# soedinglab/PEnG-motif

Measured on AMD Instinct MI355X. Metric: 4^W pattern z-scores/s + EM PWM-kmer evals/s at W=10; Gbp/s k-mer count, higher is better.
Workload: dtype u32 counts / f32 scores / f32 serial EM sums (f64 tree sums in the throughput EM mode)

## Files before the change

### include/pengk.h

```cpp
#ifndef PENGK_H_
#define PENGK_H_

#include <stddef.h>
#include <stdint.h>

#ifdef __cplusplus
extern "C" {
#endif
#if defined(__GNUC__)
#pragma GCC visibility push(default)
#endif

#define PENGK_VERSION 100

#define PENGK_OK 0
#define PENGK_ERR_ARG 1
#define PENGK_ERR_DEVICE 2
#define PENGK_ERR_RANGE 3
#define PENGK_ERR_UNSUPPORTED 4
#define PENGK_ERR_NOMEM 5

#define PENGK_MIN_W 2
#define PENGK_MAX_W 14
#define PENGK_FRONT_PAD_BASES 64
#define PENGK_DEFAULT_ITEM_WINDOWS 256
#define PENGK_MIN_ITEM_WINDOWS 64

typedef struct pengk_ctx pengk_ctx;

int pengk_version(void);
const char* pengk_last_error(void);
const char* pengk_error_name(int code);

int pengk_create(int device, pengk_ctx** out);
int pengk_destroy(pengk_ctx* ctx);
int pengk_synchronize(pengk_ctx* ctx);
void* pengk_stream(pengk_ctx* ctx);
int pengk_set_stream(pengk_ctx* ctx, void* hip_stream);

int pengk_set_option(pengk_ctx* ctx, const char* name, int64_t value);
int pengk_get_info(pengk_ctx* ctx, const char* name, int64_t* value_out);

int pengk_malloc(pengk_ctx* ctx, size_t bytes, void** d_out);
int pengk_free(pengk_ctx* ctx, void* d_ptr);
int pengk_memcpy_h2d(pengk_ctx* ctx, void* d_dst, const void* h_src, size_t bytes);
int pengk_memcpy_d2h(pengk_ctx* ctx, void* h_dst, const void* d_src, size_t bytes);
int pengk_warmup(pengk_ctx* ctx);
int pengk_memset(pengk_ctx* ctx, void* d_dst, int byte, size_t bytes);
int pengk_host_alloc(pengk_ctx* ctx, size_t bytes, void** h_out);
int pengk_host_free(pengk_ctx* ctx, void* h_ptr);

int pengk_timer_create(pengk_ctx* ctx, void** timer_out);
int pengk_timer_record(pengk_ctx* ctx, void* timer);
int pengk_timer_elapsed_ms(pengk_ctx* ctx, void* start, void* stop, float* ms_out);
int pengk_timer_destroy(pengk_ctx* ctx, void* timer);

typedef struct pengk_packed {
  uint64_t* words;
  uint64_t n_words;
  uint64_t* items;
  uint64_t n_items;
  uint64_t n_bases;
  uint64_t n_windows;
  uint64_t max_bin_bound;
  int64_t bg_counts[84];
  uint64_t n_sequences;
  uint64_t max_len;
  int W;
  int item_windows;
  int all_whole;
} pengk_packed;

int pengk_pack(const uint8_t* h_codes, const int64_t* h_offs, int64_t n_seq, int W, int item_windows,
               pengk_packed* out);
int pengk_pack_threads(const uint8_t* h_codes, const int64_t* h_offs, int64_t n_seq, int W, int item_windows, int threads,
                       pengk_packed* out);
void pengk_packed_free(pengk_packed* p);

typedef struct pengk_pack_target {
  uint64_t* words;
  uint64_t words_cap;
  uint64_t* items;
  uint64_t items_cap;
  uint64_t word_cursor;
  uint64_t item_cursor;
} pengk_pack_target;
int pengk_pack_append(const uint8_t* h_codes, const int64_t* h_offs, int64_t n_seq, int W, int item_windows,
                      pengk_pack_target* target, pengk_packed* out);

int pengk_set_sequences(pengk_ctx* ctx, const uint64_t* d_words, uint64_t n_words, const uint64_t* d_items,
                        uint64_t n_items, int W, int item_windows, uint64_t max_bin_bound, int all_whole);

int pengk_synth_sizes(uint64_t n_seq, uint32_t L, int W, int item_windows, uint64_t* n_words, uint64_t* n_items);
int pengk_synth_sequences(pengk_ctx* ctx, uint64_t seed, uint64_t seq0, uint64_t n_seq, uint32_t L, int W,
                          int item_windows, uint64_t* d_words, uint64_t* d_items);

int pengk_count(pengk_ctx* ctx, int both_strands, uint32_t* d_counts, uint64_t* d_ltot);
int pengk_mirror_counts(pengk_ctx* ctx, int W, uint32_t* d_counts);
int pengk_count_bg(pengk_ctx* ctx, int both_strands, uint32_t* d_counts, uint64_t* d_ltot, uint64_t* d_bg_counts);

int pengk_bg_count(pengk_ctx* ctx, uint64_t* d_bg_counts);

int pengk_bg_model(pengk_ctx* ctx, const uint64_t* d_bg_counts, int K, const float* h_alpha, float* d_V);

int pengk_pattern_stats(pengk_ctx* ctx, int W, int both_strands, int k, int max_k, const float* d_V,
                        const uint64_t* d_ltot, const uint32_t* d_counts, float* d_bgprob, float* d_expected,
                        float* d_logp, float* d_z);

int pengk_seed_candidates(pengk_ctx* ctx, int W, const float* d_z, const uint32_t* d_counts, float z_threshold,
                          uint64_t count_threshold, uint32_t* h_ids, float* h_z, int64_t capacity, int64_t* n_out);

typedef struct pengk_iupac_stats {
  uint64_t sites;
  float bg_p;
  float expected;
  float zscore;
  float log_pvalue;
} pengk_iupac_stats;

int pengk_iupac_aggregate(pengk_ctx* ctx, int W, int both_strands, const uint64_t* h_iupac_ids, int64_t n,
                          const uint32_t* d_counts, const float* d_bgp, const float* d_expected,
                          pengk_iupac_stats* h_out);

int pengk_em(pengk_ctx* ctx, int W, int64_t n_pwm, float* h_pwms, float saturation, float threshold,
             int max_iterations, const uint32_t* d_counts, const float* d_bg, int* h_iters, float* h_change);

int pengk_test_em_generation(pengk_ctx* ctx, int generation);

int pengk_em_device(pengk_ctx* ctx, int W, int64_t n_pwm, float* d_pwms, float saturation, float threshold,
                    int max_iterations, const uint32_t* d_counts, const float* d_bg, int32_t* d_state,
                    float* d_change);

int pengk_sequential_sum_f32(pengk_ctx* ctx, const float* d_terms, uint64_t n_chains, uint64_t chain_len, float* d_out);

#define PENGK_MAX_MOTIF_LEN 64
int pengk_motif_similarity(pengk_ctx* ctx, int n, const float* h_pwm, const float* h_comp, const int32_t* h_len,
                           const uint64_t* h_sites, int both_strands, const float* h_bg, int first_new, float* h_out);

#define PENGK_SCORE_SENTINEL (-2147483647 - 1)

int pengk_scan_layout_words(const int64_t* h_code_offs, int64_t n_seq, uint64_t* n_words);
int pengk_scan_layout_build(const uint8_t* h_codes, const int64_t* h_code_offs, int64_t n_seq, uint64_t word0,
                            uint64_t* h_words, uint32_t* h_valid, int64_t* h_offs, uint32_t* h_lens);
int pengk_synth_scan_sequences(pengk_ctx* ctx, uint64_t seed, uint64_t seq0, uint64_t n_seq, uint32_t L, uint64_t* d_words,
                               uint32_t* d_valid, int64_t* d_offs, uint32_t* d_lens);
int pengk_sample_background(pengk_ctx* ctx, uint64_t seed, uint64_t seq0, uint64_t n_seq, const int64_t* d_offs,
                            const uint32_t* d_lens, int K, const uint32_t* h_thresholds, uint64_t* d_words);
int pengk_shuffle_sequences(pengk_ctx* ctx, uint64_t seed, uint64_t seq0, uint64_t n_seq, const uint64_t* d_words,
                            const uint32_t* d_valid, const int64_t* d_offs, const uint32_t* d_lens, uint64_t* d_out_words,
                            uint32_t* d_out_valid);
int pengk_motif_scan(pengk_ctx* ctx, const uint64_t* d_words, const uint32_t* d_valid, const int64_t* d_offs,
                     const uint32_t* d_lens, uint64_t n_seq, int n_motifs, const int32_t* h_S, const int32_t* h_len,
                     int both_strands, int32_t* d_best);
int pengk_score_histograms(pengk_ctx* ctx, int n_motifs, const int32_t* d_best, uint64_t n_seq, const int32_t* h_lo,
                           const int32_t* h_hi, const uint64_t* h_hist_offs, uint64_t* d_hist);
int pengk_score_summary(const uint64_t* h_pos, const uint64_t* h_neg, uint64_t nbins, double* zoops_out, double* occur_out);

#define PENGK_SITES_BLOCK 4096
typedef struct {
  uint32_t seq;
  uint32_t pos;
  int32_t score;
  uint32_t motif_strand;
} pengk_site;

int pengk_score_tail_pvalues(const int32_t* h_S, int w, const float* h_bg, int32_t* lo_out, int32_t* hi_out, double* h_tail);
int pengk_score_threshold(const double* h_tail, int32_t lo, int32_t hi, double p, int32_t* t_out);
int pengk_sites_count(pengk_ctx* ctx, const uint64_t* d_words, const uint32_t* d_valid, const int64_t* d_offs,
                      const uint32_t* d_lens, uint64_t n_seq, int n_motifs, const int32_t* h_S, const int32_t* h_len,
                      int both_strands, const int32_t* h_thr, uint64_t* d_counts);
int pengk_sites_histograms(pengk_ctx* ctx, const uint64_t* d_words, const uint32_t* d_valid, const int64_t* d_offs,
                           const uint32_t* d_lens, uint64_t n_seq, int n_motifs, const int32_t* h_S, const int32_t* h_len,
                           int both_strands, const int32_t* h_thr, const int32_t* h_hi, const uint64_t* h_hist_offs,
                           uint64_t* d_hist, uint64_t* d_tests, uint64_t* d_counts);
int pengk_sites_qvalues(const uint64_t* h_hist, uint64_t nbins, uint64_t n_tests, const double* h_tail_from_thr, double* h_q);
int pengk_qvalue_threshold(const double* h_q, uint64_t nbins, int32_t t, double q_max, int32_t* t_out);
int pengk_sites_slices(pengk_ctx* ctx, const uint64_t* d_counts, uint64_t n_seq, int n_motifs, uint64_t* h_motif_totals,
                       uint64_t max_slices, uint64_t* h_bounds, uint64_t* h_records, uint64_t* n_slices);
int pengk_sites_emit(pengk_ctx* ctx, const uint64_t* d_words, const uint32_t* d_valid, const int64_t* d_offs,
                     const uint32_t* d_lens, uint64_t n_seq, int n_motifs, const int32_t* h_S, const int32_t* h_len,
                     int both_strands, const int32_t* h_thr, const uint64_t* d_counts, uint64_t i0, uint64_t i1,
                     pengk_site* d_sites, uint64_t cap);

#define PENGK_CENTRALITY_MAX_LEN 65536
int pengk_motif_best_sites(pengk_ctx* ctx, const uint64_t* d_words, const uint32_t* d_valid, const int64_t* d_offs,
                           const uint32_t* d_lens, uint64_t n_seq, uint64_t seq0, int n_motifs, const int32_t* h_S,
                           const int32_t* h_len, int both_strands, int32_t* d_best, uint64_t* d_site);
int pengk_centrality_histograms(pengk_ctx* ctx, int n_motifs, const int32_t* d_best, const uint64_t* d_site,
                                const uint32_t* d_lens, uint64_t n_seq, const int32_t* h_len, const int32_t* h_thr,
                                uint32_t max_len, uint64_t* d_hist_offsets, uint64_t* d_hist_lengths);
typedef struct {
  uint64_t sites;
  uint32_t max_offset;
  uint32_t window;
  uint64_t in_window;
  double expected;
  double log10_pvalue;
  double log10_evalue;
} pengk_centrality;
int pengk_centrality_summary(const uint64_t* h_hist_offsets, const uint64_t* h_hist_lengths, uint32_t max_len, int w,
                             int n_motifs, pengk_centrality* out);
int pengk_binomial_log10_sf(uint64_t n, uint64_t k, double p, double* out);

int pengk_site_profiles(pengk_ctx* ctx, const uint64_t* d_words, const uint32_t* d_valid, const int64_t* d_offs,
                        const uint32_t* d_lens, uint64_t n_seq, int n_motifs, const int32_t* d_best, const uint64_t* d_site,
                        const int32_t* h_len, const int32_t* h_thr, int flank, uint64_t* d_counts);
int pengk_profile_refine(const uint64_t* h_counts, int w, int flank, const float* h_bg, double min_ic, double* h_q,
                         double* h_ic, float* h_pwm, int32_t* first_out, int32_t* last_out, uint64_t* sites_out);

int pengk_site_pair_profiles(pengk_ctx* ctx, const uint64_t* d_words, const uint32_t* d_valid, const int64_t* d_offs,
                             const uint32_t* d_lens, uint64_t n_seq, int n_motifs, const int32_t* d_best, const uint64_t* d_site,
                             const int32_t* h_len, const int32_t* h_thr, int flank, uint64_t* d_counts);
int pengk_dinuc_model(const uint64_t* h_counts1, const uint64_t* h_counts2, int w, int flank, const float* h_bg0,
                      const float* h_bg1, double alpha, double* h_q0, double* h_q1, double* h_mi, int32_t* h_S0, int32_t* h_D1,
                      int32_t* h_D0, uint64_t* sites_out);
int pengk_motif_scan_dinuc(pengk_ctx* ctx, const uint64_t* d_words, const uint32_t* d_valid, const int64_t* d_offs,
                           const uint32_t* d_lens, uint64_t n_seq, int n_motifs, const int32_t* h_S0, const int32_t* h_D,
                           const int32_t* h_len, int both_strands, int32_t* d_best);

#define PENGK_SPACING_MAX_MOTIFS 64
#define PENGK_SPACING_MAX_GAP 1024
int pengk_spacing_histograms(pengk_ctx* ctx, int n_motifs, const int32_t* d_best, const uint64_t* d_site,
                             const uint32_t* d_lens, uint64_t n_seq, const int32_t* h_len, const int32_t* h_thr,
                             uint32_t max_gap, uint32_t min_len, uint32_t max_len,
                             uint64_t* d_hist_gaps,
                             uint64_t* d_hist_lengths,
                             uint64_t* d_hist_motifs);
typedef struct {
  uint64_t both;
  uint64_t overlapping;
  uint64_t apart;
  uint64_t far;
  double expected_both;
  double log10_pvalue_both;
  uint32_t orientation;
  uint32_t gap;
  uint64_t count;
  double expected;
  double log10_pvalue;
  double log10_evalue;
  uint32_t tested_gaps;
} pengk_spacing;
int pengk_spacing_summary(const uint64_t* h_gaps , const uint64_t* h_lengths ,
                          uint32_t max_gap, uint32_t max_len, int w_a, int w_b, int n_classes ,
                          uint64_t n, uint64_t n_a, uint64_t n_b, int n_pairs, pengk_spacing* out);

int pengk_selftest_division(pengk_ctx* ctx, uint64_t seed, uint32_t pairs_per_thread, uint64_t* h_out );

int pengk_comm_host_init_env(void);
int pengk_comm_host_info(int* rank_out, int* world_out);
int pengk_comm_host_allgather(const void* h_send, void* h_recv, size_t bytes_per_rank);
int pengk_comm_host_allreduce_u64(uint64_t* h_buf, size_t n);
int pengk_comm_host_shutdown(void);

#define PENGK_COMM_ID_BYTES 128
int pengk_comm_unique_id(void* id_out );
int pengk_comm_init(pengk_ctx* ctx, const void* id, int rank, int world);
int pengk_comm_init_env(pengk_ctx* ctx);
int pengk_comm_info(pengk_ctx* ctx, int* rank_out, int* world_out);
int pengk_comm_init_abandoned(void);
int pengk_comm_rccl_version(void);
int pengk_comm_destroy(pengk_ctx* ctx);
int pengk_allreduce_tables(pengk_ctx* ctx, int W, uint32_t* d_counts, uint64_t* d_ltot, uint64_t* d_bg_counts);
int pengk_comm_check_bin_bound(pengk_ctx* ctx);
int pengk_allgather(pengk_ctx* ctx, const void* d_send, void* d_recv, size_t bytes_per_rank);

#if defined(__GNUC__)
#pragma GCC visibility pop
#endif
#ifdef __cplusplus
}
#endif
#endif
```

### peng-motif_amd/__init__.py

```python
import ctypes as C
import os

import numpy as np

_HERE = os.path.dirname(os.path.abspath(__file__))
LIB_PATH = os.environ.get("PENGK_LIB") or os.path.join(_HERE, "libpengk.so")
_lib = None

PENGK_OK = 0
ERR_ARG, ERR_DEVICE, ERR_RANGE, ERR_UNSUPPORTED, ERR_NOMEM = 1, 2, 3, 4, 5
FRONT_PAD_BASES = 64

EXPORTS = [
    "pengk_version", "pengk_last_error", "pengk_error_name", "pengk_create", "pengk_destroy", "pengk_synchronize",
    "pengk_stream", "pengk_set_stream", "pengk_set_option", "pengk_get_info", "pengk_malloc", "pengk_free", "pengk_memcpy_h2d", "pengk_memcpy_d2h",
    "pengk_memset", "pengk_warmup", "pengk_host_alloc", "pengk_host_free", "pengk_timer_create", "pengk_timer_record", "pengk_timer_elapsed_ms", "pengk_timer_destroy",
    "pengk_pack", "pengk_pack_threads", "pengk_pack_append", "pengk_packed_free", "pengk_set_sequences", "pengk_synth_sizes", "pengk_synth_sequences",
    "pengk_count", "pengk_count_bg", "pengk_mirror_counts", "pengk_bg_count", "pengk_bg_model", "pengk_pattern_stats",
    "pengk_seed_candidates", "pengk_iupac_aggregate", "pengk_em", "pengk_em_device", "pengk_test_em_generation", "pengk_sequential_sum_f32", "pengk_motif_similarity", "pengk_selftest_division",
    "pengk_comm_unique_id", "pengk_comm_init", "pengk_comm_init_env", "pengk_comm_info", "pengk_comm_init_abandoned", "pengk_comm_rccl_version", "pengk_comm_destroy",
    "pengk_allreduce_tables", "pengk_comm_check_bin_bound", "pengk_allgather",
    "pengk_comm_host_init_env", "pengk_comm_host_info", "pengk_comm_host_allgather", "pengk_comm_host_allreduce_u64",
    "pengk_comm_host_shutdown",
    "pengk_scan_layout_words", "pengk_scan_layout_build", "pengk_synth_scan_sequences", "pengk_sample_background",
    "pengk_shuffle_sequences",
    "pengk_motif_scan", "pengk_score_histograms", "pengk_score_summary",
    "pengk_score_tail_pvalues", "pengk_score_threshold", "pengk_sites_count", "pengk_sites_slices", "pengk_sites_emit",
    "pengk_sites_histograms", "pengk_sites_qvalues", "pengk_qvalue_threshold",
    "pengk_motif_best_sites", "pengk_centrality_histograms", "pengk_centrality_summary", "pengk_binomial_log10_sf",
    "pengk_site_profiles", "pengk_profile_refine",
    "pengk_site_pair_profiles", "pengk_dinuc_model", "pengk_motif_scan_dinuc",
    "pengk_spacing_histograms", "pengk_spacing_summary",
]
MAX_MOTIF_LEN = 64
SCORE_SENTINEL = -2 ** 31
SITES_BLOCK = 4096
SITE = np.dtype([("seq", np.uint32), ("pos", np.uint32), ("score", np.int32), ("motif_strand", np.uint32)])
CENTRALITY_MAX_LEN = 65536
SPACING_MAX_MOTIFS = 64
SPACING_MAX_GAP = 1024
SPACING_CLASSES = ("same_downstream", "same_upstream", "opposite_downstream", "opposite_upstream")


class CentralityStruct(C.Structure):
    _fields_ = [("sites", C.c_uint64), ("max_offset", C.c_uint32), ("window", C.c_uint32), ("in_window", C.c_uint64),
                ("expected", C.c_double), ("log10_pvalue", C.c_double), ("log10_evalue", C.c_double)]


class SpacingStruct(C.Structure):
    _fields_ = [("both", C.c_uint64), ("overlapping", C.c_uint64), ("apart", C.c_uint64), ("far", C.c_uint64),
                ("expected_both", C.c_double), ("log10_pvalue_both", C.c_double), ("orientation", C.c_uint32),
                ("gap", C.c_uint32), ("count", C.c_uint64), ("expected", C.c_double), ("log10_pvalue", C.c_double),
                ("log10_evalue", C.c_double), ("tested_gaps", C.c_uint32)]


class PengkError(RuntimeError):
    def __init__(self, code, msg):
        super().__init__("%s: %s" % (lib().pengk_error_name(code).decode(), msg))
        self.code = code


class PackedStruct(C.Structure):
    _fields_ = [("words", C.POINTER(C.c_uint64)), ("n_words", C.c_uint64), ("items", C.POINTER(C.c_uint64)),
                ("n_items", C.c_uint64), ("n_bases", C.c_uint64), ("n_windows", C.c_uint64), ("max_bin_bound", C.c_uint64),
                ("bg_counts", C.c_int64 * 84), ("n_sequences", C.c_uint64), ("max_len", C.c_uint64), ("W", C.c_int),
                ("item_windows", C.c_int), ("all_whole", C.c_int)]


IUPAC_STATS = np.dtype([("sites", np.uint64), ("bg_p", np.float32), ("expected", np.float32), ("zscore", np.float32),
                        ("log_pvalue", np.float32)], align=True)


def lib():
    global _lib
    if _lib is None:
        if not os.path.exists(LIB_PATH):
            raise ImportError("libpengk.so is not built: run `python peng-motif_amd/build.py` (needs hipcc)")
        L = C.CDLL(LIB_PATH)
        vp, u64, i64, f32 = C.c_void_p, C.c_uint64, C.c_int64, C.c_float
        L.pengk_version.restype = C.c_int
        L.pengk_last_error.restype = C.c_char_p
        L.pengk_error_name.restype = C.c_char_p
        L.pengk_error_name.argtypes = [C.c_int]
        L.pengk_create.argtypes = [C.c_int, C.POINTER(vp)]
        L.pengk_destroy.argtypes = [vp]
        L.pengk_synchronize.argtypes = [vp]
        L.pengk_stream.restype = vp
        L.pengk_stream.argtypes = [vp]
        L.pengk_set_stream.argtypes = [vp, vp]
        L.pengk_set_option.argtypes = [vp, C.c_char_p, i64]
        L.pengk_get_info.argtypes = [vp, C.c_char_p, C.POINTER(i64)]
        L.pengk_malloc.argtypes = [vp, C.c_size_t, C.POINTER(vp)]
        L.pengk_free.argtypes = [vp, vp]
        L.pengk_memcpy_h2d.argtypes = [vp, vp, vp, C.c_size_t]
        L.pengk_memcpy_d2h.argtypes = [vp, vp, vp, C.c_size_t]
        L.pengk_memset.argtypes = [vp, vp, C.c_int, C.c_size_t]
        L.pengk_warmup.argtypes = [vp]
        L.pengk_host_alloc.argtypes = [vp, C.c_size_t, C.POINTER(vp)]
        L.pengk_host_free.argtypes = [vp, vp]
        L.pengk_timer_create.argtypes = [vp, C.POINTER(vp)]
        L.pengk_timer_record.argtypes = [vp, vp]
        L.pengk_timer_elapsed_ms.argtypes = [vp, vp, vp, C.POINTER(f32)]
        L.pengk_timer_destroy.argtypes = [vp, vp]
        L.pengk_pack.argtypes = [vp, vp, i64, C.c_int, C.c_int, C.POINTER(PackedStruct)]
        L.pengk_pack_threads.argtypes = [vp, vp, i64, C.c_int, C.c_int, C.c_int, C.POINTER(PackedStruct)]
        L.pengk_pack_append.argtypes = [vp, vp, i64, C.c_int, C.c_int, vp, C.POINTER(PackedStruct)]
        L.pengk_packed_free.restype = None
        L.pengk_packed_free.argtypes = [C.POINTER(PackedStruct)]
        L.pengk_set_sequences.argtypes = [vp, vp, u64, vp, u64, C.c_int, C.c_int, u64, C.c_int]
        L.pengk_synth_sizes.argtypes = [u64, C.c_uint32, C.c_int, C.c_int, C.POINTER(u64), C.POINTER(u64)]
        L.pengk_synth_sequences.argtypes = [vp, u64, u64, u64, C.c_uint32, C.c_int, C.c_int, vp, vp]
        L.pengk_count.argtypes = [vp, C.c_int, vp, vp]
        L.pengk_count_bg.argtypes = [vp, C.c_int, vp, vp, vp]
        L.pengk_mirror_counts.argtypes = [vp, C.c_int, vp]
        L.pengk_bg_count.argtypes = [vp, vp]
        L.pengk_bg_model.argtypes = [vp, vp, C.c_int, vp, vp]
        L.pengk_pattern_stats.argtypes = [vp, C.c_int, C.c_int, C.c_int, C.c_int, vp, vp, vp, vp, vp, vp, vp]
        L.pengk_seed_candidates.argtypes = [vp, C.c_int, vp, vp, f32, u64, vp, vp, i64, C.POINTER(i64)]
        L.pengk_iupac_aggregate.argtypes = [vp, C.c_int, C.c_int, vp, i64, vp, vp, vp, vp]
        L.pengk_em.argtypes = [vp, C.c_int, i64, vp, f32, f32, C.c_int, vp, vp, vp, vp]
        L.pengk_em_device.argtypes = [vp, C.c_int, i64, vp, f32, f32, C.c_int, vp, vp, vp, vp]
        L.pengk_test_em_generation.argtypes = [vp, C.c_int]
        L.pengk_sequential_sum_f32.argtypes = [vp, vp, u64, u64, vp]
        L.pengk_selftest_division.argtypes = [vp, u64, C.c_uint32, vp]
        L.pengk_motif_similarity.argtypes = [vp, C.c_int, vp, vp, vp, vp, C.c_int, vp, C.c_int, vp]
        L.pengk_comm_unique_id.argtypes = [vp]
        L.pengk_comm_init.argtypes = [vp, vp, C.c_int, C.c_int]
        L.pengk_comm_init_env.argtypes = [vp]
        L.pengk_comm_info.argtypes = [vp, C.POINTER(C.c_int), C.POINTER(C.c_int)]
        L.pengk_comm_destroy.argtypes = [vp]
        L.pengk_allreduce_tables.argtypes = [vp, C.c_int, vp, vp, vp]
        L.pengk_comm_check_bin_bound.argtypes = [vp]
        L.pengk_allgather.argtypes = [vp, vp, vp, C.c_size_t]
        L.pengk_comm_host_init_env.argtypes = []
        L.pengk_comm_host_info.argtypes = [C.POINTER(C.c_int), C.POINTER(C.c_int)]
        L.pengk_comm_host_allgather.argtypes = [vp, vp, C.c_size_t]
        L.pengk_comm_host_allreduce_u64.argtypes = [vp, C.c_size_t]
        L.pengk_comm_host_shutdown.argtypes = []
        L.pengk_scan_layout_words.argtypes = [vp, i64, C.POINTER(u64)]
        L.pengk_scan_layout_build.argtypes = [vp, vp, i64, u64, vp, vp, vp, vp]
        L.pengk_synth_scan_sequences.argtypes = [vp, u64, u64, u64, C.c_uint32, vp, vp, vp, vp]
        L.pengk_sample_background.argtypes = [vp, u64, u64, u64, vp, vp, C.c_int, vp, vp]
        L.pengk_shuffle_sequences.argtypes = [vp, u64, u64, u64, vp, vp, vp, vp, vp, vp]
        L.pengk_motif_scan.argtypes = [vp, vp, vp, vp, vp, u64, C.c_int, vp, vp, C.c_int, vp]
        L.pengk_score_histograms.argtypes = [vp, C.c_int, vp, u64, vp, vp, vp, vp]
        L.pengk_score_summary.argtypes = [vp, vp, u64, C.POINTER(C.c_double), C.POINTER(C.c_double)]
        L.pengk_score_tail_pvalues.argtypes = [vp, C.c_int, vp, C.POINTER(C.c_int32), C.POINTER(C.c_int32), vp]
        L.pengk_score_threshold.argtypes = [vp, C.c_int32, C.c_int32, C.c_double, C.POINTER(C.c_int32)]
        L.pengk_sites_count.argtypes = [vp, vp, vp, vp, vp, u64, C.c_int, vp, vp, C.c_int, vp, vp]
        L.pengk_sites_histograms.argtypes = [vp, vp, vp, vp, vp, u64, C.c_int, vp, vp, C.c_int, vp, vp, vp, vp, vp, vp]
        L.pengk_sites_qvalues.argtypes = [vp, u64, u64, vp, vp]
        L.pengk_qvalue_threshold.argtypes = [vp, u64, C.c_int32, C.c_double, C.POINTER(C.c_int32)]
        L.pengk_sites_slices.argtypes = [vp, vp, u64, C.c_int, vp, u64, vp, vp, C.POINTER(u64)]
        L.pengk_sites_emit.argtypes = [vp, vp, vp, vp, vp, u64, C.c_int, vp, vp, C.c_int, vp, vp, u64, u64, vp, u64]
        L.pengk_motif_best_sites.argtypes = [vp, vp, vp, vp, vp, u64, u64, C.c_int, vp, vp, C.c_int, vp, vp]
        L.pengk_centrality_histograms.argtypes = [vp, C.c_int, vp, vp, vp, u64, vp, vp, C.c_uint32, vp, vp]
        L.pengk_centrality_summary.argtypes = [vp, vp, C.c_uint32, C.c_int, C.c_int, C.POINTER(CentralityStruct)]
        L.pengk_binomial_log10_sf.argtypes = [u64, u64, C.c_double, C.POINTER(C.c_double)]
        L.pengk_site_profiles.argtypes = [vp, vp, vp, vp, vp, u64, C.c_int, vp, vp, vp, vp, C.c_int, vp]
        L.pengk_profile_refine.argtypes = [vp, C.c_int, C.c_int, vp, C.c_double, vp, vp, vp, C.POINTER(C.c_int32),
                                           C.POINTER(C.c_int32), C.POINTER(u64)]
        L.pengk_site_pair_profiles.argtypes = [vp, vp, vp, vp, vp, u64, C.c_int, vp, vp, vp, vp, C.c_int, vp]
        L.pengk_dinuc_model.argtypes = [vp, vp, C.c_int, C.c_int, vp, vp, C.c_double, vp, vp, vp, vp, vp, vp, C.POINTER(u64)]
        L.pengk_motif_scan_dinuc.argtypes = [vp, vp, vp, vp, vp, u64, C.c_int, vp, vp, vp, C.c_int, vp]
        L.pengk_spacing_histograms.argtypes = [vp, C.c_int, vp, vp, vp, u64, vp, vp, C.c_uint32, C.c_uint32, C.c_uint32, vp, vp, vp]
        L.pengk_spacing_summary.argtypes = [vp, vp, C.c_uint32, C.c_uint32, C.c_int, C.c_int, C.c_int, u64, u64, u64, C.c_int,
                                            C.POINTER(SpacingStruct)]
        _lib = L
    return _lib


def _check(rc):
    if rc != PENGK_OK:
        raise PengkError(rc, lib().pengk_last_error().decode())


class Packed:

    def __init__(self, codes, offs, W, item_windows=0):
        codes = np.ascontiguousarray(codes, np.uint8)
        offs = np.ascontiguousarray(offs, np.int64)
        st = PackedStruct()
        _check(lib().pengk_pack(codes.ctypes.data, offs.ctypes.data, len(offs) - 1, W, item_windows, C.byref(st)))
        try:
            self.words = np.ctypeslib.as_array(st.words, shape=(st.n_words,)).copy()
            self.items = np.ctypeslib.as_array(st.items, shape=(max(st.n_items, 1),)).copy()[:st.n_items]
            self.n_bases = int(st.n_bases)
            self.n_windows = int(st.n_windows)
            self.max_bin_bound = int(st.max_bin_bound)
            self.bg_counts = np.array(list(st.bg_counts), np.int64)
            self.n_sequences = int(st.n_sequences)
            self.max_len = int(st.max_len)
            self.W = int(st.W)
            self.item_windows = int(st.item_windows)
            self.all_whole = int(st.all_whole)
        finally:
            lib().pengk_packed_free(C.byref(st))


class ScanLayout:

    def __init__(self, codes, offs):
        codes = np.ascontiguousarray(codes, np.uint8)
        offs = np.ascontiguousarray(offs, np.int64)
        n = len(offs) - 1
        nw = C.c_uint64()
        _check(lib().pengk_scan_layout_words(offs.ctypes.data, n, C.byref(nw)))
        self.n_seq = n
        self.words = np.zeros(max(nw.value, 1), np.uint64)
        self.valid = np.zeros(max(nw.value, 1), np.uint32)
        self.offs = np.zeros(max(n, 1), np.int64)
        self.lens = np.zeros(max(n, 1), np.uint32)
        _check(lib().pengk_scan_layout_build(codes.ctypes.data, offs.ctypes.data, n, 0, self.words.ctypes.data,
                                             self.valid.ctypes.data, self.offs.ctypes.data, self.lens.ctypes.data))


def score_summary(pos_hist, neg_hist):
    p = np.ascontiguousarray(pos_hist, np.uint64)
    n = np.ascontiguousarray(neg_hist, np.uint64)
    assert p.shape == n.shape
    z, o = C.c_double(), C.c_double()
    _check(lib().pengk_score_summary(p.ctypes.data, n.ctypes.data, len(p), C.byref(z), C.byref(o)))
    return z.value, o.value


def score_tail_pvalues(S, bg):
    S = np.ascontiguousarray(S, np.int32)
    bg = np.ascontiguousarray(bg, np.float32)
    lo, hi = C.c_int32(), C.c_int32()
    _check(lib().pengk_score_tail_pvalues(S.ctypes.data, S.shape[0], bg.ctypes.data, C.byref(lo), C.byref(hi), None))
    tail = np.zeros(hi.value - lo.value + 1, np.float64)
    _check(lib().pengk_score_tail_pvalues(S.ctypes.data, S.shape[0], bg.ctypes.data, C.byref(lo), C.byref(hi), tail.ctypes.data))
    return lo.value, tail


def score_threshold(tail, lo, p):
    tail = np.ascontiguousarray(tail, np.float64)
    t = C.c_int32()
    _check(lib().pengk_score_threshold(tail.ctypes.data, lo, lo + len(tail) - 1, p, C.byref(t)))
    return t.value


def sites_qvalues(hist, n_tests, tail_from_thr):
    h = np.ascontiguousarray(hist, np.uint64)
    tail = np.ascontiguousarray(tail_from_thr, np.float64)
    assert len(tail) >= len(h)
    q = np.zeros(len(h), np.float64)
    _check(lib().pengk_sites_qvalues(h.ctypes.data, len(h), int(n_tests), tail.ctypes.data, q.ctypes.data))
    return q


def qvalue_threshold(q, t, q_max):
    q = np.ascontiguousarray(q, np.float64)
    out = C.c_int32()
    _check(lib().pengk_qvalue_threshold(q.ctypes.data, len(q), t, q_max, C.byref(out)))
    return out.value


def centrality_summary(hist_offsets, hist_lengths, max_len, w, n_motifs):
    hd = np.ascontiguousarray(hist_offsets, np.uint64)
    hl = np.ascontiguousarray(hist_lengths, np.uint64)
    assert len(hd) == 2 * max_len + 1 and len(hl) == max_len + 1
    out = CentralityStruct()
    _check(lib().pengk_centrality_summary(hd.ctypes.data, hl.ctypes.data, max_len, w, n_motifs, C.byref(out)))
    return {k: getattr(out, k) for k, _ in CentralityStruct._fields_}


def binomial_log10_sf(n, k, p):
    out = C.c_double()
    _check(lib().pengk_binomial_log10_sf(int(n), int(k), float(p), C.byref(out)))
    return out.value


def spacing_summary(hist_gaps, hist_lengths, max_gap, max_len, w_a, w_b, n_classes, n, n_a, n_b, n_pairs):
    hg = np.ascontiguousarray(hist_gaps, np.uint64)
    hl = np.ascontiguousarray(hist_lengths, np.uint64)
    assert len(hg) == 4 * (max_gap + 1) + 2 and len(hl) == max_len + 1
    out = SpacingStruct()
    _check(lib().pengk_spacing_summary(hg.ctypes.data, hl.ctypes.data, max_gap, max_len, w_a, w_b, n_classes, int(n), int(n_a),
                                       int(n_b), n_pairs, C.byref(out)))
    return {k: getattr(out, k) for k, _ in SpacingStruct._fields_}


def clamp_flank(w, flank):
    return min(int(flank), (MAX_MOTIF_LEN - int(w)) // 2)


def profile_refine(counts, w, flank, bg, min_ic):
    F = clamp_flank(w, flank)
    n = w + 2 * F
    k = np.ascontiguousarray(np.asarray(counts, np.uint64).reshape(-1, 5)[:n])
    assert len(k) == n
    b = np.ascontiguousarray(bg, np.float32)
    q, ic = np.zeros((n, 4), np.float64), np.zeros(n, np.float64)
    pwm = np.zeros((MAX_MOTIF_LEN, 4), np.float32)
    first, last, sites = C.c_int32(), C.c_int32(), C.c_uint64()
    _check(lib().pengk_profile_refine(k.ctypes.data, w, int(flank), b.ctypes.data, float(min_ic), q.ctypes.data, ic.ctypes.data,
                                      pwm.ctypes.data, C.byref(first), C.byref(last), C.byref(sites)))
    return {"q": q, "ic": ic, "first": first.value, "last": last.value, "pwm": pwm[:last.value - first.value].copy(),
            "sites": sites.value}


def dinuc_model(counts1, counts2, w, flank, bg0, bg1, alpha):
    F = clamp_flank(w, flank)
    n = w + 2 * F
    k1 = np.ascontiguousarray(np.asarray(counts1, np.uint64).reshape(-1, 5)[:n])
    k2 = np.ascontiguousarray(np.asarray(counts2, np.uint64).reshape(-1, 17)[:n])
    assert len(k1) == n and len(k2) == n
    g0 = np.ascontiguousarray(bg0, np.float32)
    g1 = np.ascontiguousarray(bg1, np.float32).reshape(-1)
    assert len(g0) == 4 and len(g1) == 16
    q0, q1, mi = np.zeros((n, 4), np.float64), np.zeros((n, 16), np.float64), np.zeros(n, np.float64)
    S0, D1, D0 = np.zeros(4, np.int32), np.zeros((n, 16), np.int32), np.zeros((n, 16), np.int32)
    sites = C.c_uint64()
    _check(lib().pengk_dinuc_model(k1.ctypes.data, k2.ctypes.data, w, int(flank), g0.ctypes.data, g1.ctypes.data, float(alpha),
                                   q0.ctypes.data, q1.ctypes.data, mi.ctypes.data, S0.ctypes.data, D1.ctypes.data,
                                   D0.ctypes.data, C.byref(sites)))
    return {"q0": q0, "q1": q1, "mi": mi, "S0": S0, "D1": D1, "D0": D0, "sites": sites.value, "flank": F}


def _pad_motifs(S, lens):
    n = len(lens)
    Sp = np.zeros((max(n, 1), MAX_MOTIF_LEN, 4), np.int32)
    for m in range(n):
        Sp[m, :lens[m]] = np.asarray(S[m], np.int32)[:lens[m]]
    return Sp, np.ascontiguousarray(lens, np.int32)


class DeviceArray:

    def __init__(self, ctx, shape, dtype):
        self.ctx = ctx
        self.shape = tuple(np.atleast_1d(shape).tolist())
        self.dtype = np.dtype(dtype)
        self.nbytes = int(np.prod(self.shape)) * self.dtype.itemsize
        p = C.c_void_p()
        _check(lib().pengk_malloc(ctx.h, self.nbytes, C.byref(p)))
        self.ptr = p.value

    @classmethod
    def from_host(cls, ctx, a):
        a = np.ascontiguousarray(a)
        d = cls(ctx, a.shape, a.dtype)
        if d.nbytes:
            _check(lib().pengk_memcpy_h2d(ctx.h, d.ptr, a.ctypes.data, d.nbytes))
        return d

    def to_host(self):
        out = np.empty(self.shape, self.dtype)
        if self.nbytes:
            _check(lib().pengk_memcpy_d2h(self.ctx.h, out.ctypes.data, self.ptr, self.nbytes))
        return out

    def free(self):
        if self.ptr and self.ctx.h:
            lib().pengk_free(self.ctx.h, self.ptr)
        self.ptr = None

    def __del__(self):
        try:
            self.free()
        except Exception:
            pass


def _ptr(x):
    if isinstance(x, DeviceArray):
        return x.ptr
    if hasattr(x, "data_ptr"):
        return x.data_ptr()
    return int(x)


class Context:
    def __init__(self, device=0):
        h = C.c_void_p()
        self.h = None
        _check(lib().pengk_create(device, C.byref(h)))
        self.h = h.value
        self._keep = []
        self.W = None

    def close(self):
        if self.h:
            for k in self._keep:
                if isinstance(k, DeviceArray):
                    k.free()
            self._keep = []
            lib().pengk_destroy(self.h)
            self.h = None

    def __del__(self):
        try:
            self.close()
        except Exception:
            pass

    def synchronize(self):
        _check(lib().pengk_synchronize(self.h))

    def set_option(self, name, value):
        _check(lib().pengk_set_option(self.h, name.encode(), int(value)))

    def test_em_generation(self, generation):
        _check(lib().pengk_test_em_generation(self.h, int(generation)))

    def info(self, name):
        v = C.c_int64()
        _check(lib().pengk_get_info(self.h, name.encode(), C.byref(v)))
        return int(v.value)

    def empty(self, shape, dtype):
        return DeviceArray(self, shape, dtype)

    def to_device(self, a):
        return DeviceArray.from_host(self, a)

    def timer(self):
        t = C.c_void_p()
        _check(lib().pengk_timer_create(self.h, C.byref(t)))
        return t.value

    def record(self, t):
        _check(lib().pengk_timer_record(self.h, t))

    def elapsed_ms(self, a, b):
        ms = C.c_float()
        _check(lib().pengk_timer_elapsed_ms(self.h, a, b, C.byref(ms)))
        return float(ms.value)

    def set_sequences(self, words, items, n_words, n_items, W, item_windows, max_bin_bound, all_whole):
        _check(lib().pengk_set_sequences(self.h, _ptr(words), n_words, _ptr(items), n_items, W, item_windows,
                                         max_bin_bound, all_whole))
        self._keep = [words, items]
        self.W = W

    def upload(self, packed):
        words = self.to_device(packed.words)
        items = self.to_device(packed.items if len(packed.items) else np.zeros(1, np.uint64))
        self.set_sequences(words, items, len(packed.words), len(packed.items), packed.W, packed.item_windows,
                           packed.max_bin_bound, packed.all_whole)
        self.set_option("n_windows_hint", packed.n_windows)
        return words, items

    def synth(self, seed, seq0, n_seq, L, W, item_windows=0, words=None, items=None):
        nw, ni = C.c_uint64(), C.c_uint64()
        _check(lib().pengk_synth_sizes(n_seq, L, W, item_windows, C.byref(nw), C.byref(ni)))
        if words is None:
            words = self.empty(nw.value, np.uint64)
        if items is None:
            items = self.empty(max(ni.value, 1), np.uint64)
        _check(lib().pengk_synth_sequences(self.h, seed, seq0, n_seq, L, W, item_windows, _ptr(words), _ptr(items)))
        self._keep = [words, items]
        self.W = W
        return words, items, int(nw.value), int(ni.value)

    def count(self, both, counts=None, ltot=None):
        if counts is None:
            counts = self.empty(4 ** self.W, np.uint32)
        if ltot is None:
            ltot = self.empty(1, np.uint64)
        _check(lib().pengk_count(self.h, int(both), _ptr(counts), _ptr(ltot)))
        return counts, ltot

    def count_bg(self, both, counts=None, ltot=None, bg=None):
        counts = counts if counts is not None else self.empty(4 ** self.W, np.uint32)
        ltot = ltot if ltot is not None else self.empty(1, np.uint64)
        bg = bg if bg is not None else self.empty(84, np.uint64)
        _check(lib().pengk_count_bg(self.h, int(both), _ptr(counts), _ptr(ltot), _ptr(bg)))
        return counts, ltot, bg

    def mirror(self, W, counts):
        _check(lib().pengk_mirror_counts(self.h, W, _ptr(counts)))

    def bg_count(self, out=None):
        if out is None:
            out = self.empty(84, np.uint64)
        _check(lib().pengk_bg_count(self.h, _ptr(out)))
        return out

    def bg_model(self, bg_counts, K=2, alpha=(1.0, 1.0, 1.0), out=None):
        if out is None:
            out = self.empty(84, np.float32)
        a = np.asarray(alpha, np.float32)
        _check(lib().pengk_bg_model(self.h, _ptr(bg_counts), K, a.ctypes.data, _ptr(out)))
        return out

    def pattern_stats(self, W, both, k, max_k, V, ltot, counts, bgprob=None, expected=None, logp=None, z=None):
        n = 4 ** W
        bgprob = bgprob if bgprob is not None else self.empty((max_k + 1, n), np.float32)
        expected = expected if expected is not None else self.empty(n, np.float32)
        logp = logp if logp is not None else self.empty(n, np.float32)
        z = z if z is not None else self.empty(n, np.float32)
        _check(lib().pengk_pattern_stats(self.h, W, int(both), k, max_k, _ptr(V), _ptr(ltot), _ptr(counts), _ptr(bgprob),
                                         _ptr(expected), _ptr(logp), _ptr(z)))
        return bgprob, expected, logp, z

    def iupac_aggregate(self, W, both, ids, counts, bgp, expected):
        ids = np.ascontiguousarray(ids, np.uint64)
        out = np.zeros(len(ids), IUPAC_STATS)
        assert IUPAC_STATS.itemsize == 24
        _check(lib().pengk_iupac_aggregate(self.h, W, int(both), ids.ctypes.data, len(ids), _ptr(counts), _ptr(bgp),
                                           _ptr(expected), out.ctypes.data))
        return out

    def em(self, W, pwms, counts, bg, saturation=1e4, threshold=0.08, max_iterations=10):
        p = np.ascontiguousarray(pwms, np.float32).copy().reshape(-1, W, 4)
        n = p.shape[0]
        iters = np.zeros(n, np.int32)
        change = np.zeros(n, np.float32)
        _check(lib().pengk_em(self.h, W, n, p.ctypes.data, saturation, threshold, max_iterations, _ptr(counts), _ptr(bg),
                              iters.ctypes.data, change.ctypes.data))
        return p, iters, change

    def sequential_sum(self, terms):
        t = np.ascontiguousarray(terms, np.float32)
        t = t.reshape(1, -1) if t.ndim == 1 else t
        d_t = DeviceArray.from_host(self, t.reshape(-1)) if t.size else None
        d_o = DeviceArray.from_host(self, np.zeros(max(t.shape[0], 1), np.float32))
        _check(lib().pengk_sequential_sum_f32(self.h, _ptr(d_t) if d_t is not None else None, t.shape[0], t.shape[1], _ptr(d_o)))
        return d_o.to_host()[:t.shape[0]]

    def upload_scan(self, layout):
        return (self.to_device(layout.words), self.to_device(layout.valid), self.to_device(layout.offs),
                self.to_device(layout.lens), layout.n_seq)

    def synth_scan(self, seed, seq0, n_seq, L):
        nw = n_seq * ((L + 31) // 32)
        words, valid = self.empty(max(nw, 1), np.uint64), self.empty(max(nw, 1), np.uint32)
        offs, lens = self.empty(max(n_seq, 1), np.int64), self.empty(max(n_seq, 1), np.uint32)
        _check(lib().pengk_synth_scan_sequences(self.h, seed, seq0, n_seq, L, _ptr(words), _ptr(valid), _ptr(offs), _ptr(lens)))
        return words, valid, offs, lens, n_seq

    def sample_background(self, scan, seed, seq0, K, thresholds, words=None):
        th = np.ascontiguousarray(thresholds, np.uint32).reshape(-1)
        assert len(th) == 3 * (1, 5, 21)[K]
        if words is None:
            words = self.empty(scan[0].shape, np.uint64)
        _check(lib().pengk_sample_background(self.h, seed, seq0, scan[4], _ptr(scan[2]), _ptr(scan[3]), K, th.ctypes.data,
                                             _ptr(words)))
        return words

    def shuffle_sequences(self, scan, seed, seq0, all_valid=False, words=None, valid=None):
        if words is None:
            words = self.empty(scan[0].shape, np.uint64)
        if valid is None and not all_valid:
            valid = self.empty(scan[1].shape, np.uint32)
        _check(lib().pengk_shuffle_sequences(self.h, seed, seq0, scan[4], _ptr(scan[0]), None if all_valid else _ptr(scan[1]),
                                             _ptr(scan[2]), _ptr(scan[3]), _ptr(words), None if valid is None else _ptr(valid)))
        return words, valid

    def motif_scan(self, scan, S, lens, both, words=None, all_valid=False, best=None):
        n = len(lens)
        Sp = np.zeros((max(n, 1), MAX_MOTIF_LEN, 4), np.int32)
        for m in range(n):
            Sp[m, :lens[m]] = np.asarray(S[m], np.int32)[:lens[m]]
        ln = np.ascontiguousarray(lens, np.int32)
        if best is None:
            best = self.empty((max(n, 1), max(scan[4], 1)), np.int32)
# ... 176 lines not shown
```

### peng-motif_amd/csrc/api.hip

```cpp
#include <stdarg.h>
#include <stdio.h>
#include <string.h>
#include <stdlib.h>
#include <time.h>

#include <new>

#include "pengk_internal.h"

namespace pengk {

static thread_local char g_err[512] = "";

int fail(int code, const char* fmt, ...) {
  va_list ap;
  va_start(ap, fmt);
  vsnprintf(g_err, sizeof g_err, fmt, ap);
  va_end(ap);
  return code;
}

int hip_fail(hipError_t e, const char* what) {
  return fail(PENGK_ERR_DEVICE, "%s: %s", what, hipGetErrorString(e));
}

int ensure_scratch(pengk_ctx* ctx, void** slot, size_t* have, size_t need) {
  if (*have >= need) return PENGK_OK;
  if (*slot) PENGK_HIP(hipFree(*slot));
  *slot = nullptr;
  *have = 0;
  PENGK_HIP(hipMalloc(slot, need));
  *have = need;
  return PENGK_OK;
}

int enter(pengk_ctx* ctx) {
  PENGK_HIP(hipSetDevice(ctx->device));
  return PENGK_OK;
}

static int warm_code_objects() {
  int rc = warm_stats();
  if (!rc) rc = warm_iupac();
  if (!rc) rc = warm_em();
  if (!rc) rc = warm_similarity();
  return rc;
}

}

using namespace pengk;

#define PENGK_ENTER(ctx)               \
  do {                                 \
    int rc_enter_ = ::pengk::enter(ctx); \
    if (rc_enter_) return rc_enter_;   \
  } while (0)

extern "C" {

int pengk_version(void) { return PENGK_VERSION; }
const char* pengk_last_error(void) { return g_err; }

const char* pengk_error_name(int code) {
  switch (code) {
    case PENGK_OK: return "PENGK_OK";
    case PENGK_ERR_ARG: return "PENGK_ERR_ARG";
    case PENGK_ERR_DEVICE: return "PENGK_ERR_DEVICE";
    case PENGK_ERR_RANGE: return "PENGK_ERR_RANGE";
    case PENGK_ERR_UNSUPPORTED: return "PENGK_ERR_UNSUPPORTED";
    case PENGK_ERR_NOMEM: return "PENGK_ERR_NOMEM";
    default: return "PENGK_ERR_?";
  }
}

int pengk_create(int device, pengk_ctx** out) {
  if (!out) return fail(PENGK_ERR_ARG, "pengk_create: out is NULL");
  *out = nullptr;
  const bool timing = getenv("PENGK_TIMING_CREATE") != nullptr;
  timespec t_prev;
  clock_gettime(CLOCK_MONOTONIC, &t_prev);
  auto lap = [&](const char* what) {
    if (!timing) return;
    timespec t;
    clock_gettime(CLOCK_MONOTONIC, &t);
    fprintf(stderr, "[pengk_create] %s: %.1f ms\n", what, (t.tv_sec - t_prev.tv_sec) * 1e3 + (t.tv_nsec - t_prev.tv_nsec) * 1e-6);
    t_prev = t;
  };
  int n = 0;
  hipError_t e = hipGetDeviceCount(&n);
  lap("hipGetDeviceCount (runtime start)");
  if (e != hipSuccess || n <= 0)
    return fail(PENGK_ERR_DEVICE, "pengk_create: no HIP device (%s); this library has no CPU fallback",
                e == hipSuccess ? "device count 0" : hipGetErrorString(e));
  if (device < 0 || device >= n) return fail(PENGK_ERR_ARG, "pengk_create: device %d out of range [0,%d)", device, n);
  PENGK_HIP(hipSetDevice(device));
  hipDeviceProp_t prop;
  PENGK_HIP(hipGetDeviceProperties(&prop, device));
  lap("hipSetDevice + properties");
  if (strncmp(prop.gcnArchName, "gfx950", 6) != 0)
    return fail(PENGK_ERR_DEVICE, "pengk_create: device %d is %s; this build targets gfx950 only", device, prop.gcnArchName);
  pengk_ctx* c = new (std::nothrow) pengk_ctx();
  if (!c) return fail(PENGK_ERR_NOMEM, "pengk_create: out of host memory");
  c->device = device;
  c->num_cu = prop.multiProcessorCount;
  e = hipStreamCreateWithFlags(&c->stream, hipStreamNonBlocking);
  if (e != hipSuccess) {
    delete c;
    return hip_fail(e, "hipStreamCreate");
  }
  c->own_stream = true;
  lap("stream");
  int rc = count_init_device();
  lap("kernel attributes (code object load)");
  if (rc) {
    (void)hipStreamDestroy(c->stream);
    delete c;
    return rc;
  }
  *out = c;
  return PENGK_OK;
}

int pengk_destroy(pengk_ctx* ctx) {
  if (!ctx) return PENGK_OK;
  (void)hipSetDevice(ctx->device);
  (void)hipStreamSynchronize(ctx->stream);
  comm_release(ctx);
  if (ctx->d_defer) (void)hipFree(ctx->d_defer);
  if (ctx->d_em_partials) (void)hipFree(ctx->d_em_partials);
  if (ctx->d_em_tables) (void)hipFree(ctx->d_em_tables);
  if (ctx->d_em_blocks) (void)hipFree(ctx->d_em_blocks);
  if (ctx->d_em_counters) (void)hipFree(ctx->d_em_counters);
  if (ctx->d_em_look) (void)hipFree(ctx->d_em_look);
  if (ctx->d_pair_mids) (void)hipFree(ctx->d_pair_mids);
  for (int l = 0; l < 3; ++l) {
    if (ctx->em_streams[l]) (void)hipStreamDestroy(ctx->em_streams[l]);
    if (ctx->em_join[l]) (void)hipEventDestroy(ctx->em_join[l]);
  }
  if (ctx->em_fork) (void)hipEventDestroy(ctx->em_fork);
  if (ctx->d_misc) (void)hipFree(ctx->d_misc);
  if (ctx->d_keys) (void)hipFree(ctx->d_keys);
  if (ctx->d_iupac_big) (void)hipFree(ctx->d_iupac_big);
  if (ctx->d_bg_partials) (void)hipFree(ctx->d_bg_partials);
  if (ctx->d_count_aux) (void)hipFree(ctx->d_count_aux);
  if (ctx->d_sim) (void)hipFree(ctx->d_sim);
  if (ctx->d_score) (void)hipFree(ctx->d_score);
  if (ctx->d_sites) (void)hipFree(ctx->d_sites);
  if (ctx->own_stream && ctx->stream) (void)hipStreamDestroy(ctx->stream);
  delete ctx;
  return PENGK_OK;
}

int pengk_synchronize(pengk_ctx* ctx) {
  if (!ctx) return fail(PENGK_ERR_ARG, "ctx is NULL");
  PENGK_ENTER(ctx);
  PENGK_HIP(hipStreamSynchronize(ctx->stream));
  return PENGK_OK;
}

int pengk_set_option(pengk_ctx* ctx, const char* name, int64_t value) {
  if (!ctx || !name) return fail(PENGK_ERR_ARG, "pengk_set_option: NULL argument");
  if (strcmp(name, "count_impl") == 0) {
    if (value < 0 || value > 2) return fail(PENGK_ERR_ARG, "count_impl must be 0 (auto), 1 (direct) or 2 (partition)");
    ctx->count_impl = (int)value;
    return PENGK_OK;
  }
  if (strcmp(name, "count_group") == 0) {
    if (value != 0 && value != 64 && value != 128) return fail(PENGK_ERR_ARG, "count_group must be 0 (auto), 64 or 128 keys per group");
    ctx->count_group = (int)value;
    return PENGK_OK;
  }
  if (strcmp(name, "count_probe_slice") == 0) {
    if (value < 0) return fail(PENGK_ERR_ARG, "count_probe_slice must be >= 0 (wave * buckets + bucket)");
    ctx->count_probe_slice = (uint64_t)value;
    return PENGK_OK;
  }
  if (strcmp(name, "key_cap_override") == 0) {
    ctx->key_cap_override = (uint64_t)value;
    return PENGK_OK;
  }
  if (strcmp(name, "em_fast") == 0) {
    if (value < 0 || value > 2) return fail(PENGK_ERR_ARG, "em_fast must be 0 (reference terms), 1 (fast) or 2 (serial, bit-exact)");
    ctx->em_fast = (int)value;
    return PENGK_OK;
  }
  if (strcmp(name, "em_serial_scan") == 0) {
    if (value < 2 || value > 3)
      return fail(PENGK_ERR_ARG, "em_serial_scan must be 2 (blocks evaluated ahead of their chain, three launches per iteration) or 3 (two: weights and block evaluation as one kernel); earlier generations: pengk_test_em_generation");
    ctx->em_serial_scan = (int)value;
    return PENGK_OK;
  }
  if (strcmp(name, "em_test_lookback") == 0) {
    if (value < 0 || value > 1000000) return fail(PENGK_ERR_ARG, "em_test_lookback must be 0 (off) or the n of 'every n-th workgroup'");
    ctx->em_test_lookback = (int)value;
    return PENGK_OK;
  }
  if (strcmp(name, "em_test_skew") == 0) {
    if (value < 0 || value > 1000000) return fail(PENGK_ERR_ARG, "em_test_skew must be 0 (off) or the n of 'every n-th block'");
    ctx->em_test_skew = (int)value;
    return PENGK_OK;
  }
  if (strcmp(name, "em_head_blocks") == 0) {
    if (value < 1 || value > 64) return PENGK_ERR_ARG;
    ctx->em_head_blocks = (int)value;
    return PENGK_OK;
  }
  if (strcmp(name, "sweep_pairs") == 0) {
    ctx->sweep_pairs = value != 0;
    return PENGK_OK;
  }
  if (strcmp(name, "em_lean_div") == 0) {
    ctx->em_lean_div = value != 0;
    return PENGK_OK;
  }
  if (strcmp(name, "em_overlap") == 0) {
    if (value < 1 || value > MAX_EM_LANES) return fail(PENGK_ERR_ARG, "em_overlap must be 1 .. %d streams", MAX_EM_LANES);
    ctx->em_overlap = (int)value;
    return PENGK_OK;
  }
  if (strcmp(name, "em_table_budget_mb") == 0) {
    if (value < 0) return fail(PENGK_ERR_ARG, "em_table_budget_mb must be >= 0 (0 = automatic)");
    ctx->em_table_budget_mb = (uint64_t)value;
    return PENGK_OK;
  }
  if (strcmp(name, "iupac_group_bytes") == 0) {
    ctx->iupac_group_bytes = (uint64_t)value;
    return PENGK_OK;
  }
  if (strcmp(name, "sites_record_budget") == 0) {
    if (value < 1) return fail(PENGK_ERR_ARG, "sites_record_budget must be >= 1 record");
    ctx->sites_record_budget = (uint64_t)value;
    return PENGK_OK;
  }
  if (strcmp(name, "scatter_blocks_per_cu") == 0) {
    if (value < 0 || value > 8) return fail(PENGK_ERR_ARG, "scatter_blocks_per_cu must be 0 (default) .. 8");
    ctx->scatter_blocks_per_cu = (int)value;
    return PENGK_OK;
  }
  if (strcmp(name, "n_windows_hint") == 0) {
    ctx->n_windows_hint = (uint64_t)value;
    return PENGK_OK;
  }
  return fail(PENGK_ERR_ARG, "unknown option '%s'", name);
}

int pengk_get_info(pengk_ctx* ctx, const char* name, int64_t* value) {
  if (!ctx || !name || !value) return fail(PENGK_ERR_ARG, "pengk_get_info: NULL argument");
  PENGK_ENTER(ctx);
  if (strcmp(name, "deferred_items") == 0) {
    uint32_t n = 0;
    if (ctx->d_defer_count) {
      PENGK_HIP(hipMemcpyAsync(&n, ctx->d_defer_count, sizeof n, hipMemcpyDeviceToHost, ctx->stream));
      PENGK_HIP(hipStreamSynchronize(ctx->stream));
    }
    *value = n;
    return PENGK_OK;
  }
  if (strcmp(name, "count_wrapped_workgroups") == 0) {
    uint32_t n = 0;
    if (ctx->d_wrap_count) {
      PENGK_HIP(hipMemcpyAsync(&n, ctx->d_wrap_count, sizeof n, hipMemcpyDeviceToHost, ctx->stream));
      PENGK_HIP(hipStreamSynchronize(ctx->stream));
    }
    *value = n;
    return PENGK_OK;
  }
  if (strcmp(name, "count_group") == 0) {
    *value = ctx->count_group;
    return PENGK_OK;
  }
  if (strcmp(name, "count_group_used") == 0) {
    *value = ctx->count_group_used;
    return PENGK_OK;
  }
  if (strcmp(name, "count_slices") == 0) {
    *value = ctx->d_slice_fill ? (int64_t)ctx->n_slice_fill : 0;
    return PENGK_OK;
  }
  if (strcmp(name, "count_slice_fill") == 0) {
    if (!ctx->d_slice_fill || ctx->count_probe_slice >= ctx->n_slice_fill)
      return fail(PENGK_ERR_ARG, "count_slice_fill: the last count has no slice %llu", (unsigned long long)ctx->count_probe_slice);
    uint32_t n = 0;
    PENGK_HIP(hipMemcpyAsync(&n, ctx->d_slice_fill + ctx->count_probe_slice, sizeof n, hipMemcpyDeviceToHost, ctx->stream));
    PENGK_HIP(hipStreamSynchronize(ctx->stream));
    *value = n;
    return PENGK_OK;
  }
  if (strcmp(name, "sites_record_budget") == 0) {
    *value = (int64_t)ctx->sites_record_budget;
    return PENGK_OK;
  }
  if (strcmp(name, "num_cu") == 0) {
    *value = ctx->num_cu;
    return PENGK_OK;
  }
  static const char* const em_names[4] = {"em_fetched_blocks", "em_mispredicted_blocks", "em_restaged_blocks", "em_restaged_waits"};
  for (int i = 0; i < 4; ++i)
    if (strcmp(name, em_names[i]) == 0) {
      unsigned long long v = 0;
      if (ctx->d_em_counters) {
        PENGK_HIP(hipMemcpyAsync(&v, ctx->d_em_counters + i, sizeof v, hipMemcpyDeviceToHost, ctx->stream));
        PENGK_HIP(hipStreamSynchronize(ctx->stream));
      }
      *value = (int64_t)v;
      return PENGK_OK;
    }
  return fail(PENGK_ERR_ARG, "unknown info '%s'", name);
}

void* pengk_stream(pengk_ctx* ctx) { return ctx ? (void*)ctx->stream : nullptr; }

int pengk_set_stream(pengk_ctx* ctx, void* s) {
  if (!ctx) return fail(PENGK_ERR_ARG, "ctx is NULL");
  PENGK_ENTER(ctx);
  PENGK_HIP(hipStreamSynchronize(ctx->stream));
  if (ctx->own_stream && ctx->stream) PENGK_HIP(hipStreamDestroy(ctx->stream));
  ctx->stream = (hipStream_t)s;
  ctx->own_stream = false;
  return PENGK_OK;
}

int pengk_malloc(pengk_ctx* ctx, size_t bytes, void** d_out) {
  if (!ctx || !d_out) return fail(PENGK_ERR_ARG, "pengk_malloc: NULL argument");
  PENGK_HIP(hipSetDevice(ctx->device));
  hipError_t e = hipMalloc(d_out, bytes ? bytes : 1);
  if (e != hipSuccess) return fail(PENGK_ERR_NOMEM, "hipMalloc(%zu): %s", bytes, hipGetErrorString(e));
  return PENGK_OK;
}

int pengk_free(pengk_ctx* ctx, void* d_ptr) {
  if (!ctx) return fail(PENGK_ERR_ARG, "ctx is NULL");
  PENGK_ENTER(ctx);
  if (d_ptr) {
    PENGK_HIP(hipStreamSynchronize(ctx->stream));
    PENGK_HIP(hipFree(d_ptr));
  }
  return PENGK_OK;
}

int pengk_host_alloc(pengk_ctx* ctx, size_t bytes, void** h_out) {
  if (!ctx || !h_out) return fail(PENGK_ERR_ARG, "pengk_host_alloc: NULL argument");
  PENGK_HIP(hipSetDevice(ctx->device));
  hipError_t e = hipHostMalloc(h_out, bytes ? bytes : 1, hipHostMallocDefault);
  if (e != hipSuccess) return fail(PENGK_ERR_NOMEM, "hipHostMalloc(%zu): %s", bytes, hipGetErrorString(e));
  return PENGK_OK;
}

int pengk_host_free(pengk_ctx* ctx, void* h_ptr) {
  if (!ctx) return fail(PENGK_ERR_ARG, "ctx is NULL");
  PENGK_ENTER(ctx);
  if (h_ptr) {
    PENGK_HIP(hipStreamSynchronize(ctx->stream));
    PENGK_HIP(hipHostFree(h_ptr));
  }
  return PENGK_OK;
}

int pengk_memcpy_h2d(pengk_ctx* ctx, void* d_dst, const void* h_src, size_t bytes) {
  if (!ctx || (bytes && (!d_dst || !h_src))) return fail(PENGK_ERR_ARG, "pengk_memcpy_h2d: NULL argument");
  PENGK_ENTER(ctx);
  PENGK_HIP(hipMemcpyAsync(d_dst, h_src, bytes, hipMemcpyHostToDevice, ctx->stream));
  PENGK_HIP(hipStreamSynchronize(ctx->stream));
  return PENGK_OK;
}

int pengk_warmup(pengk_ctx* ctx) {
  if (!ctx) return fail(PENGK_ERR_ARG, "ctx is NULL");
  PENGK_ENTER(ctx);
  constexpr size_t N = (size_t)4 << 20;
  void* d = nullptr;
  void* h = nullptr;
  hipError_t e = hipMalloc(&d, N);
  if (e == hipSuccess) e = hipHostMalloc(&h, N, hipHostMallocDefault);
  if (e == hipSuccess) e = hipMemcpyAsync(h, d, N, hipMemcpyDeviceToHost, ctx->stream);
  if (e == hipSuccess) e = hipStreamSynchronize(ctx->stream);
  if (h) (void)hipHostFree(h);
  if (d) (void)hipFree(d);
  if (e != hipSuccess) return hip_fail(e, "pengk_warmup");
  return warm_code_objects();
}

int pengk_memcpy_d2h(pengk_ctx* ctx, void* h_dst, const void* d_src, size_t bytes) {
  if (!ctx || (bytes && (!h_dst || !d_src))) return fail(PENGK_ERR_ARG, "pengk_memcpy_d2h: NULL argument");
  PENGK_ENTER(ctx);
  PENGK_HIP(hipMemcpyAsync(h_dst, d_src, bytes, hipMemcpyDeviceToHost, ctx->stream));
  PENGK_HIP(hipStreamSynchronize(ctx->stream));
  return PENGK_OK;
}

int pengk_memset(pengk_ctx* ctx, void* d_dst, int byte, size_t bytes) {
  if (!ctx || (bytes && !d_dst)) return fail(PENGK_ERR_ARG, "pengk_memset: NULL argument");
  PENGK_ENTER(ctx);
  PENGK_HIP(hipMemsetAsync(d_dst, byte, bytes, ctx->stream));
  return PENGK_OK;
}

int pengk_timer_create(pengk_ctx* ctx, void** out) {
  if (!ctx || !out) return fail(PENGK_ERR_ARG, "pengk_timer_create: NULL argument");
  PENGK_ENTER(ctx);
  hipEvent_t ev;
  PENGK_HIP(hipEventCreate(&ev));
  *out = (void*)ev;
  return PENGK_OK;
}
int pengk_timer_record(pengk_ctx* ctx, void* t) {
  if (!ctx || !t) return fail(PENGK_ERR_ARG, "pengk_timer_record: NULL argument");
  PENGK_ENTER(ctx);
  PENGK_HIP(hipEventRecord((hipEvent_t)t, ctx->stream));
  return PENGK_OK;
}
int pengk_timer_elapsed_ms(pengk_ctx* ctx, void* a, void* b, float* ms) {
  if (!ctx || !a || !b || !ms) return fail(PENGK_ERR_ARG, "pengk_timer_elapsed_ms: NULL argument");
  PENGK_ENTER(ctx);
  PENGK_HIP(hipEventSynchronize((hipEvent_t)b));
  PENGK_HIP(hipEventElapsedTime(ms, (hipEvent_t)a, (hipEvent_t)b));
  return PENGK_OK;
}
int pengk_timer_destroy(pengk_ctx* ctx, void* t) {
  (void)ctx;
  if (t) PENGK_HIP(hipEventDestroy((hipEvent_t)t));
  return PENGK_OK;
// ... 28 lines not shown
  const uint64_t per = (nwin + item_windows - 1) / item_windows;
  *n_items = n_seq * per;
  const uint64_t bases = PENGK_FRONT_PAD_BASES + n_seq * (uint64_t)L;
  *n_words = (bases + 31) / 32 + 4;
  return PENGK_OK;
}

int pengk_synth_sequences(pengk_ctx* ctx, uint64_t seed, uint64_t seq0, uint64_t n_seq, uint32_t L, int W,
                          int item_windows, uint64_t* d_words, uint64_t* d_items) {
  if (!ctx || !d_words || !d_items) return fail(PENGK_ERR_ARG, "pengk_synth_sequences: NULL argument");
  PENGK_ENTER(ctx);
  if (item_windows == 0) item_windows = PENGK_DEFAULT_ITEM_WINDOWS;
  uint64_t nw = 0, ni = 0;
  int rc = pengk_synth_sizes(n_seq, L, W, item_windows, &nw, &ni);
  if (rc) return rc;
  if (item_windows < PENGK_MIN_ITEM_WINDOWS || item_windows > 65535) return fail(PENGK_ERR_ARG, "item_windows out of range");
  rc = launch_synth(ctx, seed, seq0, n_seq, L, W, item_windows, d_words, d_items);
  if (rc) return rc;
  const uint64_t nwin = (uint64_t)L - W + 1;
  rc = pengk_set_sequences(ctx, d_words, nw, d_items, ni, W, item_windows, n_seq * ((nwin + W - 1) / W), 1);
  if (rc) return rc;
  ctx->n_windows_hint = n_seq * nwin;
  return PENGK_OK;
}

int pengk_count(pengk_ctx* ctx, int both, uint32_t* d_counts, uint64_t* d_ltot) {
  if (!ctx || !d_counts || !d_ltot) return fail(PENGK_ERR_ARG, "pengk_count: NULL argument");
  if (!ctx->d_words) return fail(PENGK_ERR_ARG, "pengk_count: no sequences attached");
  PENGK_ENTER(ctx);
  if (ctx->max_bin_bound >= (1ull << 32))
    return fail(PENGK_ERR_RANGE, "a count bin could reach %llu >= 2^32 on this shard; split the input",
                (unsigned long long)ctx->max_bin_bound);
  return launch_count(ctx, both ? 1 : 0, d_counts, d_ltot, nullptr);
}

int pengk_count_bg(pengk_ctx* ctx, int both, uint32_t* d_counts, uint64_t* d_ltot, uint64_t* d_bg) {
  if (!ctx || !d_counts || !d_ltot || !d_bg) return fail(PENGK_ERR_ARG, "pengk_count_bg: NULL argument");
  if (!ctx->d_words) return fail(PENGK_ERR_ARG, "pengk_count_bg: no sequences attached");
  PENGK_ENTER(ctx);
  if (!ctx->all_whole)
    return fail(PENGK_ERR_UNSUPPORTED, "pengk_count_bg: input has invalid bases or sequences shorter than W; use pengk_packed.bg_counts");
  if (ctx->max_bin_bound >= (1ull << 32))
    return fail(PENGK_ERR_RANGE, "a count bin could reach %llu >= 2^32 on this shard; split the input",
                (unsigned long long)ctx->max_bin_bound);
  return launch_count(ctx, both ? 1 : 0, d_counts, d_ltot, d_bg);
}

int pengk_mirror_counts(pengk_ctx* ctx, int W, uint32_t* d_counts) {
  if (!ctx || !d_counts) return fail(PENGK_ERR_ARG, "pengk_mirror_counts: NULL argument");
  PENGK_ENTER(ctx);
  if (!valid_w(W)) return fail(PENGK_ERR_ARG, "pattern length %d unsupported", W);
  return launch_mirror(ctx, W, d_counts);
}

int pengk_bg_count(pengk_ctx* ctx, uint64_t* d_bg) {
  if (!ctx || !d_bg) return fail(PENGK_ERR_ARG, "pengk_bg_count: NULL argument");
  if (!ctx->d_words) return fail(PENGK_ERR_ARG, "pengk_bg_count: no sequences attached");
  PENGK_ENTER(ctx);
  if (!ctx->all_whole)
    return fail(PENGK_ERR_UNSUPPORTED, "pengk_bg_count: input has invalid bases or sequences shorter than W; use pengk_packed.bg_counts");
  return launch_bg_count(ctx, d_bg);
}

int pengk_bg_model(pengk_ctx* ctx, const uint64_t* d_bg, int K, const float* h_alpha, float* d_V) {
  if (!ctx || !d_bg || !h_alpha || !d_V) return fail(PENGK_ERR_ARG, "pengk_bg_model: NULL argument");
  PENGK_ENTER(ctx);
  if (K < 0 || K > 2) return fail(PENGK_ERR_ARG, "background order %d unsupported (0..2)", K);
  return launch_bg_model(ctx, d_bg, K, h_alpha, d_V);
}

int pengk_pattern_stats(pengk_ctx* ctx, int W, int both, int k, int max_k, const float* d_V, const uint64_t* d_ltot,
                        const uint32_t* d_counts, float* d_bgprob, float* d_expected, float* d_logp, float* d_z) {
  if (!ctx || !d_V || !d_ltot || !d_counts || !d_bgprob || !d_expected || !d_logp || !d_z)
    return fail(PENGK_ERR_ARG, "pengk_pattern_stats: NULL argument");
  PENGK_ENTER(ctx);
  if (!valid_w(W)) return fail(PENGK_ERR_ARG, "pattern length %d unsupported", W);
  if (k < 0 || max_k > 2 || k > max_k || max_k > W - 1) return fail(PENGK_ERR_ARG, "background orders k=%d max_k=%d unsupported", k, max_k);
  return launch_stats(ctx, W, both ? 1 : 0, k, max_k, d_V, d_ltot, d_counts, d_bgprob, d_expected, d_logp, d_z);
}

int pengk_seed_candidates(pengk_ctx* ctx, int W, const float* d_z, const uint32_t* d_counts, float z_threshold,
                          uint64_t count_threshold, uint32_t* h_ids, float* h_z, int64_t capacity, int64_t* n_out) {
  if (!ctx || !d_z || !d_counts || !n_out || (capacity && (!h_ids || !h_z))) return fail(PENGK_ERR_ARG, "pengk_seed_candidates: NULL argument");
  if (!valid_w(W)) return fail(PENGK_ERR_ARG, "pattern length %d unsupported", W);
  if (capacity < 0 || capacity > (int64_t)1 << 28) return fail(PENGK_ERR_ARG, "pengk_seed_candidates: capacity out of range");
  PENGK_ENTER(ctx);
  const uint32_t cap = (uint32_t)capacity;
  const size_t need = 256 + (size_t)cap * 8;
  int rc = ensure_scratch(ctx, &ctx->d_misc, &ctx->misc_bytes, need);
  if (rc) return rc;
  uint32_t* d_n = (uint32_t*)ctx->d_misc;
  uint32_t* d_ids = (uint32_t*)((char*)ctx->d_misc + 256);
  float* d_zs = (float*)(d_ids + cap);
  rc = launch_seed_candidates(ctx, W, d_z, d_counts, z_threshold, count_threshold, cap, d_n, d_ids, d_zs);
  if (rc) return rc;
  uint32_t n = 0;
  PENGK_HIP(hipMemcpyAsync(&n, d_n, sizeof n, hipMemcpyDeviceToHost, ctx->stream));
  PENGK_HIP(hipStreamSynchronize(ctx->stream));
  *n_out = n;
  const uint32_t got = n < cap ? n : cap;
  if (got) {
    PENGK_HIP(hipMemcpyAsync(h_ids, d_ids, (size_t)got * 4, hipMemcpyDeviceToHost, ctx->stream));
    PENGK_HIP(hipMemcpyAsync(h_z, d_zs, (size_t)got * 4, hipMemcpyDeviceToHost, ctx->stream));
    PENGK_HIP(hipStreamSynchronize(ctx->stream));
  }
  return PENGK_OK;
}

int pengk_iupac_aggregate(pengk_ctx* ctx, int W, int both, const uint64_t* h_ids, int64_t n, const uint32_t* d_counts,
                          const float* d_bgp, const float* d_expected, pengk_iupac_stats* h_out) {
  if (!ctx || (n && (!h_ids || !h_out)) || !d_counts || !d_bgp || !d_expected)
    return fail(PENGK_ERR_ARG, "pengk_iupac_aggregate: NULL argument");
  PENGK_ENTER(ctx);
  if (!valid_w(W)) return fail(PENGK_ERR_ARG, "pattern length %d unsupported", W);
  if (n < 0) return fail(PENGK_ERR_ARG, "negative pattern count");
  if (n == 0) return PENGK_OK;
  return launch_iupac(ctx, W, both ? 1 : 0, h_ids, n, d_counts, d_bgp, d_expected, h_out);
}

int pengk_motif_similarity(pengk_ctx* ctx, int n, const float* h_pwm, const float* h_comp, const int32_t* h_len,
                           const uint64_t* h_sites, int both, const float* h_bg, int first_new, float* h_out) {
  if (!ctx || !h_pwm || !h_comp || !h_len || !h_sites || !h_bg || !h_out) return fail(PENGK_ERR_ARG, "pengk_motif_similarity: NULL argument");
  if (n < 0 || first_new < 0 || first_new > n) return fail(PENGK_ERR_ARG, "pengk_motif_similarity: n = %d, first_new = %d", n, first_new);
  for (int i = 0; i < n; ++i)
    if (h_len[i] < 1 || h_len[i] > PENGK_MAX_MOTIF_LEN)
      return fail(PENGK_ERR_UNSUPPORTED, "pengk_motif_similarity: motif %d has %d columns (1..%d)", i, h_len[i], PENGK_MAX_MOTIF_LEN);
  long long pairs = 0;
  for (int j = first_new; j < n; ++j) pairs += j;
  if (pairs == 0) return PENGK_OK;
  PENGK_ENTER(ctx);
  const size_t pw = (size_t)n * PENGK_MAX_MOTIF_LEN * 4 * sizeof(float);
  const size_t o_len = 2 * pw, o_sites = (o_len + (size_t)n * 4 + 255) & ~(size_t)255, o_out = (o_sites + (size_t)n * 8 + 255) & ~(size_t)255;
  int rc = ensure_scratch(ctx, &ctx->d_sim, &ctx->sim_bytes, o_out + (size_t)pairs * sizeof(float));
  if (rc) return rc;
  char* base = (char*)ctx->d_sim;
  PENGK_HIP(hipMemcpyAsync(base, h_pwm, pw, hipMemcpyHostToDevice, ctx->stream));
  PENGK_HIP(hipMemcpyAsync(base + pw, h_comp, pw, hipMemcpyHostToDevice, ctx->stream));
  PENGK_HIP(hipMemcpyAsync(base + o_len, h_len, (size_t)n * 4, hipMemcpyHostToDevice, ctx->stream));
  PENGK_HIP(hipMemcpyAsync(base + o_sites, h_sites, (size_t)n * 8, hipMemcpyHostToDevice, ctx->stream));
  rc = launch_similarity(ctx, n, (const float*)base, (const float*)(base + pw), (const int32_t*)(base + o_len),
                         (const uint64_t*)(base + o_sites), both ? 1 : 0, h_bg, first_new, (float*)(base + o_out));
  if (rc) return rc;
  PENGK_HIP(hipMemcpyAsync(h_out, base + o_out, (size_t)pairs * sizeof(float), hipMemcpyDeviceToHost, ctx->stream));
  PENGK_HIP(hipStreamSynchronize(ctx->stream));
  return PENGK_OK;
}

int pengk_sequential_sum_f32(pengk_ctx* ctx, const float* d_terms, uint64_t n_chains, uint64_t chain_len, float* d_out) {
  if (!ctx || (!d_terms && n_chains && chain_len) || (!d_out && n_chains)) return fail(PENGK_ERR_ARG, "pengk_sequential_sum_f32: NULL argument");
  PENGK_ENTER(ctx);
  return launch_sequential_sum(ctx, d_terms, n_chains, chain_len, d_out);
}

int pengk_test_em_generation(pengk_ctx* ctx, int generation) {
  if (!ctx) return fail(PENGK_ERR_ARG, "pengk_test_em_generation: NULL context");
  if (generation < 0 || generation > 3) return fail(PENGK_ERR_ARG, "pengk_test_em_generation: 0 (dependent additions), 1 (scan), 2 / 3 (the library's scheme)");
  ctx->em_serial_scan = generation;
  return PENGK_OK;
}

int pengk_em_device(pengk_ctx* ctx, int W, int64_t n_pwm, float* d_pwms, float saturation, float threshold, int max_it,
                    const uint32_t* d_counts, const float* d_bg, int32_t* d_state, float* d_change) {
  if (!ctx || !d_pwms || !d_counts || !d_bg || !d_state || !d_change) return fail(PENGK_ERR_ARG, "pengk_em_device: NULL argument");
  PENGK_ENTER(ctx);
  if (!valid_w(W)) return fail(PENGK_ERR_ARG, "pattern length %d unsupported", W);
  if (n_pwm < 0) return fail(PENGK_ERR_ARG, "negative count");
  if (max_it < 0) max_it = 0;
  if (n_pwm == 0) return PENGK_OK;
  return launch_em(ctx, W, n_pwm, d_pwms, saturation, threshold, max_it, d_counts, d_bg, d_state, d_change);
}

int pengk_em(pengk_ctx* ctx, int W, int64_t n_pwm, float* h_pwms, float saturation, float threshold, int max_it,
             const uint32_t* d_counts, const float* d_bg, int* h_iters, float* h_change) {
  if (!ctx || (n_pwm && !h_pwms) || !d_counts || !d_bg) return fail(PENGK_ERR_ARG, "pengk_em: NULL argument");
  PENGK_ENTER(ctx);
  if (!valid_w(W)) return fail(PENGK_ERR_ARG, "pattern length %d unsupported", W);
  if (n_pwm < 0) return fail(PENGK_ERR_ARG, "negative count");
  if (max_it < 0) max_it = 0;
  if (n_pwm == 0) return PENGK_OK;
  const size_t pw = (size_t)n_pwm * W * 4 * sizeof(float);
  const size_t st = (size_t)n_pwm * 2 * sizeof(int32_t);
  const size_t ch = (size_t)n_pwm * sizeof(float);
  const size_t need = ((pw + 255) & ~(size_t)255) + ((st + 255) & ~(size_t)255) + ch;
  int rc = ensure_scratch(ctx, &ctx->d_misc, &ctx->misc_bytes, need);
  if (rc) return rc;
  float* d_pwms = (float*)ctx->d_misc;
  int32_t* d_state = (int32_t*)((char*)ctx->d_misc + ((pw + 255) & ~(size_t)255));
  float* d_change = (float*)((char*)d_state + ((st + 255) & ~(size_t)255));
  PENGK_HIP(hipMemcpyAsync(d_pwms, h_pwms, pw, hipMemcpyHostToDevice, ctx->stream));
  rc = launch_em(ctx, W, n_pwm, d_pwms, saturation, threshold, max_it, d_counts, d_bg, d_state, d_change);
  if (rc) return rc;
  PENGK_HIP(hipMemcpyAsync(h_pwms, d_pwms, pw, hipMemcpyDeviceToHost, ctx->stream));
  PENGK_HIP(hipStreamSynchronize(ctx->stream));
  if (h_iters || h_change) {
    int32_t* tmp = new (std::nothrow) int32_t[(size_t)n_pwm * 2];
    if (!tmp) return fail(PENGK_ERR_NOMEM, "pengk_em: out of host memory");
    hipError_t e = hipMemcpy(tmp, d_state, st, hipMemcpyDeviceToHost);
    if (e == hipSuccess && h_change) e = hipMemcpy(h_change, d_change, ch, hipMemcpyDeviceToHost);
    if (h_iters)
      for (int64_t i = 0; i < n_pwm; ++i) h_iters[i] = tmp[2 * i];
    delete[] tmp;
    if (e != hipSuccess) return hip_fail(e, "pengk_em: copy back");
  }
  return PENGK_OK;
}

}
```

### peng-motif_amd/csrc/count.hip

```cpp
#include <stdlib.h>

#include <type_traits>

#include "pengk_internal.h"

namespace pengk {

namespace {

constexpr uint32_t INVALID_ID = 0xFFFFFFFFu;

__device__ __forceinline__ uint32_t funnel(uint32_t hi, uint32_t lo, uint32_t shift) {
  return __builtin_amdgcn_alignbit(hi, lo, shift);
}

template <int W>
struct Geo {
  static constexpr int P = ((3 * W - 3 + 15) / 16) * 16;
  static constexpr uint32_t MASK = (1u << (2 * W)) - 1u;
  static constexpr int TOP = 2 * (W - 1);
  static constexpr int PER = (32 - 2 * W) / 2 + 1;
  static constexpr int NVIEW = (W - 1 + PER - 1) / PER;
};

__device__ __forceinline__ uint32_t revcomp16(uint32_t x) {
  const uint32_t r = __builtin_bitreverse32(x);
  return ~(((r >> 1) & 0x55555555u) | ((r & 0x55555555u) << 1));
}

struct BgLds {
  uint32_t bins[96];
  uint32_t bins4[256];
};
__device__ __forceinline__ BgLds& bg_lds() {
  __shared__ BgLds sh;
  return sh;
}
template <int W, bool BG>
struct BgCount {
  uint32_t wave;
  __device__ __forceinline__ void kmer3(uint32_t id, bool on) const {
    if (BG) atomicAdd(&bg_lds().bins[on ? (id >> (2 * W - 6)) : 95u], 1u);
  }
  __device__ __forceinline__ void kmer4(uint32_t v) const {
    if (BG) atomicAdd(&bg_lds().bins4[v], 1u);
  }
  __device__ __forceinline__ void head(uint32_t id, int sp, bool on) const {
    if (!BG || !on || sp < 0) return;
    if (sp == 0) atomicAdd(&bg_lds().bins[64 + (id >> (2 * W - 2))], 1u);
    else if (sp == 1) atomicAdd(&bg_lds().bins[68 + (id >> (2 * W - 4))], 1u);
    else atomicAdd(&bg_lds().bins[id >> (2 * W - 6)], 1u);
  }
};

template <bool BG>
__device__ __forceinline__ void bg_begin() {
  if (BG) {
    for (uint32_t i = threadIdx.x; i < 96u; i += blockDim.x) bg_lds().bins[i] = 0;
    for (uint32_t i = threadIdx.x; i < 256u; i += blockDim.x) bg_lds().bins4[i] = 0;
  }
}
template <bool BG>
__device__ __forceinline__ void bg_end(uint32_t* __restrict__ bg_partials) {
  if (BG) {
    __syncthreads();
    if (threadIdx.x < 84) {
      const BgLds& b = bg_lds();
      const uint32_t k = threadIdx.x;
      uint32_t v = b.bins[k];
      if (k < 64) {
        for (uint32_t c = 0; c < 4; ++c) v += b.bins4[k | (c << 6)] + b.bins4[(k << 2) | c];
      }
      bg_partials[(size_t)blockIdx.x * 84 + k] = v;
    }
  }
}

template <int W>
struct Suppress {
  static __device__ __forceinline__ uint32_t apply(uint32_t can, const uint32_t (&ring)[16], int u) {
    uint32_t out = INVALID_ID;
    unsigned long long save;
#define PENGK_R(d) "v"(ring[(u - (d)) & 15])
#define PENGK_CX(n) "v_cmpx_ne_u32_e32 %2, %" #n "\n\t"
#define PENGK_HEAD "s_mov_b64 %1, exec\n\t"
#define PENGK_TAIL "v_mov_b32_e32 %0, %2\n\ts_mov_b64 exec, %1"
    if constexpr (W == 2)
      asm volatile(PENGK_HEAD PENGK_CX(3) PENGK_TAIL : "+v"(out), "=&s"(save) : "v"(can), PENGK_R(1) : "vcc");
    else if constexpr (W == 4)
      asm volatile(PENGK_HEAD PENGK_CX(3) PENGK_CX(4) PENGK_CX(5) PENGK_TAIL
                   : "+v"(out), "=&s"(save) : "v"(can), PENGK_R(1), PENGK_R(2), PENGK_R(3) : "vcc");
    else if constexpr (W == 6)
      asm volatile(PENGK_HEAD PENGK_CX(3) PENGK_CX(4) PENGK_CX(5) PENGK_CX(6) PENGK_CX(7) PENGK_TAIL
                   : "+v"(out), "=&s"(save) : "v"(can), PENGK_R(1), PENGK_R(2), PENGK_R(3), PENGK_R(4), PENGK_R(5) : "vcc");
    else if constexpr (W == 8)
      asm volatile(PENGK_HEAD PENGK_CX(3) PENGK_CX(4) PENGK_CX(5) PENGK_CX(6) PENGK_CX(7) PENGK_CX(8) PENGK_CX(9) PENGK_TAIL
                   : "+v"(out), "=&s"(save)
                   : "v"(can), PENGK_R(1), PENGK_R(2), PENGK_R(3), PENGK_R(4), PENGK_R(5), PENGK_R(6), PENGK_R(7) : "vcc");
    else if constexpr (W == 10)
      asm volatile(PENGK_HEAD PENGK_CX(3) PENGK_CX(4) PENGK_CX(5) PENGK_CX(6) PENGK_CX(7) PENGK_CX(8) PENGK_CX(9) PENGK_CX(10)
                   PENGK_CX(11) PENGK_TAIL
                   : "+v"(out), "=&s"(save)
                   : "v"(can), PENGK_R(1), PENGK_R(2), PENGK_R(3), PENGK_R(4), PENGK_R(5), PENGK_R(6), PENGK_R(7), PENGK_R(8),
                     PENGK_R(9) : "vcc");
    else if constexpr (W == 12)
      asm volatile(PENGK_HEAD PENGK_CX(3) PENGK_CX(4) PENGK_CX(5) PENGK_CX(6) PENGK_CX(7) PENGK_CX(8) PENGK_CX(9) PENGK_CX(10)
                   PENGK_CX(11) PENGK_CX(12) PENGK_CX(13) PENGK_TAIL
                   : "+v"(out), "=&s"(save)
                   : "v"(can), PENGK_R(1), PENGK_R(2), PENGK_R(3), PENGK_R(4), PENGK_R(5), PENGK_R(6), PENGK_R(7), PENGK_R(8),
                     PENGK_R(9), PENGK_R(10), PENGK_R(11) : "vcc");
    else {
      static_assert(W == 14, "pattern lengths 2 .. 14");
      asm volatile(PENGK_HEAD PENGK_CX(3) PENGK_CX(4) PENGK_CX(5) PENGK_CX(6) PENGK_CX(7) PENGK_CX(8) PENGK_CX(9) PENGK_CX(10)
                   PENGK_CX(11) PENGK_CX(12) PENGK_CX(13) PENGK_CX(14) PENGK_CX(15) PENGK_TAIL
                   : "+v"(out), "=&s"(save)
                   : "v"(can), PENGK_R(1), PENGK_R(2), PENGK_R(3), PENGK_R(4), PENGK_R(5), PENGK_R(6), PENGK_R(7), PENGK_R(8),
                     PENGK_R(9), PENGK_R(10), PENGK_R(11), PENGK_R(12), PENGK_R(13) : "vcc");
    }
#undef PENGK_R
#undef PENGK_CX
#undef PENGK_HEAD
#undef PENGK_TAIL
    return out;
  }
};

template <int W, bool BOTH, bool BG, class Emit>
__device__ __forceinline__ void scan_items(const uint32_t* __restrict__ words32, const uint64_t* __restrict__ items,
                                           uint32_t n_items, unsigned long long* __restrict__ ltot,
                                           uint32_t* __restrict__ defer_count, uint32_t* __restrict__ defer_list,
                                           Emit& emit) {
  using G = Geo<W>;
  const BgCount<W, BG> bgc{threadIdx.x >> 6};
  const uint32_t lane_global = blockIdx.x * blockDim.x + threadIdx.x;
  const uint32_t stride = gridDim.x * blockDim.x;
  unsigned long long my_windows = 0;

  for (uint32_t wave_base = lane_global & ~63u; wave_base < n_items; wave_base += stride) {
    const uint32_t it = wave_base + (threadIdx.x & 63u);
    const bool live = it < n_items;
    const uint64_t rec = live ? items[it] : 0ull;
    uint32_t nw = (uint32_t)((rec >> ITEM_NW_SHIFT) & ITEM_NW_MASK);
    const uint64_t ws = rec & ITEM_WS_MASK;
    const bool cont = ((rec >> ITEM_CONT_SHIFT) & 1ull) != 0;
    const uint32_t nw_all = nw;
    my_windows += nw;

    uint32_t ring[16];
#pragma unroll
    for (int i = 0; i < 16; ++i) ring[i] = INVALID_ID;
    uint32_t id = 0, rc = 0;

    const uint64_t g0 = live ? ws + (uint64_t)(W - 1) - (uint64_t)G::P : 0ull;
    uint64_t wi = g0 >> 4;
    const uint32_t shift = 2u * (uint32_t)(g0 & 15u);
    uint32_t lo;
    uint32_t pchunk = 0;

    if (__any(cont ? 1 : 0)) {
      lo = words32[wi];
      bool dirty = false;
      if (cont) {
        uint32_t have = 0;
        for (uint32_t j = it; j > 0 && have < (uint32_t)(G::P - W + 1);) {
          const uint64_t prev = items[--j];
          have += (uint32_t)((prev >> ITEM_NW_SHIFT) & ITEM_NW_MASK);
          if (((prev >> ITEM_CONT_SHIFT) & 1ull) == 0) {
            dirty = have < (uint32_t)(G::P - W + 1);
            break;
          }
        }
      }
#pragma unroll
      for (int ch = 0; ch < G::P / 16; ++ch) {
        const uint32_t hi = words32[wi + 1];
        ++wi;
        const uint32_t chunk = funnel(hi, lo, shift);
        lo = hi;
        pchunk = chunk;
#pragma unroll
        for (int u = 0; u < 16; ++u) {
          const int b = ch * 16 + u;
          const uint32_t c = (chunk >> (2 * u)) & 3u;
          id = (id >> 2) | (c << G::TOP);
          rc = ((rc << 2) & G::MASK) | (c ^ 3u);
          bgc.head(id, b - (G::P - (W - 1)), live && !cont && nw > 0);
          if (b >= W - 1) {
            const uint32_t can = BOTH ? min(id, rc) : id;
            bool match = false;
#pragma unroll
            for (int d = 1; d <= W - 1; ++d)
              if (b - d >= W - 1) match |= (can == ring[(u - d) & 15]);
            dirty |= match;
            ring[u] = (cont && !match) ? can : INVALID_ID;
          }
        }
      }
      if (cont && dirty) {
        const uint32_t slot = atomicAdd(defer_count, 1u);
        defer_list[slot] = it;
        nw = 0;
      }
    } else {
      wi += (G::P / 16) - 1;
      lo = words32[wi];
      const uint32_t hi = words32[wi + 1];
      ++wi;
      const uint32_t chunk = funnel(hi, lo, shift);
      lo = hi;
      pchunk = chunk;
#pragma unroll
      for (int u = 0; u < 16; ++u) {
        const uint32_t c = (chunk >> (2 * u)) & 3u;
        id = (id >> 2) | (c << G::TOP);
        rc = ((rc << 2) & G::MASK) | (c ^ 3u);
        bgc.head(id, u - (17 - W), live && nw > 0);
      }
    }

    const uint32_t nw_scan = BG ? nw_all : nw;
    uint32_t nw_max = nw_scan;
#pragma unroll
    for (int off = 32; off > 0; off >>= 1) nw_max = max(nw_max, (uint32_t)__shfl_xor((int)nw_max, off, 64));
    uint32_t nxt = (0u < nw_scan) ? words32[wi + 1] : 0u;
    uint32_t rprev = revcomp16(pchunk);
    for (uint32_t t0 = 0; t0 < nw_max; t0 += 16) {
      const uint32_t hi = nxt;
      ++wi;
      nxt = (t0 + 16u < nw_scan) ? words32[wi + 1] : 0u;
      const uint32_t chunk = funnel(hi, lo, shift);
      lo = hi;
      const uint32_t rchunk = BOTH ? revcomp16(chunk) : 0u;
      uint32_t view[G::NVIEW], rview[G::NVIEW];
#pragma unroll
      for (int j = 0; j < G::NVIEW; ++j) {
        view[j] = funnel(chunk, pchunk, 2u * (uint32_t)(j * G::PER + 17 - W));
        rview[j] = BOTH ? funnel(rprev, rchunk, 2u * (uint32_t)(j * G::PER + 17 - W)) : 0u;
      }
      auto body = [&](auto mode_tag, uint32_t tail) {
        constexpr bool TAIL = decltype(mode_tag)::value == 2;
        constexpr bool FULL = decltype(mode_tag)::value != 0;
#pragma unroll
        for (int u = 0; u < 16; ++u) {
          if (!TAIL || (uint32_t)u < tail) {
            uint32_t id_u, rc_u = 0;
            if (u >= W - 1) {
              id_u = __builtin_amdgcn_ubfe(chunk, 2u * (uint32_t)(u - (W - 1)), 2u * W);
              if (BOTH) rc_u = __builtin_amdgcn_ubfe(rchunk, 2u * (uint32_t)(15 - u), 2u * W);
            } else {
              const int j = u / G::PER, k = W - 2 - u, jr = k / G::PER;
              id_u = __builtin_amdgcn_ubfe(view[j], 2u * (uint32_t)(u - j * G::PER), 2u * W);
              if (BOTH) rc_u = __builtin_amdgcn_ubfe(rview[jr], 2u * (uint32_t)(k - jr * G::PER), 2u * W);
            }
            const uint32_t can = BOTH ? min(id_u, rc_u) : id_u;
#ifdef PENGK_ABLATE_NOSUPPRESS
            const uint32_t key = can;
#else
            const uint32_t key = Suppress<W>::apply(can, ring, u);
#endif
            ring[u] = key;
            if (FULL) {
              if (BG && (u & 1)) {
                const uint32_t v4 = u >= 3 ? __builtin_amdgcn_ubfe(chunk, 2u * (uint32_t)(u - 3), 8u)
                                           : funnel(chunk, pchunk, 2u * (uint32_t)(13 + u)) & 0xFFu;
                bgc.kmer4(v4);
              } else if (TAIL && BG && (uint32_t)u + 1u == tail) {
                bgc.kmer3(id_u, true);
              }
              emit.full(key);
            } else {
              bgc.kmer3(id_u, t0 + (uint32_t)u < nw_all);
              emit.masked(key, key != INVALID_ID && t0 + (uint32_t)u < nw);
            }
          }
        }
      };
      if (__all((t0 + 16u <= nw && nw == nw_all) ? 1 : 0)) {
        body(std::integral_constant<int, 1>{}, 16u);
      } else {
        const uint32_t nw0 = (uint32_t)__builtin_amdgcn_readfirstlane((int)nw);
        if (__all((nw == nw0 && nw == nw_all) ? 1 : 0)) body(std::integral_constant<int, 2>{}, nw0 - t0);
        else body(std::integral_constant<int, 0>{}, 0u);
      }
      pchunk = chunk;
      rprev = rchunk;
    }
  }

#pragma unroll
  for (int off = 32; off > 0; off >>= 1) my_windows += __shfl_down(my_windows, off, 64);
  if ((threadIdx.x & 63u) == 0 && my_windows) atomicAdd(ltot, my_windows);
}

struct DirectEmit {
  uint32_t* __restrict__ hist;
  __device__ __forceinline__ void masked(uint32_t key, bool active) const {
    if (active) __hip_atomic_fetch_add(&hist[key], 1u, __ATOMIC_RELAXED, __HIP_MEMORY_SCOPE_AGENT);
  }
  __device__ __forceinline__ void full(uint32_t key) const { masked(key, key != INVALID_ID); }
};

template <int W, bool BOTH, bool BG>
__global__ __launch_bounds__(256) void count_kernel(const uint32_t* __restrict__ words32,
                                                    const uint64_t* __restrict__ items, uint32_t n_items,
                                                    uint32_t* __restrict__ hist,
                                                    unsigned long long* __restrict__ ltot,
                                                    uint32_t* __restrict__ defer, uint32_t* __restrict__ bg_partials) {
  bg_begin<BG>();
  if (BG) __syncthreads();
  DirectEmit e{hist};
  scan_items<W, BOTH, BG>(words32, items, n_items, ltot, defer, defer + 1, e);
  bg_end<BG>(bg_partials);
}

constexpr int RING_CAP = 128;
constexpr int GROUP = RING_CAP / 2;
constexpr uint32_t KEY_INVALID = 0xFFFFu;
constexpr int PAYLOAD_BITS = 15;

template <int W, int NBITS>
struct KeySplit {
  static constexpr int S = ((2 * W - NBITS) / 2) & ~1;
  static constexpr uint32_t LOW = (1u << S) - 1u;
  static constexpr uint32_t NB = 1u << NBITS;
  __host__ __device__ static inline uint32_t bucket(uint32_t id) { return (id >> S) & (NB - 1u); }
  __host__ __device__ static inline uint32_t payload(uint32_t id) {
#if defined(__HIP_DEVICE_COMPILE__)
    uint32_t r;
    asm("v_bfi_b32 %0, %1, %2, %3" : "=v"(r) : "s"(LOW), "v"(id), "v"(id >> NBITS));
    return r;
#else
    return (id & LOW) | ((id >> NBITS) & ~LOW);
#endif
  }
  __host__ __device__ static inline uint32_t join(uint32_t b, uint32_t p, uint32_t  = 0) {
    return (p & LOW) | (b << S) | ((p >> S) << (S + NBITS));
  }
  __host__ __device__ static inline bool valid(uint32_t p) { return p != KEY_INVALID; }
};

#ifndef PENGK_W12_L1_BITS
#define PENGK_W12_L1_BITS 4
#endif
struct Split12L1 {
  static constexpr int NBITS = PENGK_W12_L1_BITS;
  static constexpr uint32_t NB = 1u << NBITS;
  static constexpr uint32_t PBITS = 24 - NBITS;
  __host__ __device__ static inline uint32_t bucket(uint32_t id) { return (id >> 8) & (NB - 1u); }
  __host__ __device__ static inline uint32_t payload(uint32_t id) { return (id & 0xFFu) | ((id >> (8 + NBITS)) << 8); }
  __host__ __device__ static inline uint32_t join(uint32_t b1, uint32_t p1, uint32_t  = 0) { return (p1 & 0xFFu) | (b1 << 8) | ((p1 >> 8) << (8 + NBITS)); }
  __host__ __device__ static inline bool valid(uint32_t p1) { return p1 < (1u << PBITS); }
};
struct Split12L2 {
  static constexpr int NBITS = 9 - Split12L1::NBITS;
  static constexpr uint32_t NB = 1u << NBITS;
  __host__ __device__ static inline uint32_t bucket(uint32_t p1) { return (p1 >> 8) & (NB - 1u); }
  __host__ __device__ static inline uint32_t payload(uint32_t p1) { return (p1 & 0xFFu) | ((p1 >> (8 + NBITS)) << 8); }
  __host__ __device__ static inline uint32_t join(uint32_t b2, uint32_t p2, uint32_t outer) {
    const uint32_t p1 = (p2 & 0xFFu) | (b2 << 8) | ((p2 >> 8) << (8 + NBITS));
    return Split12L1::join(outer, p1);
  }
  __host__ __device__ static inline bool valid(uint32_t p2) { return p2 != KEY_INVALID; }
};

struct Split14L1 {
  static constexpr int NBITS = 4;
  static constexpr uint32_t NB = 16;
  __host__ __device__ static inline uint32_t bucket(uint32_t id) { return (id >> 10) & 15u; }
  __host__ __device__ static inline uint32_t payload(uint32_t id) { return (id & 0x3FFu) | ((id >> 14) << 10); }
  __host__ __device__ static inline uint32_t join(uint32_t b1, uint32_t p1, uint32_t  = 0) { return (p1 & 0x3FFu) | (b1 << 10) | ((p1 >> 10) << 14); }
  __host__ __device__ static inline bool valid(uint32_t p1) { return p1 < (1u << 24); }
};
struct Split14L2 {
  static constexpr int NBITS = 4;
  static constexpr uint32_t NB = 16;
  __host__ __device__ static inline uint32_t bucket(uint32_t p1) { return (p1 >> 9) & 15u; }
  __host__ __device__ static inline uint32_t payload(uint32_t p1) { return (p1 & 0x1FFu) | ((p1 >> 13) << 9); }
  __host__ __device__ static inline uint32_t join(uint32_t b2, uint32_t p2, uint32_t outer) {
    return Split14L1::join(outer, (p2 & 0x1FFu) | (b2 << 9) | ((p2 >> 9) << 13));
  }
  __host__ __device__ static inline bool valid(uint32_t p2) { return p2 < (1u << 20); }
};
struct Split14L3 {
  static constexpr int NBITS = 5;
  static constexpr uint32_t NB = 32;
  __host__ __device__ static inline uint32_t bucket(uint32_t p2) { return (p2 >> 8) & 31u; }
  __host__ __device__ static inline uint32_t payload(uint32_t p2) { return (p2 & 0xFFu) | ((p2 >> 13) << 8); }
  __host__ __device__ static inline uint32_t join(uint32_t b3, uint32_t p3, uint32_t outer) {
    return Split14L2::join(outer & 15u, (p3 & 0xFFu) | (b3 << 8) | ((p3 >> 8) << 13), outer >> 4);
  }
  __host__ __device__ static inline bool valid(uint32_t p3) { return p3 != KEY_INVALID; }
};

template <class E, int CAP = RING_CAP>
struct ScatterRowT {
  E ring[CAP];
  uint32_t fill4;
};
template <int NBITS, int WPW, class E = uint16_t, int CAP = RING_CAP>
struct ScatterShared {
  static constexpr int NB = 1 << NBITS;
  ScatterRowT<E, CAP> row[WPW][NB];
};

template <int NBITS, int WPW, class E = uint16_t, int CAP = RING_CAP>
__device__ __forceinline__ ScatterShared<NBITS, WPW, E, CAP>& scatter_lds() {
  __shared__ ScatterShared<NBITS, WPW, E, CAP> sh;
  return sh;
}

template <class KS, int NBITS, int WPW = 4, class E = uint16_t, int G = GROUP>
struct ScatterEmit {
  static constexpr int NB = 1 << NBITS;
  static constexpr int CAP = 2 * G;
  static constexpr uint32_t ES = (uint32_t)sizeof(E);
  static constexpr uint32_t ESH = ES == 2u ? 1u : 2u;
  static constexpr uint32_t STEP = 256u / (uint32_t)G;
  static constexpr uint32_t SSH = G == 64 ? 2u : 1u;
  static constexpr uint32_t MV = ES * (uint32_t)G / 64u;
  static constexpr uint32_t PAD = ES == 2u ? KEY_INVALID : 0xFFFFFFFFu;
  typedef ScatterRowT<E, CAP> Row;
  static_assert(G == 64 || (G == 128 && ES == 2u), "a group is one entry, or one dword of two 16-bit entries, per lane");
  static_assert(STEP * (uint32_t)G == 256u, "byte 0 of the counter addresses the group");
  E* __restrict__ keys;
  uint32_t slice_cap;
  uint32_t* __restrict__ slice_fill;
  uint32_t* __restrict__ hist;
  uint32_t wave, lane, wave_global;
  uint32_t outer;

  static __device__ __forceinline__ void init_lds() {
    ScatterShared<NBITS, WPW, E, CAP>& sh = scatter_lds<NBITS, WPW, E, CAP>();
    static_assert(sizeof(Row) == ES * CAP + 4, "row = ring + counter");
    static_assert((sizeof(Row) / 4u) % 2u == 1u, "odd row stride in dwords");
    uint32_t* w = reinterpret_cast<uint32_t*>(&sh.row[0][0]);
    for (uint32_t i = threadIdx.x; i < (uint32_t)WPW * NB * (sizeof(Row) / 4u); i += blockDim.x)
      w[i] = (i % (uint32_t)(sizeof(Row) / 4u)) == (uint32_t)(ES * CAP / 4u) ? 0u : 0xFFFFFFFFu;
  }

  typedef __attribute__((address_space(3))) uint32_t lds_u32_t;
  typedef __attribute__((address_space(3))) E lds_e_t;
  typedef __attribute__((address_space(1))) E global_e_t;
  typedef __attribute__((address_space(1))) uint32_t global_u32_t;

  __device__ __forceinline__ void flush_triggered(unsigned long long trig, uint32_t row, uint32_t b, uint32_t s4,
                                                  uint32_t nvalid = (uint32_t)G) {
    asm volatile("");
    const uint32_t g4 = s4 - STEP * (uint32_t)(G - 1);
    const uint32_t src = row + ((g4 >> (SSH - ESH)) & (ES * (uint32_t)G));
    const uint32_t dst = b * (ES * slice_cap) + (g4 >> (SSH - ESH));
    const unsigned long long fits = __builtin_amdgcn_ballot_w64(g4 + STEP * G <= STEP * slice_cap);
    unsigned long long todo = trig & fits;
    unsigned long long over = trig & ~fits;
    while (todo) {
      const int p = __builtin_ctzll(todo);
      todo &= todo - 1;
      const uint32_t s_src = (uint32_t)__builtin_amdgcn_readlane((int)src, p);
      const uint32_t s_dst = (uint32_t)__builtin_amdgcn_readlane((int)dst, p);
      if constexpr (MV == ES) {
        uint32_t v = *(lds_e_t*)(uintptr_t)(s_src + ES * lane);
        asm volatile("" : "+v"(v));
        global_e_t* out = (global_e_t*)((char*)region + s_dst);
        __builtin_nontemporal_store((E)v, &out[lane]);
      } else {
        uint32_t v = *(lds_u32_t*)(uintptr_t)(s_src + 4u * lane);
        asm volatile("" : "+v"(v));
        global_u32_t* out = (global_u32_t*)((char*)region + s_dst);
        __builtin_nontemporal_store(v, &out[lane]);
      }
    }
    while (over) {
      const int p = __builtin_ctzll(over);
      over &= over - 1;
      const uint32_t s_src = (uint32_t)__builtin_amdgcn_readlane((int)src, p);
      const uint32_t fb = (uint32_t)__builtin_amdgcn_readlane((int)b, p);
      if constexpr (MV == ES) {
        const uint32_t v = *(lds_e_t*)(uintptr_t)(s_src + ES * lane);
        if (KS::valid(v)) __hip_atomic_fetch_add(&hist[KS::join(fb, v, outer)], 1u, __ATOMIC_RELAXED, __HIP_MEMORY_SCOPE_AGENT);
      } else {
        const uint32_t nv = (uint32_t)__builtin_amdgcn_readlane((int)nvalid, p);
        const uint32_t v = *(lds_u32_t*)(uintptr_t)(s_src + 4u * lane);
        if (2u * lane < nv)
          __hip_atomic_fetch_add(&hist[KS::join(fb, v & 0xFFFFu, outer)], 1u, __ATOMIC_RELAXED, __HIP_MEMORY_SCOPE_AGENT);
        if (2u * lane + 1u < nv)
          __hip_atomic_fetch_add(&hist[KS::join(fb, v >> 16, outer)], 1u, __ATOMIC_RELAXED, __HIP_MEMORY_SCOPE_AGENT);
      }
    }
  }

  uint32_t rowbase = 0;
  __device__ __forceinline__ void bind() {
    rowbase = (uint32_t)(uintptr_t)(__attribute__((address_space(3))) char*)&scatter_lds<NBITS, WPW, E, CAP>().row[wave][0];
    asm volatile("" : "+v"(rowbase));
    region = keys + (size_t)wave_global * NB * slice_cap;
  }
  E* region = nullptr;

  __device__ __forceinline__ uint32_t append(uint32_t b, uint32_t key, uint32_t& row) const {
    row = b * (uint32_t)sizeof(Row) + rowbase;
    const uint32_t s4 = __hip_atomic_fetch_add((lds_u32_t*)(uintptr_t)(row + ES * CAP), STEP, __ATOMIC_RELAXED,
                                               __HIP_MEMORY_SCOPE_WORKGROUP);
    *(lds_e_t*)(uintptr_t)(row + ((s4 >> (SSH - ESH)) & (ES * CAP - 1u))) = (E)KS::payload(key);
    return s4;
  }

  __device__ __forceinline__ void full(uint32_t key) {
    const uint32_t b = KS::bucket(key);
    uint32_t row;
    const uint32_t s4 = append(b, key, row);
    const unsigned long long trig = __builtin_amdgcn_ballot_w64((s4 & 0xFFu) == STEP * (uint32_t)(G - 1));
    if (trig) flush_triggered(trig, row, b, s4);
  }

  __device__ __forceinline__ void masked(uint32_t key, bool active) {
    const uint32_t b = KS::bucket(key);
    uint32_t s4 = 0, row = 0;
    if (active) s4 = append(b, key, row);
    const unsigned long long trig = __builtin_amdgcn_ballot_w64(active && (s4 & 0xFFu) == STEP * (uint32_t)(G - 1));
    if (trig) flush_triggered(trig, row, b, s4);
  }

  __device__ __forceinline__ void drain() {
    __builtin_amdgcn_wave_barrier();
    uint32_t row = 0, s4_last = 0, nvalid = 0;
    bool padded = false;
    if (lane < (uint32_t)NB) {
      row = lane * (uint32_t)sizeof(Row) + rowbase;
      const uint32_t c4 = __hip_atomic_load((lds_u32_t*)(uintptr_t)(row + ES * CAP), __ATOMIC_RELAXED, __HIP_MEMORY_SCOPE_WAVEFRONT);
      const uint32_t r = (c4 >> SSH) & (uint32_t)(G - 1);
      if (r) {
        if constexpr (G == 64) {
          for (uint32_t i = r; i < (uint32_t)G; ++i)
            *(lds_e_t*)(uintptr_t)(row + (((c4 >> (SSH - ESH)) & (ES * CAP - 1u)) + ES * (i - r))) = (E)PAD;
        }
        s4_last = c4 + STEP * ((uint32_t)G - r) - STEP;
        nvalid = r;
        padded = true;
      }
      const uint32_t full = G == 64 ? ((c4 >> SSH) + (uint32_t)(G - 1)) & ~(uint32_t)(G - 1) : c4 >> SSH;
      slice_fill[(size_t)wave_global * NB + lane] = full < slice_cap ? full : slice_cap;
    }
    __builtin_amdgcn_wave_barrier();
    const unsigned long long trig = __builtin_amdgcn_ballot_w64(padded);
    if (trig) flush_triggered(trig, row, lane, s4_last, nvalid);
  }
};

#ifndef PENGK_SCATTER_WPW
#define PENGK_SCATTER_WPW 4
#endif
constexpr int SCATTER_WPW = PENGK_SCATTER_WPW;
template <int W, int NBITS>
struct KeySplitTemp : KeySplit<W, NBITS> {
  static constexpr int PBITS = 2 * W - NBITS;
  static constexpr int G = PBITS == 16 ? 128 : GROUP;
  static_assert(PBITS == PAYLOAD_BITS || (PBITS == 16 && W == 10), "15-bit payloads, or 16-bit ones at W = 10");
  __host__ __device__ static inline uint32_t join(uint32_t b, uint32_t p, uint32_t  = 0) { return (b << PBITS) | p; }
  __host__ __device__ static inline uint32_t index(uint32_t id) {
    return (KeySplit<W, NBITS>::bucket(id) << PBITS) | KeySplit<W, NBITS>::payload(id);
  }
};
template <int W, bool BOTH, int NBITS, bool BG>
__global__ __launch_bounds__(64 * SCATTER_WPW) void count_scatter_kernel(const uint32_t* __restrict__ words32,
                                                            const uint64_t* __restrict__ items, uint32_t n_items,
                                                            uint16_t* __restrict__ keys, uint32_t slice_cap,
                                                            uint32_t* __restrict__ slice_fill, uint32_t* __restrict__ temp,
                                                            unsigned long long* __restrict__ ltot,
                                                            uint32_t* __restrict__ defer_count,
                                                            uint32_t* __restrict__ defer_list,
                                                            uint32_t* __restrict__ bg_partials) {
  typedef KeySplitTemp<W, NBITS> KS;
  static_assert(KS::PBITS == PAYLOAD_BITS || BOTH, "the 16-bucket split needs both strands");
  typedef ScatterEmit<KS, NBITS, SCATTER_WPW, uint16_t, KS::G> Emit;
  Emit::init_lds();
  bg_begin<BG>();
  __syncthreads();
  const uint32_t wave = (uint32_t)__builtin_amdgcn_readfirstlane((int)(threadIdx.x >> 6));
  Emit e{keys, slice_cap, slice_fill, temp, wave, threadIdx.x & 63u, blockIdx.x * (uint32_t)SCATTER_WPW + wave, 0u};
  e.bind();
  scan_items<W, BOTH, BG>(words32, items, n_items, ltot, defer_count, defer_list, e);
  e.drain();
  bg_end<BG>(bg_partials);
}

#ifndef PENGK_SCATTER12_WPW
#define PENGK_SCATTER12_WPW 3
#endif
constexpr int SCATTER12_WPW = PENGK_SCATTER12_WPW;
#ifndef PENGK_SCATTER12L1_WPW
#define PENGK_SCATTER12L1_WPW (PENGK_W12_L1_BITS == 5 ? 3 : 4)
#endif
constexpr int SCATTER12L1_WPW = PENGK_SCATTER12L1_WPW;
typedef ScatterEmit<Split12L1, Split12L1::NBITS, SCATTER12L1_WPW, uint32_t> Scatter12Emit;

template <bool BOTH, bool BG>
__global__ __launch_bounds__(64 * SCATTER12L1_WPW) void count_scatter12_kernel(const uint32_t* __restrict__ words32,
                                                              const uint64_t* __restrict__ items, uint32_t n_items,
                                                              uint32_t* __restrict__ keys, uint32_t slice_cap,
                                                              uint32_t* __restrict__ slice_fill, uint32_t* __restrict__ hist,
                                                              unsigned long long* __restrict__ ltot,
                                                              uint32_t* __restrict__ defer, uint32_t* __restrict__ bg_partials) {
  Scatter12Emit::init_lds();
  bg_begin<BG>();
  __syncthreads();
  const uint32_t wave = (uint32_t)__builtin_amdgcn_readfirstlane((int)(threadIdx.x >> 6));
  Scatter12Emit e{keys, slice_cap, slice_fill, hist, wave, threadIdx.x & 63u, blockIdx.x * (uint32_t)SCATTER12L1_WPW + wave, 0u};
  e.bind();
  scan_items<12, BOTH, BG>(words32, items, n_items, ltot, defer, defer + 1, e);
  e.drain();
  bg_end<BG>(bg_partials);
}

__global__ __launch_bounds__(256) void count_rescatter12_kernel(const uint32_t* __restrict__ keys1, uint32_t cap1,
                                                                const uint32_t* __restrict__ fill1, uint32_t n_slices1,
                                                                uint32_t bpb1, uint16_t* __restrict__ keys2, uint32_t cap2,
                                                                uint32_t* __restrict__ fill2, uint32_t* __restrict__ hist) {
  ScatterEmit<Split12L2, Split12L2::NBITS>::init_lds();
  __syncthreads();
  const uint32_t b1 = blockIdx.x / bpb1, j = blockIdx.x % bpb1;
  const uint32_t wave = (uint32_t)__builtin_amdgcn_readfirstlane((int)(threadIdx.x >> 6)), lane = threadIdx.x & 63u;
  ScatterEmit<Split12L2, Split12L2::NBITS> e{keys2, cap2, fill2, hist, wave, lane, blockIdx.x * 4u + wave, b1};
  e.bind();
  const uint32_t per = (n_slices1 + bpb1 - 1) / bpb1;
  const uint32_t first = j * per, last = min(n_slices1, first + per);
  for (uint32_t s = first + wave; s < last; s += 4) {
    const uint32_t n = fill1[(size_t)s * Split12L1::NB + b1];
    const uint32_t* src = keys1 + ((size_t)s * Split12L1::NB + b1) * cap1;
    typedef uint32_t u4 __attribute__((ext_vector_type(4)));
    const u4 pad = {0xFFFFFFFFu, 0xFFFFFFFFu, 0xFFFFFFFFu, 0xFFFFFFFFu};
    const u4* src4 = reinterpret_cast<const u4*>(src);
    const uint32_t n4 = n / 4u;
    u4 nxt = lane < n4 ? __builtin_nontemporal_load(&src4[lane]) : pad;
    for (uint32_t i = 0; i < n4; i += 64) {
      const u4 k = nxt;
      nxt = (i + 64u + lane < n4) ? __builtin_nontemporal_load(&src4[i + 64u + lane]) : pad;
      e.full(k.x);
      e.full(k.y);
      e.full(k.z);
      e.full(k.w);
    }
  }
  e.drain();
}

typedef ScatterEmit<Split14L1, Split14L1::NBITS, SCATTER12L1_WPW, uint32_t> Scatter14Emit;

template <bool BOTH, bool BG>
__global__ __launch_bounds__(64 * SCATTER12L1_WPW) void count_scatter14_kernel(const uint32_t* __restrict__ words32,
                                                              const uint64_t* __restrict__ items, uint32_t n_items,
                                                              uint32_t* __restrict__ keys, uint32_t slice_cap,
                                                              uint32_t* __restrict__ slice_fill, uint32_t* __restrict__ hist,
                                                              unsigned long long* __restrict__ ltot,
                                                              uint32_t* __restrict__ defer, uint32_t* __restrict__ bg_partials) {
  Scatter14Emit::init_lds();
  bg_begin<BG>();
  __syncthreads();
  const uint32_t wave = (uint32_t)__builtin_amdgcn_readfirstlane((int)(threadIdx.x >> 6));
  Scatter14Emit e{keys, slice_cap, slice_fill, hist, wave, threadIdx.x & 63u, blockIdx.x * (uint32_t)SCATTER12L1_WPW + wave, 0u};
  e.bind();
  scan_items<14, BOTH, BG>(words32, items, n_items, ltot, defer, defer + 1, e);
  e.drain();
  bg_end<BG>(bg_partials);
}

template <class KS, class E_OUT, uint32_t NB_IN>
__global__ __launch_bounds__(256) void count_rescatter_kernel(const uint32_t* __restrict__ keys_in, uint32_t cap_in,
                                                              const uint32_t* __restrict__ fill_in, uint32_t n_slices_in,
                                                              uint32_t slices_per_group, uint32_t bpb, E_OUT* __restrict__ keys_out,
                                                              uint32_t cap_out, uint32_t* __restrict__ fill_out,
                                                              uint32_t* __restrict__ hist) {
  typedef ScatterEmit<KS, KS::NBITS, 4, E_OUT> Emit;
  Emit::init_lds();
  __syncthreads();
  const uint32_t o = blockIdx.x / bpb, j = blockIdx.x % bpb;
  const uint32_t b_in = slices_per_group ? o % NB_IN : o;
  const uint32_t slice0 = slices_per_group ? (o / NB_IN) * slices_per_group : 0u;
  const uint32_t n_in = slices_per_group ? slices_per_group : n_slices_in;
  const uint32_t wave = (uint32_t)__builtin_amdgcn_readfirstlane((int)(threadIdx.x >> 6)), lane = threadIdx.x & 63u;
  Emit e{keys_out, cap_out, fill_out, hist, wave, lane, blockIdx.x * 4u + wave, o};
  e.bind();
  const uint32_t per = (n_in + bpb - 1) / bpb;
  const uint32_t first = j * per, last = min(n_in, first + per);
  for (uint32_t t = first + wave; t < last; t += 4) {
    const uint32_t sl = slice0 + t;
    const uint32_t n = fill_in[(size_t)sl * NB_IN + b_in];
    typedef uint32_t u4 __attribute__((ext_vector_type(4)));
    const u4 pad = {0xFFFFFFFFu, 0xFFFFFFFFu, 0xFFFFFFFFu, 0xFFFFFFFFu};
    const u4* src4 = reinterpret_cast<const u4*>(keys_in + ((size_t)sl * NB_IN + b_in) * cap_in);
    const uint32_t n4 = n / 4u;
    u4 nxt = lane < n4 ? __builtin_nontemporal_load(&src4[lane]) : pad;
    for (uint32_t i = 0; i < n4; i += 64) {
      const u4 k = nxt;
      nxt = (i + 64u + lane < n4) ? __builtin_nontemporal_load(&src4[i + 64u + lane]) : pad;
      e.full(k.x);
      e.full(k.y);
      e.full(k.z);
      e.full(k.w);
    }
  }
  e.drain();
}

__global__ __launch_bounds__(256) void count_gather14_kernel(const uint32_t* __restrict__ temp, uint32_t* __restrict__ hist) {
  const uint32_t np = 1u << 28;
  for (uint32_t x = blockIdx.x * blockDim.x + threadIdx.x; x < np; x += gridDim.x * blockDim.x) {
    const uint32_t p1 = Split14L1::payload(x), p2 = Split14L2::payload(p1);
    const uint32_t fb = (Split14L1::bucket(x) * Split14L2::NB + Split14L2::bucket(p1)) * Split14L3::NB + Split14L3::bucket(p2);
    const uint32_t v = temp[((size_t)fb << PAYLOAD_BITS) | Split14L3::payload(p2)];
    if (v) hist[x] += v;
  }
}

__device__ __forceinline__ void hist_block(uint32_t* __restrict__ h, uint32_t block, const uint16_t* __restrict__ keys,
                                           uint32_t slice_cap, uint32_t n_slices, uint32_t nb,
                                           const uint32_t* __restrict__ slice_fill, uint32_t bpb,
                                           uint32_t* __restrict__ temp, uint32_t slices_per_outer) {
  const uint32_t f = block / bpb, j = block % bpb;
  const uint32_t b = slices_per_outer ? f % nb : f;
  const uint32_t slice0 = slices_per_outer ? (f / nb) * slices_per_outer : 0u;
  if (slices_per_outer) n_slices = slices_per_outer;
  for (uint32_t i = threadIdx.x; i < (1u << PAYLOAD_BITS); i += blockDim.x) h[i] = 0;
  __syncthreads();
  const uint32_t per = (n_slices + bpb - 1) / bpb;
  const uint32_t first = slice0 + j * per, last = slice0 + min(n_slices, j * per + per);
  const uint32_t wave = threadIdx.x >> 6, lane = threadIdx.x & 63u;
  uint32_t fill_next = first + wave < last ? slice_fill[(size_t)(first + wave) * nb + b] : 0u;
  for (uint32_t s = first + wave; s < last; s += 16) {
    const uint32_t n8 = fill_next >> 3;
    if (s + 16 < last) fill_next = slice_fill[(size_t)(s + 16) * nb + b];
    const uint4* src = reinterpret_cast<const uint4*>(keys + ((size_t)s * nb + b) * slice_cap);
    auto count8 = [&](const uint4& v) {
      const uint32_t k[8] = {v.x & 0xFFFFu, v.x >> 16, v.y & 0xFFFFu, v.y >> 16, v.z & 0xFFFFu, v.z >> 16, v.w & 0xFFFFu, v.w >> 16};
#pragma unroll
      for (int q = 0; q < 8; ++q)
        if (k[q] < (1u << PAYLOAD_BITS)) atomicAdd(&h[k[q]], 1u);
    };
    uint32_t i = lane;
    for (; i + 448 < n8; i += 512) {
      uint4 v[8];
#pragma unroll
      for (int q = 0; q < 8; ++q) {
        typedef uint32_t u32x4 __attribute__((ext_vector_type(4)));
        const u32x4 t = __builtin_nontemporal_load(reinterpret_cast<const u32x4*>(&src[i + 64 * q]));
        v[q] = make_uint4(t.x, t.y, t.z, t.w);
      }
#pragma unroll
      for (int q = 0; q < 8; ++q) count8(v[q]);
    }
    if (i < n8) {
      uint4 v[7];
#pragma unroll
      for (int q = 0; q < 7; ++q) {
        typedef uint32_t u32x4 __attribute__((ext_vector_type(4)));
        const u32x4 ones = {0xFFFFFFFFu, 0xFFFFFFFFu, 0xFFFFFFFFu, 0xFFFFFFFFu};
        const u32x4 t = i + 64u * q < n8 ? __builtin_nontemporal_load(reinterpret_cast<const u32x4*>(&src[i + 64 * q])) : ones;
        v[q] = make_uint4(t.x, t.y, t.z, t.w);
      }
#pragma unroll
      for (int q = 0; q < 7; ++q) count8(v[q]);
    }
  }
  __syncthreads();
  uint32_t* dst = temp + ((size_t)f << PAYLOAD_BITS);
  for (uint32_t i = threadIdx.x; i < (1u << PAYLOAD_BITS); i += blockDim.x) {
    const uint32_t v = h[i];
    if (v) __hip_atomic_fetch_add(&dst[i], v, __ATOMIC_RELAXED, __HIP_MEMORY_SCOPE_AGENT);
  }
}

__device__ __forceinline__ void hist16_block(uint32_t* __restrict__ h, uint32_t block, const uint16_t* __restrict__ keys,
                                             uint32_t slice_cap, uint32_t n_slices, uint32_t nb,
                                             const uint32_t* __restrict__ slice_fill, uint32_t bpb,
                                             uint32_t* __restrict__ temp, uint32_t* __restrict__ wrapped) {
  __shared__ unsigned long long sums[2];
  const uint32_t b = block / bpb, j = block % bpb;
  for (uint32_t i = threadIdx.x; i < (1u << 15); i += blockDim.x) h[i] = 0;
  if (threadIdx.x < 2) sums[threadIdx.x] = 0;
  __syncthreads();
  const uint32_t per = (n_slices + bpb - 1) / bpb;
  const uint32_t first = j * per, last = min(n_slices, j * per + per);
  const uint32_t wave = threadIdx.x >> 6, lane = threadIdx.x & 63u;
  typedef uint32_t u32x4 __attribute__((ext_vector_type(4)));
  auto add2 = [&](uint32_t x) {
    atomicAdd(&h[x & 0x7FFFu], 1u << ((x >> 11) & 16u));
    atomicAdd(&h[(x >> 16) & 0x7FFFu], 1u << ((x >> 27) & 16u));
  };
  auto count8 = [&](const u32x4& v) {
    add2(v.x);
    add2(v.y);
    add2(v.z);
    add2(v.w);
  };
  unsigned long long n_keys = 0;
  uint32_t fill_next = first + wave < last ? slice_fill[(size_t)(first + wave) * nb + b] : 0u;
  for (uint32_t s = first + wave; s < last; s += 16) {
    const uint32_t fill = fill_next;
    const uint32_t n8 = fill >> 3;
    if (s + 16 < last) fill_next = slice_fill[(size_t)(s + 16) * nb + b];
    n_keys += fill;
    const u32x4* src = reinterpret_cast<const u32x4*>(keys + ((size_t)s * nb + b) * slice_cap);
    uint32_t i = lane;
    for (; i + 448 < n8; i += 512) {
      u32x4 v[8];
#pragma unroll
      for (int q = 0; q < 8; ++q) v[q] = __builtin_nontemporal_load(&src[i + 64 * q]);
#pragma unroll
      for (int q = 0; q < 8; ++q) count8(v[q]);
    }
    const uint32_t part = fill & 7u;
    const bool has_part = part != 0u && lane == 0u;
    u32x4 vp = {0u, 0u, 0u, 0u};
    if (has_part) vp = __builtin_nontemporal_load(&src[n8]);
    if (i < n8) {
      u32x4 v[7];
#pragma unroll
      for (int q = 0; q < 7; ++q) {
        const u32x4 zero = {0u, 0u, 0u, 0u};
        v[q] = i + 64u * q < n8 ? __builtin_nontemporal_load(&src[i + 64 * q]) : zero;
      }
#pragma unroll
      for (int q = 0; q < 7; ++q)
        if (i + 64u * q < n8) count8(v[q]);
    }
    if (has_part) {
      const uint32_t w[4] = {vp.x, vp.y, vp.z, vp.w};
#pragma unroll
      for (uint32_t q = 0; q < 7u; ++q) {
        const uint32_t k = (w[q >> 1] >> (16u * (q & 1u))) & 0xFFFFu;
        if (q < part) atomicAdd(&h[k & 0x7FFFu], 1u << ((k >> 11) & 16u));
      }
    }
  }
  if (lane == 0 && n_keys) atomicAdd(&sums[0], n_keys);
  __syncthreads();
  {
    unsigned long long sum = 0;
    for (uint32_t i = threadIdx.x; i < (1u << 15); i += blockDim.x) {
      const uint32_t v = h[i];
      sum += (v & 0xFFFFu) + (v >> 16);
    }
#pragma unroll
    for (int off = 32; off > 0; off >>= 1) sum += __shfl_down(sum, off, 64);
    if (lane == 0 && sum) atomicAdd(&sums[1], sum);
  }
  __syncthreads();
  uint32_t* dst = temp + ((size_t)b << 16);
  if (sums[0] == sums[1]) {
    for (uint32_t i = threadIdx.x; i < (1u << 15); i += blockDim.x) {
      const uint32_t v = h[i];
      if (v & 0xFFFFu) __hip_atomic_fetch_add(&dst[i], v & 0xFFFFu, __ATOMIC_RELAXED, __HIP_MEMORY_SCOPE_AGENT);
      if (v >> 16) __hip_atomic_fetch_add(&dst[0x8000u | i], v >> 16, __ATOMIC_RELAXED, __HIP_MEMORY_SCOPE_AGENT);
    }
    return;
  }
  if (threadIdx.x == 0) __hip_atomic_fetch_add(wrapped, 1u, __ATOMIC_RELAXED, __HIP_MEMORY_SCOPE_AGENT);
  for (uint32_t s = first + wave; s < last; s += 16) {
    const uint32_t fill = slice_fill[(size_t)s * nb + b];
    const uint16_t* src = keys + ((size_t)s * nb + b) * slice_cap;
    for (uint32_t i = lane; i < fill; i += 64)
      __hip_atomic_fetch_add(&dst[src[i]], 1u, __ATOMIC_RELAXED, __HIP_MEMORY_SCOPE_AGENT);
  }
}

__global__ __launch_bounds__(1024) void count_hist_kernel(const uint16_t* __restrict__ keys, uint32_t slice_cap,
                                                          uint32_t n_slices, uint32_t nb,
                                                          const uint32_t* __restrict__ slice_fill, uint32_t bpb,
                                                          uint32_t* __restrict__ temp, uint32_t slices_per_outer) {
  extern __shared__ __attribute__((aligned(16))) uint32_t h[];
  hist_block(h, blockIdx.x, keys, slice_cap, n_slices, nb, slice_fill, bpb, temp, slices_per_outer);
}

__global__ __launch_bounds__(256) void count_gather12_kernel(const uint32_t* __restrict__ temp, uint32_t* __restrict__ hist) {
  const uint32_t np = 1u << 24;
  for (uint32_t x = blockIdx.x * blockDim.x + threadIdx.x; x < np; x += gridDim.x * blockDim.x) {
    const uint32_t p1 = Split12L1::payload(x);
    const uint32_t fb = Split12L1::bucket(x) * Split12L2::NB + Split12L2::bucket(p1);
    const uint32_t v = temp[((size_t)fb << PAYLOAD_BITS) | Split12L2::payload(p1)];
    if (v) hist[x] += v;
  }
}

template <int W, int NBITS>
__global__ __launch_bounds__(256) void count_gather_kernel(const uint32_t* __restrict__ temp, uint32_t np,
                                                           uint32_t* __restrict__ hist,
                                                           const unsigned long long* __restrict__ ltot_acc,
                                                           unsigned long long* __restrict__ ltot) {
  using KS = KeySplitTemp<W, NBITS>;
  if (blockIdx.x == 0 && threadIdx.x == 0) *ltot = *ltot_acc;
  for (uint32_t x = blockIdx.x * blockDim.x + threadIdx.x; x < np; x += gridDim.x * blockDim.x) {
    uint32_t v = temp[KS::index(x)];
    if (KS::PBITS == 16 && x == np - 1u) v = 0;
    hist[x] = v;
  }
}

__device__ __forceinline__ uint32_t base_at(const uint32_t* __restrict__ words32, uint64_t g) {
  return (words32[g >> 4] >> (2u * (uint32_t)(g & 15u))) & 3u;
}

template <class Ring, class Add>
__device__ __forceinline__ void fixup_items(const uint32_t* __restrict__ words32, const uint64_t* __restrict__ items, int W,
                                            int both, uint32_t n, const uint32_t* __restrict__ list, uint32_t first,
                                            uint32_t stride, Ring ring, Add add) {
  const uint32_t mask = (1u << (2 * W)) - 1u;
  const int top = 2 * (W - 1);
  for (uint32_t q = first; q < n; q += stride) {
    const uint32_t it = list[q];
    const uint64_t rec = items[it];
    const uint32_t nw = (uint32_t)((rec >> ITEM_NW_SHIFT) & ITEM_NW_MASK);
    const uint64_t ws = rec & ITEM_WS_MASK;
    uint32_t j = it;
    while ((items[j] >> ITEM_CONT_SHIFT) & 1ull) --j;
    const uint64_t head = items[j] & ITEM_WS_MASK;
    uint64_t back = 8ull * (uint64_t)(W - 1);
    for (;;) {
      const uint64_t p0 = (ws - head > back) ? ws - back : head;
      bool certified = (p0 == head);
      for (int i = 0; i < 16; ++i) ring(i) = INVALID_ID;
      uint32_t id = 0, rc = 0;
      for (int b = 0; b < W - 1; ++b) {
        const uint32_t c = base_at(words32, p0 + b);
        id = (id >> 2) | (c << top);
        rc = ((rc << 2) & mask) | (c ^ 3u);
      }
      uint32_t clean = 0;
      bool ok = true;
      for (uint64_t t = p0; t < ws + nw; ++t) {
        const uint32_t c = base_at(words32, t + (uint64_t)(W - 1));
        id = (id >> 2) | (c << top);
        rc = ((rc << 2) & mask) | (c ^ 3u);
        const uint32_t can = both ? min(id, rc) : id;
        bool match = false;
        for (int d = 1; d <= W - 1; ++d) match |= (ring((uint32_t)(t - d) & 15u) == can);
        if (t < ws) {
          clean = match ? 0u : clean + 1u;
          if (clean >= 2u * (uint32_t)(W - 1)) certified = true;
        } else {
          if (!certified) {
            ok = false;
            break;
          }
          if (!match) add(can);
        }
        ring((uint32_t)t & 15u) = match ? INVALID_ID : can;
      }
      if (ok) break;
      back *= 4ull;
    }
  }
}

__global__ __launch_bounds__(64) void count_fixup_kernel(const uint32_t* __restrict__ words32,
                                                         const uint64_t* __restrict__ items, int W, int both,
                                                         uint32_t* __restrict__ hist,
                                                         const uint32_t* __restrict__ defer) {
  uint32_t r[16];
  fixup_items(words32, items, W, both, defer[0], defer + 1, blockIdx.x * blockDim.x + threadIdx.x, gridDim.x * blockDim.x,
              [&](uint32_t i) -> uint32_t& { return r[i]; },
              [&](uint32_t id) { __hip_atomic_fetch_add(&hist[id], 1u, __ATOMIC_RELAXED, __HIP_MEMORY_SCOPE_AGENT); });
}

__global__ __launch_bounds__(256) void mirror_kernel(uint32_t* __restrict__ hist, int W, uint32_t np) {
  for (uint32_t x = blockIdx.x * blockDim.x + threadIdx.x; x < np; x += gridDim.x * blockDim.x) {
    const uint32_t r = revcomp32(x, W);
    if (x > r) hist[x] = hist[r];
  }
}

__global__ __launch_bounds__(256) void bg_count_kernel(const uint32_t* __restrict__ words32,
                                                       const uint64_t* __restrict__ items, uint32_t n_items, int W,
                                                       unsigned long long* __restrict__ out ) {
  __shared__ uint32_t h3[64][65];
  __shared__ uint32_t hfirst[20];
  for (int i = threadIdx.x; i < 64 * 65; i += blockDim.x) (&h3[0][0])[i] = 0;
  if (threadIdx.x < 20) hfirst[threadIdx.x] = 0;
  __syncthreads();
  const uint32_t col = threadIdx.x & 63u;
  for (uint32_t it = blockIdx.x * blockDim.x + threadIdx.x; it < n_items; it += gridDim.x * blockDim.x) {
    const uint64_t rec = items[it];
    const uint32_t nw = (uint32_t)((rec >> ITEM_NW_SHIFT) & ITEM_NW_MASK);
    const uint64_t ws = rec & ITEM_WS_MASK;
    const bool cont = ((rec >> ITEM_CONT_SHIFT) & 1ull) != 0;
    const bool last = (it + 1 == n_items) || (((items[it + 1] >> ITEM_CONT_SHIFT) & 1ull) == 0);
    const uint32_t nb = nw + (last ? (uint32_t)(W - 1) : 0u);
    uint32_t y = 0;
    uint32_t pos = 2;
    if (cont) {
      const uint64_t prev = items[it - 1];
      const bool second = ((prev >> ITEM_CONT_SHIFT) & 1ull) == 0 && ((prev >> ITEM_NW_SHIFT) & ITEM_NW_MASK) == 1;
      if (second) {
        y = base_at(words32, ws - 1);
        pos = 1;
      } else {
        y = (base_at(words32, ws - 2) << 2) | base_at(words32, ws - 1);
      }
    } else {
      pos = 0;
    }
    for (uint32_t b = 0; b < nb; ++b) {
      const uint32_t c = base_at(words32, ws + b);
      y = ((y << 2) | c) & 63u;
      if (pos >= 2) {
        atomicAdd(&h3[y][col], 1u);
      } else if (pos == 1) {
        atomicAdd(&hfirst[4 + (y & 15u)], 1u);
        pos = 2;
      } else {
        atomicAdd(&hfirst[c], 1u);
        pos = 1;
      }
    }
  }
  __syncthreads();
  if (threadIdx.x < 64) {
    unsigned long long s = 0;
    for (int i = 0; i < 64; ++i) s += h3[threadIdx.x][i];
    if (s) atomicAdd(&out[threadIdx.x], s);
  } else if (threadIdx.x < 84) {
    const uint32_t v = hfirst[threadIdx.x - 64];
    if (v) atomicAdd(&out[threadIdx.x], (unsigned long long)v);
  }
}

__global__ void bg_finish_kernel(const unsigned long long* __restrict__ raw, unsigned long long* __restrict__ out) {
  const int t = threadIdx.x;
  __shared__ unsigned long long n2[16];
  if (t < 16) {
    unsigned long long s = raw[64 + 4 + t];
    for (int c = 0; c < 4; ++c) s += raw[c * 16 + t];
    n2[t] = s;
    out[4 + t] = s;
  }
  __syncthreads();
  if (t < 4) {
    unsigned long long s = raw[64 + t];
    for (int b = 0; b < 4; ++b) s += n2[b * 4 + t];
    out[t] = s;
  }
  if (t < 64) out[20 + t] = raw[t];
}

constexpr uint32_t BG_FINISH_LDS = 84 + 64 + 16 + 12 * 84;
__device__ __forceinline__ void bg_finish_block(unsigned long long* __restrict__ lds, const uint32_t* __restrict__ partials,
                                                uint32_t n_blocks, unsigned long long* __restrict__ out) {
  unsigned long long* raw = lds;
  unsigned long long* n3 = raw + 84;
  unsigned long long* n2 = n3 + 64;
  unsigned long long(*part)[84] = reinterpret_cast<unsigned long long(*)[84]>(n2 + 16);
  const int t = threadIdx.x;
  {
    const int bin = t % 84, strand = t / 84;
    if (strand < 12) {
      unsigned long long acc[8] = {0, 0, 0, 0, 0, 0, 0, 0};
      uint32_t b = strand;
      for (; b + 31u * 12u < n_blocks; b += 32u * 12u) {
        uint32_t v[32];
#pragma unroll
        for (uint32_t j = 0; j < 32u; ++j) v[j] = partials[(size_t)(b + 12u * j) * 84 + bin];
#pragma unroll
        for (uint32_t j = 0; j < 32u; ++j) acc[j & 7u] += v[j];
      }
      for (; b < n_blocks; b += 12) acc[0] += partials[(size_t)b * 84 + bin];
      part[strand][bin] = ((acc[0] + acc[1]) + (acc[2] + acc[3])) + ((acc[4] + acc[5]) + (acc[6] + acc[7]));
    }
  }
  __syncthreads();
  if (t < 84) {
    unsigned long long s = 0;
    for (int k = 0; k < 12; ++k) s += part[k][t];
    raw[t] = s;
  }
  __syncthreads();
  if (t < 64) {
    const int d0 = t >> 4, d1 = (t >> 2) & 3, d2 = t & 3;
    n3[t] = raw[d0 | (d1 << 2) | (d2 << 4)];
    out[20 + t] = n3[t];
  }
  __syncthreads();
  if (t < 16) {
    const int a = t >> 2, b = t & 3;
    unsigned long long s = raw[68 + (a | (b << 2))];
    for (int c = 0; c < 4; ++c) s += n3[c * 16 + t];
    n2[t] = s;
    out[4 + t] = s;
  }
  __syncthreads();
  if (t < 4) {
    unsigned long long s = raw[64 + t];
    for (int b = 0; b < 4; ++b) s += n2[b * 4 + t];
    out[t] = s;
  }
}

__global__ __launch_bounds__(1024) void bg_finish_fused_kernel(const uint32_t* __restrict__ partials, uint32_t n_blocks,
                                                               unsigned long long* __restrict__ out) {
  __shared__ unsigned long long lds[BG_FINISH_LDS];
  bg_finish_block(lds, partials, n_blocks, out);
}

template <int W, int NBITS>
__global__ __launch_bounds__(1024) void count_hist_front_kernel(const uint16_t* __restrict__ keys, uint32_t slice_cap,
                                                                uint32_t n_slices, const uint32_t* __restrict__ slice_fill,
                                                                uint32_t bpb, uint32_t* __restrict__ temp,
                                                                const uint32_t* __restrict__ bg_partials, uint32_t bg_blocks,
                                                                unsigned long long* __restrict__ bg_out,
                                                                const uint32_t* __restrict__ words32,
                                                                const uint64_t* __restrict__ items, int both,
                                                                const uint32_t* __restrict__ defer_count,
                                                                const uint32_t* __restrict__ defer_list, uint32_t n_fix,
                                                                uint32_t* __restrict__ wrapped) {
  extern __shared__ __attribute__((aligned(16))) uint32_t h[];
  if (blockIdx.x == 0) {
    if (bg_out) bg_finish_block(reinterpret_cast<unsigned long long*>(h), bg_partials, bg_blocks, bg_out);
    return;
  }
  if (blockIdx.x <= n_fix) {
    uint32_t* r = h + threadIdx.x;
    fixup_items(words32, items, W, both, defer_count[0], defer_list, (blockIdx.x - 1u) * blockDim.x + threadIdx.x,
                n_fix * blockDim.x, [&](uint32_t i) -> uint32_t& { return r[i * 1024u]; },
                [&](uint32_t id) {
                  __hip_atomic_fetch_add(&temp[KeySplitTemp<W, NBITS>::index(id)], 1u, __ATOMIC_RELAXED, __HIP_MEMORY_SCOPE_AGENT);
                });
    return;
  }
  if constexpr (KeySplitTemp<W, NBITS>::PBITS == 16)
    hist16_block(h, blockIdx.x - 1u - n_fix, keys, slice_cap, n_slices, 1u << NBITS, slice_fill, bpb, temp, wrapped);
  else
    hist_block(h, blockIdx.x - 1u - n_fix, keys, slice_cap, n_slices, 1u << NBITS, slice_fill, bpb, temp, 0u);
}

__global__ __launch_bounds__(128) void bg_model_kernel(const unsigned long long* __restrict__ n, int K, float a0, float a1, float a2,
                                                       float* __restrict__ V) {
  __shared__ float cnt[84];
  __shared__ float v[84];
  const int t = threadIdx.x;
  const float alpha[3] = {a0, a1, a2};
  const int off[3] = {0, 4, 20};
  if (t < 84) cnt[t] = (float)n[t];
  __shared__ float base_f;
  if (t == 0) {
    unsigned long long base_counts = 0;
    for (int y = 0; y < 4; ++y) base_counts += n[y];
    base_f = (float)base_counts;
  }
  __syncthreads();
  if (t < 4) v[t] = (cnt[t] + alpha[0] * 0.25f) / (base_f + alpha[0]);
  __syncthreads();
  for (int k = 1; k <= K; ++k) {
    const int ny = 1 << (2 * (k + 1));
    const int yk = 1 << (2 * k);
    if (t < ny) v[off[k] + t] = (cnt[off[k] + t] + alpha[k] * v[off[k - 1] + t % yk]) / (cnt[off[k - 1] + t / 4] + alpha[k]);
    __syncthreads();
    if (t < ny / 4) {
      float* g = v + off[k] + 4 * t;
      float factor = 0.0f;
      for (int a = 0; a < 4; ++a) factor += g[a];
      for (int a = 0; a < 4; ++a) g[a] /= factor;
    }
    __syncthreads();
  }
  const int used = off[K] + (1 << (2 * (K + 1)));
  if (t < 84) V[t] = t < used ? v[t] : 0.0f;
}

__device__ __forceinline__ uint64_t mix64(uint64_t x) {
  x ^= x >> 30;
  x *= 0xBF58476D1CE4E5B9ull;
  x ^= x >> 27;
  x *= 0x94D049BB133111EBull;
  x ^= x >> 31;
  return x;
}

__global__ __launch_bounds__(256) void synth_words_kernel(uint64_t seed, uint64_t seq0, uint64_t n_seq, uint32_t L,
                                                          uint64_t* __restrict__ words, uint64_t n_words) {
  const uint64_t motif = 2ull | (1ull << 2) | (3ull << 4) | (2ull << 6) | (0ull << 8) | (2ull << 10) | (3ull << 12) |
                         (1ull << 14) | (0ull << 16) | (3ull << 18);
  const uint64_t total = n_seq * (uint64_t)L;
  for (uint64_t w = blockIdx.x * (uint64_t)blockDim.x + threadIdx.x; w < n_words; w += (uint64_t)gridDim.x * blockDim.x) {
    uint64_t v = 0;
    for (int k = 0; k < 32; ++k) {
      const uint64_t g = w * 32 + k;
      if (g < PENGK_FRONT_PAD_BASES) continue;
      const uint64_t li = g - PENGK_FRONT_PAD_BASES;
      if (li >= total) break;
      const uint64_t n = seq0 + li / L;
      const uint32_t j = (uint32_t)(li % L);
      uint64_t d = mix64(seed + 0x9E3779B97F4A7C15ull * (n * (uint64_t)L + j + 1)) >> 62;
      if (L >= 10 && mix64(seed ^ 0xA5A5A5A5ull ^ (n + 1)) % 10 == 0) {
        const uint64_t q = mix64(seed ^ 0x5A5A5A5Aull ^ (n + 1)) % (L - 9);
        if (j >= q && j < q + 10) d = (motif >> (2 * (j - q))) & 3ull;
      }
      v |= d << (2 * k);
    }
    words[w] = v;
  }
}

__global__ __launch_bounds__(256) void synth_items_kernel(uint64_t n_seq, uint32_t L, int W, uint32_t M,
                                                          uint64_t* __restrict__ items) {
  const uint64_t nwin = (uint64_t)L - W + 1;
  const uint64_t per = (nwin + M - 1) / M;
  const uint64_t n = n_seq * per;
  for (uint64_t i = blockIdx.x * (uint64_t)blockDim.x + threadIdx.x; i < n; i += (uint64_t)gridDim.x * blockDim.x) {
    const uint64_t s = i / per;
    const uint64_t f = (i % per) * M;
    const uint64_t nw = nwin - f < M ? nwin - f : M;
    items[i] = (PENGK_FRONT_PAD_BASES + s * L + f) | (nw << ITEM_NW_SHIFT) | ((uint64_t)(f ? 1 : 0) << ITEM_CONT_SHIFT);
  }
}

#define PENGK_LAUNCH_BB(KERNEL, TARGS, both, bg, grid, block, ...)                                              \
  do {                                                                                                         \
    if (both) {                                                                                                \
      if (bg) hipLaunchKernelGGL((KERNEL<TARGS(true, true)>), grid, block, 0, ctx->stream, __VA_ARGS__);        \
      else hipLaunchKernelGGL((KERNEL<TARGS(true, false)>), grid, block, 0, ctx->stream, __VA_ARGS__);          \
    } else {                                                                                                   \
      if (bg) hipLaunchKernelGGL((KERNEL<TARGS(false, true)>), grid, block, 0, ctx->stream, __VA_ARGS__);       \
      else hipLaunchKernelGGL((KERNEL<TARGS(false, false)>), grid, block, 0, ctx->stream, __VA_ARGS__);         \
    }                                                                                                          \
  } while (0)

int bg_partials_buffer(pengk_ctx* ctx, uint32_t blocks, uint32_t** out) {
  int rc = ensure_scratch(ctx, &ctx->d_bg_partials, &ctx->bg_partials_bytes, (size_t)blocks * 84 * sizeof(uint32_t));
  *out = (uint32_t*)ctx->d_bg_partials;
  return rc;
}

int bg_finish_fused(pengk_ctx* ctx, uint32_t blocks, uint64_t* d_bg) {
  hipLaunchKernelGGL(bg_finish_fused_kernel, dim3(1), dim3(1024), 0, ctx->stream, (const uint32_t*)ctx->d_bg_partials, blocks,
                     (unsigned long long*)d_bg);
  PENGK_HIP(hipGetLastError());
  return PENGK_OK;
}

template <int W>
int launch_direct_w(pengk_ctx* ctx, int both, uint32_t* d_counts, uint64_t* d_ltot, uint32_t n_items, uint64_t* d_bg) {
  const uint32_t* w32 = (const uint32_t*)ctx->d_words;
  const uint32_t blocks_needed = (n_items + 255) / 256;
  const uint32_t max_blocks = (uint32_t)ctx->num_cu * 8u;
  const uint32_t blocks = blocks_needed < max_blocks ? blocks_needed : max_blocks;
  unsigned long long* lt = (unsigned long long*)d_ltot;
  uint32_t* bgp = nullptr;
  if (d_bg) {
    int rc = bg_partials_buffer(ctx, blocks, &bgp);
    if (rc) return rc;
  }
#define TA_DIRECT(B, G) W, B, G
  PENGK_LAUNCH_BB(count_kernel, TA_DIRECT, both, d_bg != nullptr, dim3(blocks), dim3(256), w32, ctx->d_items, n_items, d_counts,
                  lt, ctx->d_defer, bgp);
#undef TA_DIRECT
  PENGK_HIP(hipGetLastError());
  return d_bg ? bg_finish_fused(ctx, blocks, d_bg) : PENGK_OK;
}

template <int W, int NBITS = 2 * W - PAYLOAD_BITS>
int launch_partition_w(pengk_ctx* ctx, int both, uint32_t* d_counts, uint64_t* d_ltot, uint32_t n_items, uint64_t* d_bg) {
  typedef KeySplitTemp<W, NBITS> KS;
  constexpr uint32_t GRP = (uint32_t)KS::G;
  constexpr uint32_t NB = 1u << NBITS;
  const uint32_t np = 1u << (2 * W);
  const uint32_t* w32 = (const uint32_t*)ctx->d_words;
  constexpr uint32_t TPB = 64u * SCATTER_WPW;
  const uint32_t blocks_needed = (n_items + TPB - 1) / TPB;
  constexpr uint32_t lds_per_wg = (uint32_t)(sizeof(ScatterShared<NBITS, SCATTER_WPW, uint16_t, 2 * KS::G>) + sizeof(BgLds) + 511u) & ~511u;
  const uint32_t per_cu = ctx->scatter_blocks_per_cu ? (uint32_t)ctx->scatter_blocks_per_cu : (160u * 1024u) / lds_per_wg;
  const uint32_t max_blocks = (uint32_t)ctx->num_cu * per_cu;
  const uint32_t blocks = blocks_needed < max_blocks ? blocks_needed : max_blocks;
  const uint32_t n_waves = blocks * (uint32_t)SCATTER_WPW;
  uint64_t windows = ctx->n_windows_hint ? ctx->n_windows_hint : ctx->n_items * (uint64_t)ctx->item_windows;
  const uint64_t share = windows / ((uint64_t)NB * n_waves);
  uint64_t cap64 = share + share / 2 + 512;
  if (ctx->key_cap_override) cap64 = ctx->key_cap_override;
  cap64 = (cap64 + GRP - 1) / GRP * GRP;
  if (cap64 * NB >= (1ull << 31))
    return fail(PENGK_ERR_RANGE, "shard too large for the partitioned count (slice of %llu keys)", (unsigned long long)cap64);
  const uint32_t slice_cap = (uint32_t)cap64;
  int rc = ensure_scratch(ctx, &ctx->d_keys, &ctx->keys_bytes, (size_t)NB * n_waves * slice_cap * sizeof(uint16_t));
  if (rc) return rc;
  const size_t fill_words = ((size_t)NB * n_waves + 63) / 64 * 64;
  constexpr size_t HEAD_WORDS = 4;
  const size_t aux_need = (fill_words + HEAD_WORDS + (size_t)np) * sizeof(uint32_t);
  rc = ensure_scratch(ctx, &ctx->d_count_aux, &ctx->count_aux_bytes, aux_need);
  if (rc) return rc;
  uint32_t* slice_fill = (uint32_t*)ctx->d_count_aux;
  unsigned long long* ltot_acc = (unsigned long long*)(slice_fill + fill_words);
  uint32_t* defer_count = slice_fill + fill_words + 2;
  uint32_t* temp = slice_fill + fill_words + HEAD_WORDS;
  PENGK_HIP(hipMemsetAsync(ltot_acc, 0, (HEAD_WORDS + (size_t)np) * sizeof(uint32_t), ctx->stream));
  ctx->d_defer_count = defer_count;
  uint32_t* wrapped = slice_fill + fill_words + 3;
  ctx->d_wrap_count = wrapped;
  ctx->d_slice_fill = slice_fill;
  ctx->n_slice_fill = (uint64_t)NB * n_waves;
  ctx->count_group_used = (int)GRP;
  uint16_t* keys = (uint16_t*)ctx->d_keys;
  uint32_t* bgp = nullptr;
  if (d_bg) {
    rc = bg_partials_buffer(ctx, blocks, &bgp);
    if (rc) return rc;
  }
  if constexpr (KS::PBITS == 16) {
    if (d_bg)
      hipLaunchKernelGGL((count_scatter_kernel<W, true, NBITS, true>), dim3(blocks), dim3(TPB), 0, ctx->stream, w32, ctx->d_items,
                         n_items, keys, slice_cap, slice_fill, temp, ltot_acc, defer_count, ctx->d_defer + 1, bgp);
    else
      hipLaunchKernelGGL((count_scatter_kernel<W, true, NBITS, false>), dim3(blocks), dim3(TPB), 0, ctx->stream, w32, ctx->d_items,
                         n_items, keys, slice_cap, slice_fill, temp, ltot_acc, defer_count, ctx->d_defer + 1, bgp);
  } else {
#define TA_SCATTER(B, BG) W, B, NBITS, BG
    PENGK_LAUNCH_BB(count_scatter_kernel, TA_SCATTER, both, d_bg != nullptr, dim3(blocks), dim3(TPB), w32, ctx->d_items, n_items,
                    keys, slice_cap, slice_fill, temp, ltot_acc, defer_count, ctx->d_defer + 1, bgp);
#undef TA_SCATTER
  }
  PENGK_HIP(hipGetLastError());
  uint32_t bpb = ((uint32_t)ctx->num_cu * 2u + NB - 1) / NB;
  const uint64_t per_bucket = windows / NB + 1;
  const uint32_t useful = (uint32_t)((per_bucket + 65535) / 65536);
  if (bpb > useful) bpb = useful;
  if (bpb > n_waves) bpb = n_waves;
  if (bpb < 1) bpb = 1;
  constexpr uint32_t N_FIX = 4;
  hipLaunchKernelGGL((count_hist_front_kernel<W, NBITS>), dim3(1u + N_FIX + NB * bpb), dim3(1024), 4 << PAYLOAD_BITS, ctx->stream,
                     keys, slice_cap, n_waves, slice_fill, bpb, temp, bgp, blocks, (unsigned long long*)d_bg, w32, ctx->d_items, both,
                     defer_count, ctx->d_defer + 1, N_FIX, wrapped);
  PENGK_HIP(hipGetLastError());
  const uint32_t gb = (np + 255) / 256 < 2048u ? (np + 255) / 256 : 2048u;
  hipLaunchKernelGGL((count_gather_kernel<W, NBITS>), dim3(gb), dim3(256), 0, ctx->stream, temp, np, d_counts, ltot_acc,
                     (unsigned long long*)d_ltot);
  PENGK_HIP(hipGetLastError());
  return PENGK_OK;
}

int launch_partition12(pengk_ctx* ctx, int both, uint32_t* d_counts, uint64_t* d_ltot, uint32_t n_items, uint64_t* d_bg) {
  const uint32_t np = 1u << 24;
  const uint32_t* w32 = (const uint32_t*)ctx->d_words;
  constexpr uint32_t TPB1 = 64u * SCATTER12L1_WPW;
  constexpr uint32_t NB1 = Split12L1::NB, NB2 = Split12L2::NB;
  const uint32_t blocks_needed = (n_items + TPB1 - 1) / TPB1;
  constexpr uint32_t lds_per_wg1 = (uint32_t)(sizeof(ScatterShared<Split12L1::NBITS, SCATTER12L1_WPW, uint32_t>) + sizeof(BgLds) + 511u) & ~511u;
  const uint32_t max_blocks = (uint32_t)ctx->num_cu * ((160u * 1024u) / lds_per_wg1);
  const uint32_t blocks1 = blocks_needed < max_blocks ? blocks_needed : max_blocks;
  const uint32_t n_waves1 = blocks1 * (uint32_t)SCATTER12L1_WPW;
  const uint64_t windows = ctx->n_windows_hint ? ctx->n_windows_hint : ctx->n_items * (uint64_t)ctx->item_windows;
  uint64_t share1 = windows / ((uint64_t)NB1 * n_waves1);
  uint64_t cap1_64 = share1 + share1 / 2 + 256;
  if (ctx->key_cap_override) cap1_64 = ctx->key_cap_override;
  cap1_64 = (cap1_64 + 63) / 64 * 64;
  uint32_t bpb1 = ((uint32_t)ctx->num_cu * 8u + NB1 - 1u) / NB1;
  if (bpb1 > n_waves1) bpb1 = n_waves1;
  if (bpb1 < 1) bpb1 = 1;
  const uint32_t blocks2 = NB1 * bpb1;
  const uint32_t n_waves2 = blocks2 * 4u;
  uint64_t share2 = windows / ((uint64_t)NB2 * n_waves2);
  uint64_t cap2_64 = share2 + share2 / 2 + 512;
  if (ctx->key_cap_override) cap2_64 = ctx->key_cap_override;
  cap2_64 = (cap2_64 + 63) / 64 * 64;
  if (cap1_64 * NB1 >= (1ull << 30) || cap2_64 * NB2 >= (1ull << 31)) return fail(
      PENGK_ERR_RANGE, "shard too large for the partitioned count");
  const uint32_t cap1 = (uint32_t)cap1_64, cap2 = (uint32_t)cap2_64;
  const size_t bytes1 = (size_t)n_waves1 * NB1 * cap1 * sizeof(uint32_t);
  const size_t bytes2 = (size_t)n_waves2 * NB2 * cap2 * sizeof(uint16_t);
  int rc = ensure_scratch(ctx, &ctx->d_keys, &ctx->keys_bytes, bytes1 + bytes2);
  if (rc) return rc;
  uint32_t* keys1 = (uint32_t*)ctx->d_keys;
  uint16_t* keys2 = (uint16_t*)((char*)ctx->d_keys + bytes1);
  const size_t fill1_words = ((size_t)n_waves1 * NB1 + 63) / 64 * 64, fill2_words = ((size_t)n_waves2 * NB2 + 63) / 64 * 64;
  const size_t aux_need = (fill1_words + fill2_words + (size_t)np) * sizeof(uint32_t);
  rc = ensure_scratch(ctx, &ctx->d_count_aux, &ctx->count_aux_bytes, aux_need);
  if (rc) return rc;
  uint32_t* fill1 = (uint32_t*)ctx->d_count_aux;
  uint32_t* fill2 = fill1 + fill1_words;
  uint32_t* temp = fill2 + fill2_words;
  PENGK_HIP(hipMemsetAsync(ctx->d_count_aux, 0, aux_need, ctx->stream));
  unsigned long long* lt = (unsigned long long*)d_ltot;
  uint32_t* bgp = nullptr;
  if (d_bg) {
    rc = bg_partials_buffer(ctx, blocks1, &bgp);
    if (rc) return rc;
  }
#define TA_S12(B, G) B, G
  PENGK_LAUNCH_BB(count_scatter12_kernel, TA_S12, both, d_bg != nullptr, dim3(blocks1), dim3(TPB1), w32, ctx->d_items, n_items, keys1,
                  cap1, fill1, d_counts, lt, ctx->d_defer, bgp);
#undef TA_S12
  PENGK_HIP(hipGetLastError());
  if (d_bg) {
    rc = bg_finish_fused(ctx, blocks1, d_bg);
    if (rc) return rc;
  }
  hipLaunchKernelGGL(count_rescatter12_kernel, dim3(blocks2), dim3(256), 0, ctx->stream, keys1, cap1, fill1, n_waves1, bpb1, keys2,
                     cap2, fill2, d_counts);
  PENGK_HIP(hipGetLastError());
  hipLaunchKernelGGL(count_hist_kernel, dim3(512), dim3(1024), 4 << PAYLOAD_BITS, ctx->stream, keys2, cap2, n_waves2, NB2, fill2, 1u,
                     temp, bpb1 * 4u);
  PENGK_HIP(hipGetLastError());
  hipLaunchKernelGGL(count_gather12_kernel, dim3(4096), dim3(256), 0, ctx->stream, temp, d_counts);
  PENGK_HIP(hipGetLastError());
  return PENGK_OK;
}

int launch_partition14(pengk_ctx* ctx, int both, uint32_t* d_counts, uint64_t* d_ltot, uint32_t n_items, uint64_t* d_bg) {
  const size_t np = (size_t)1 << 28;
  const uint32_t* w32 = (const uint32_t*)ctx->d_words;
  constexpr uint32_t TPB1 = 64u * SCATTER12L1_WPW;
  constexpr uint32_t NB1 = Split14L1::NB, NB2 = Split14L2::NB, NB3 = Split14L3::NB;
  static_assert(NB1 * NB2 * NB3 == 8192, "2^13 LDS histograms");
  const uint32_t blocks_needed = (n_items + TPB1 - 1) / TPB1;
  constexpr uint32_t lds_per_wg1 = (uint32_t)(sizeof(ScatterShared<Split14L1::NBITS, SCATTER12L1_WPW, uint32_t>) + sizeof(BgLds) + 511u) & ~511u;
  const uint32_t max_blocks = (uint32_t)ctx->num_cu * ((160u * 1024u) / lds_per_wg1);
  const uint32_t blocks1 = blocks_needed < max_blocks ? blocks_needed : max_blocks;
  const uint32_t n_waves1 = blocks1 * (uint32_t)SCATTER12L1_WPW;
  const uint64_t windows = ctx->n_windows_hint ? ctx->n_windows_hint : ctx->n_items * (uint64_t)ctx->item_windows;
  auto cap_of = [&](uint64_t slices, uint64_t slack) {
    uint64_t c = windows / slices;
    c = c + c / 2 + slack;
    if (ctx->key_cap_override) c = ctx->key_cap_override;
    return (c + 63) / 64 * 64;
  };
  uint32_t bpb1 = ((uint32_t)ctx->num_cu * 8u + NB1 - 1u) / NB1;
  if (bpb1 > n_waves1) bpb1 = n_waves1;
  if (bpb1 < 1) bpb1 = 1;
  const uint32_t blocks2 = NB1 * bpb1, n_waves2 = blocks2 * 4u;
  uint32_t bpb2 = ((uint32_t)ctx->num_cu * 8u + NB1 * NB2 - 1u) / (NB1 * NB2);
  if (bpb2 > bpb1 * 4u) bpb2 = bpb1 * 4u;
  if (bpb2 < 1) bpb2 = 1;
  const uint32_t blocks3 = NB1 * NB2 * bpb2, n_waves3 = blocks3 * 4u;
  const uint64_t cap1_64 = cap_of((uint64_t)NB1 * n_waves1, 256), cap2_64 = cap_of((uint64_t)NB2 * n_waves2, 256), cap3_64 = cap_of((uint64_t)NB3 * n_waves3, 256);
  if (cap1_64 * NB1 >= (1ull << 30) || cap2_64 * NB2 >= (1ull << 30) || cap3_64 * NB3 >= (1ull << 31))
    return fail(PENGK_ERR_RANGE, "shard too large for the partitioned count");
  const uint32_t cap1 = (uint32_t)cap1_64, cap2 = (uint32_t)cap2_64, cap3 = (uint32_t)cap3_64;
  const size_t bytes1 = (size_t)n_waves1 * NB1 * cap1 * sizeof(uint32_t);
  const size_t bytes2 = (size_t)n_waves2 * NB2 * cap2 * sizeof(uint32_t);
  const size_t bytes3 = (size_t)n_waves3 * NB3 * cap3 * sizeof(uint16_t);
  int rc = ensure_scratch(ctx, &ctx->d_keys, &ctx->keys_bytes, bytes1 + bytes2 + bytes3);
  if (rc) return rc;
  uint32_t* keys1 = (uint32_t*)ctx->d_keys;
  uint32_t* keys2 = (uint32_t*)((char*)ctx->d_keys + bytes1);
  uint16_t* keys3 = (uint16_t*)((char*)ctx->d_keys + bytes1 + bytes2);
  const size_t f1 = ((size_t)n_waves1 * NB1 + 63) / 64 * 64, f2 = ((size_t)n_waves2 * NB2 + 63) / 64 * 64,
               f3 = ((size_t)n_waves3 * NB3 + 63) / 64 * 64;
  const size_t aux_need = (f1 + f2 + f3 + np) * sizeof(uint32_t);
  rc = ensure_scratch(ctx, &ctx->d_count_aux, &ctx->count_aux_bytes, aux_need);
  if (rc) return rc;
  uint32_t* fill1 = (uint32_t*)ctx->d_count_aux;
  uint32_t* fill2 = fill1 + f1;
  uint32_t* fill3 = fill2 + f2;
  uint32_t* temp = fill3 + f3;
  PENGK_HIP(hipMemsetAsync(ctx->d_count_aux, 0, aux_need, ctx->stream));
  unsigned long long* lt = (unsigned long long*)d_ltot;
  uint32_t* bgp = nullptr;
  if (d_bg) {
    rc = bg_partials_buffer(ctx, blocks1, &bgp);
    if (rc) return rc;
  }
#define TA_S14(B, G) B, G
  PENGK_LAUNCH_BB(count_scatter14_kernel, TA_S14, both, d_bg != nullptr, dim3(blocks1), dim3(TPB1), w32, ctx->d_items, n_items, keys1,
                  cap1, fill1, d_counts, lt, ctx->d_defer, bgp);
#undef TA_S14
  PENGK_HIP(hipGetLastError());
  if (d_bg) {
    rc = bg_finish_fused(ctx, blocks1, d_bg);
    if (rc) return rc;
  }
  hipLaunchKernelGGL((count_rescatter_kernel<Split14L2, uint32_t, NB1>), dim3(blocks2), dim3(256), 0, ctx->stream, keys1, cap1, fill1,
                     n_waves1, 0u, bpb1, keys2, cap2, fill2, d_counts);
  PENGK_HIP(hipGetLastError());
  hipLaunchKernelGGL((count_rescatter_kernel<Split14L3, uint16_t, NB2>), dim3(blocks3), dim3(256), 0, ctx->stream, keys2, cap2, fill2,
                     n_waves2, bpb1 * 4u, bpb2, keys3, cap3, fill3, d_counts);
  PENGK_HIP(hipGetLastError());
  hipLaunchKernelGGL(count_hist_kernel, dim3(8192), dim3(1024), 4 << PAYLOAD_BITS, ctx->stream, keys3, cap3, n_waves3, NB3, fill3, 1u,
                     temp, bpb2 * 4u);
  PENGK_HIP(hipGetLastError());
  hipLaunchKernelGGL(count_gather14_kernel, dim3(8192), dim3(256), 0, ctx->stream, temp, d_counts);
  PENGK_HIP(hipGetLastError());
  return PENGK_OK;
}

template <int W>
int launch_count_w(pengk_ctx* ctx, int both, uint32_t* d_counts, uint64_t* d_ltot, uint64_t* d_bg) {
  const uint32_t n_items = (uint32_t)ctx->n_items;
  if (n_items == 0) {
    if (d_bg) PENGK_HIP(hipMemsetAsync(d_bg, 0, 84 * sizeof(uint64_t), ctx->stream));
    return PENGK_OK;
  }
  if constexpr (W < 4) {
    if (d_bg) {
      const int rc_bg = launch_bg_count(ctx, d_bg);
      if (rc_bg) return rc_bg;
      d_bg = nullptr;
    }
  }
  int impl = ctx->count_impl;
  constexpr bool can_partition = (W == 8 || W == 10 || W == 12 || W == 14);
  if (impl == 0) impl = can_partition ? 2 : 1;
  if (impl == 2 && !can_partition) return fail(PENGK_ERR_UNSUPPORTED, "partitioned count is built for W = 8 .. 14 only");
  const bool can_group128 = W == 10 && both && impl == 2;
  if (ctx->count_group == 128 && !can_group128)
    return fail(PENGK_ERR_UNSUPPORTED, "count_group 128 is built for the partitioned count at W = 10 on both strands only (W = %d, %s, count_impl %d)",
                W, both ? "both strands" : "one strand", impl);
  if constexpr (W == 10) {
    if (can_group128 && ctx->count_group != 64) return launch_partition_w<10, 4>(ctx, both, d_counts, d_ltot, n_items, d_bg);
  }
  int rc;
  if constexpr (W == 14) {
    rc = impl == 2 ? launch_partition14(ctx, both, d_counts, d_ltot, n_items, d_bg)
                   : launch_direct_w<W>(ctx, both, d_counts, d_ltot, n_items, d_bg);
  } else if constexpr (W == 12) {
    rc = impl == 2 ? launch_partition12(ctx, both, d_counts, d_ltot, n_items, d_bg)
                   : launch_direct_w<W>(ctx, both, d_counts, d_ltot, n_items, d_bg);
  } else if constexpr (can_partition) {
    if (impl == 2) return launch_partition_w<W>(ctx, both, d_counts, d_ltot, n_items, d_bg);
    rc = launch_direct_w<W>(ctx, both, d_counts, d_ltot, n_items, d_bg);
  } else {
    rc = launch_direct_w<W>(ctx, both, d_counts, d_ltot, n_items, d_bg);
  }
  if (rc) return rc;
  hipLaunchKernelGGL(count_fixup_kernel, dim3(64), dim3(64), 0, ctx->stream, (const uint32_t*)ctx->d_words, ctx->d_items, W,
                     both, d_counts, ctx->d_defer);
  PENGK_HIP(hipGetLastError());
  return PENGK_OK;
}

}

int count_init_device() {
  PENGK_HIP(hipFuncSetAttribute((const void*)count_hist_kernel, hipFuncAttributeMaxDynamicSharedMemorySize, 4 << PAYLOAD_BITS));
  PENGK_HIP(hipFuncSetAttribute((const void*)count_hist_front_kernel<8, 16 - PAYLOAD_BITS>, hipFuncAttributeMaxDynamicSharedMemorySize, 4 << PAYLOAD_BITS));
  PENGK_HIP(hipFuncSetAttribute((const void*)count_hist_front_kernel<10, 20 - PAYLOAD_BITS>, hipFuncAttributeMaxDynamicSharedMemorySize, 4 << PAYLOAD_BITS));
  PENGK_HIP(hipFuncSetAttribute((const void*)count_hist_front_kernel<10, 4>, hipFuncAttributeMaxDynamicSharedMemorySize, 4 << PAYLOAD_BITS));
  return PENGK_OK;
}

int launch_count(pengk_ctx* ctx, int both, uint32_t* d_counts, uint64_t* d_ltot, uint64_t* d_bg) {
  const int W = ctx->W;
  const size_t np = (size_t)1 << (2 * W);
  {
    const size_t need = (ctx->n_items + 2) * sizeof(uint32_t);
    size_t have = ctx->defer_cap * sizeof(uint32_t);
    if (have < need) {
      int rc = ensure_scratch(ctx, (void**)&ctx->d_defer, &have, need);
      if (rc) return rc;
      ctx->defer_cap = have / sizeof(uint32_t);
    }
  }
  const bool one_level = (W == 8 || W == 10) && ctx->count_impl != 1 && ctx->n_items > 0;
  ctx->d_wrap_count = nullptr;
  ctx->d_slice_fill = nullptr;
  ctx->count_group_used = 0;
  if (!one_level) {
    ctx->d_defer_count = ctx->d_defer;
    PENGK_HIP(hipMemsetAsync(ctx->d_defer, 0, sizeof(uint32_t), ctx->stream));
    PENGK_HIP(hipMemsetAsync(d_counts, 0, np * sizeof(uint32_t), ctx->stream));
    PENGK_HIP(hipMemsetAsync(d_ltot, 0, sizeof(uint64_t), ctx->stream));
  }
  switch (W) {
    case 2: return launch_count_w<2>(ctx, both, d_counts, d_ltot, d_bg);
    case 4: return launch_count_w<4>(ctx, both, d_counts, d_ltot, d_bg);
    case 6: return launch_count_w<6>(ctx, both, d_counts, d_ltot, d_bg);
    case 8: return launch_count_w<8>(ctx, both, d_counts, d_ltot, d_bg);
    case 10: return launch_count_w<10>(ctx, both, d_counts, d_ltot, d_bg);
    case 12: return launch_count_w<12>(ctx, both, d_counts, d_ltot, d_bg);
    case 14: return launch_count_w<14>(ctx, both, d_counts, d_ltot, d_bg);
    default: return fail(PENGK_ERR_ARG, "pattern length %d unsupported", W);
  }
}

int launch_mirror(pengk_ctx* ctx, int W, uint32_t* d_counts) {
  const uint32_t np = 1u << (2 * W);
  const uint32_t blocks = (np + 255) / 256 < 4096u ? (np + 255) / 256 : 4096u;
  hipLaunchKernelGGL(mirror_kernel, dim3(blocks), dim3(256), 0, ctx->stream, d_counts, W, np);
  PENGK_HIP(hipGetLastError());
  return PENGK_OK;
}

int launch_bg_count(pengk_ctx* ctx, uint64_t* d_bg) {
  int rc = ensure_scratch(ctx, &ctx->d_misc, &ctx->misc_bytes, 84 * sizeof(uint64_t));
  if (rc) return rc;
  unsigned long long* raw = (unsigned long long*)ctx->d_misc;
  PENGK_HIP(hipMemsetAsync(raw, 0, 84 * sizeof(uint64_t), ctx->stream));
  const uint32_t n_items = (uint32_t)ctx->n_items;
  if (n_items) {
    const uint32_t need = (n_items + 255) / 256;
    const uint32_t blocks = need < (uint32_t)ctx->num_cu * 4u ? need : (uint32_t)ctx->num_cu * 4u;
    hipLaunchKernelGGL(bg_count_kernel, dim3(blocks), dim3(256), 0, ctx->stream, (const uint32_t*)ctx->d_words,
                       ctx->d_items, n_items, ctx->W, raw);
    PENGK_HIP(hipGetLastError());
  }
  hipLaunchKernelGGL(bg_finish_kernel, dim3(1), dim3(64), 0, ctx->stream, raw, (unsigned long long*)d_bg);
  PENGK_HIP(hipGetLastError());
  return PENGK_OK;
}

int launch_bg_model(pengk_ctx* ctx, const uint64_t* d_bg, int K, const float* h_alpha, float* d_V) {
  hipLaunchKernelGGL(bg_model_kernel, dim3(1), dim3(128), 0, ctx->stream, (const unsigned long long*)d_bg, K, h_alpha[0],
                     h_alpha[1], h_alpha[2], d_V);
  PENGK_HIP(hipGetLastError());
  return PENGK_OK;
}

int launch_synth(pengk_ctx* ctx, uint64_t seed, uint64_t seq0, uint64_t n_seq, uint32_t L, int W, int item_windows,
                 uint64_t* d_words, uint64_t* d_items) {
  uint64_t nw = 0, ni = 0;
  int rc = pengk_synth_sizes(n_seq, L, W, item_windows, &nw, &ni);
  if (rc) return rc;
  hipLaunchKernelGGL(synth_words_kernel, dim3(4096), dim3(256), 0, ctx->stream, seed, seq0, n_seq, L, d_words, nw);
  PENGK_HIP(hipGetLastError());
  if (ni) {
    hipLaunchKernelGGL(synth_items_kernel, dim3(2048), dim3(256), 0, ctx->stream, n_seq, L, W, (uint32_t)item_windows, d_items);
    PENGK_HIP(hipGetLastError());
  }
  return PENGK_OK;
}

}
```

### peng-motif_amd/csrc/pengk_internal.h

```cpp
#pragma once
#include <hip/hip_runtime.h>
#include <stdint.h>

#include "pengk.h"

struct pengk_ctx {
  int device = 0;
  hipStream_t stream = nullptr;
  bool own_stream = false;
  int num_cu = 256;
  const uint64_t* d_words = nullptr;
  uint64_t n_words = 0;
  const uint64_t* d_items = nullptr;
  uint64_t n_items = 0;
  int W = 0;
  int item_windows = 0;
  uint64_t max_bin_bound = 0;
  int all_whole = 0;
  uint32_t* d_defer = nullptr;
  uint64_t defer_cap = 0;
  const uint32_t* d_defer_count = nullptr;
  double* d_em_partials = nullptr;
  size_t em_partials_bytes = 0;
  float* d_em_tables = nullptr;
  size_t em_tables_bytes = 0;
  void* d_em_blocks = nullptr;
  size_t em_blocks_bytes = 0;
  void* d_pair_mids = nullptr;
  size_t pair_mids_bytes = 0;
  int pair_mids_W = 0;
  void* d_em_look = nullptr;
  size_t em_look_bytes = 0;
  uint32_t em_epoch = 0;
  int em_test_lookback = 0;
  unsigned long long* d_em_counters = nullptr;
  hipStream_t em_streams[3] = {nullptr, nullptr, nullptr};
  hipEvent_t em_fork = nullptr, em_join[3] = {nullptr, nullptr, nullptr};
  void* d_misc = nullptr;
  size_t misc_bytes = 0;
  void* d_bg_partials = nullptr;
  size_t bg_partials_bytes = 0;
  void* d_iupac_big = nullptr;
  size_t iupac_big_bytes = 0;
  void* d_keys = nullptr;
  size_t keys_bytes = 0;
  void* d_count_aux = nullptr;
  size_t count_aux_bytes = 0;
  uint64_t n_windows_hint = 0;
  uint64_t key_cap_override = 0;
  uint64_t iupac_group_bytes = 0;
  uint64_t em_table_budget_mb = 0;
  int em_test_skew = 0;
  int em_overlap = 2;
  int em_serial_scan = 2;
  int em_head_blocks = 1;
  int sweep_pairs = 1;
  int em_lean_div = 1;
  int em_fast = 2;
  int count_impl = 0;
  int count_group = 0;
  int count_group_used = 0;
  const uint32_t* d_wrap_count = nullptr;
  const uint32_t* d_slice_fill = nullptr;
  uint64_t n_slice_fill = 0;
  uint64_t count_probe_slice = 0;
  int scatter_blocks_per_cu = 0;
  void* d_sim = nullptr;
  size_t sim_bytes = 0;
  void* d_score = nullptr;
  size_t score_bytes = 0;
  void* d_sites = nullptr;
  size_t sites_bytes = 0;
  uint64_t sites_record_budget = 1ull << 24;
  void* comm = nullptr;
  int comm_transport = 0;
  int comm_rank = 0, comm_world = 1;
};

enum { PENGK_TRANSPORT_NONE = 0, PENGK_TRANSPORT_RCCL = 1, PENGK_TRANSPORT_TCP = 2 };

namespace pengk {

int fail(int code, const char* fmt, ...);
int hip_fail(hipError_t e, const char* what);
int ensure_scratch(pengk_ctx* ctx, void** slot, size_t* have, size_t need);
int enter(pengk_ctx* ctx);
int count_init_device();
int warm_stats();
int warm_iupac();
int warm_similarity();
int warm_em();
void comm_release(pengk_ctx* ctx);

#define PENGK_HIP(call)                                   \
  do {                                                    \
    hipError_t e_ = (call);                               \
    if (e_ != hipSuccess) return ::pengk::hip_fail(e_, #call); \
  } while (0)

inline bool valid_w(int W) { return W >= PENGK_MIN_W && W <= PENGK_MAX_W && (W % 2) == 0; }

constexpr int MAX_EM_LANES = 4;

constexpr uint64_t ITEM_WS_MASK = (1ull << 40) - 1;
constexpr int ITEM_NW_SHIFT = 40;
constexpr uint64_t ITEM_NW_MASK = 0xFFFF;
constexpr int ITEM_CONT_SHIFT = 56;

__host__ __device__ inline uint32_t revcomp32(uint32_t id, int W) {
  uint32_t v = ~id;
#if defined(__HIP_DEVICE_COMPILE__)
  v = __brev(v);
#else
  v = ((v >> 1) & 0x55555555u) | ((v & 0x55555555u) << 1);
  v = ((v >> 2) & 0x33333333u) | ((v & 0x33333333u) << 2);
  v = ((v >> 4) & 0x0F0F0F0Fu) | ((v & 0x0F0F0F0Fu) << 4);
  v = ((v >> 8) & 0x00FF00FFu) | ((v & 0x00FF00FFu) << 8);
  v = (v >> 16) | (v << 16);
#endif
  v = ((v & 0xAAAAAAAAu) >> 1) | ((v & 0x55555555u) << 1);
  return v >> (32 - 2 * W);
}

int launch_count(pengk_ctx* ctx, int both, uint32_t* d_counts, uint64_t* d_ltot, uint64_t* d_bg );
int launch_mirror(pengk_ctx* ctx, int W, uint32_t* d_counts);
int launch_bg_count(pengk_ctx* ctx, uint64_t* d_bg);
int launch_bg_model(pengk_ctx* ctx, const uint64_t* d_bg, int K, const float* h_alpha, float* d_V);
int launch_synth(pengk_ctx* ctx, uint64_t seed, uint64_t seq0, uint64_t n_seq, uint32_t L, int W, int item_windows,
                 uint64_t* d_words, uint64_t* d_items);
int launch_stats(pengk_ctx* ctx, int W, int both, int k, int max_k, const float* d_V, const uint64_t* d_ltot,
                 const uint32_t* d_counts, float* d_bgprob, float* d_expected, float* d_logp, float* d_z);
int launch_seed_candidates(pengk_ctx* ctx, int W, const float* d_z, const uint32_t* d_counts, float z_threshold,
                           uint64_t count_threshold, uint32_t cap, uint32_t* d_n, uint32_t* d_ids, float* d_zs);
int launch_sequential_sum(pengk_ctx* ctx, const float* d_terms, uint64_t n_chains, uint64_t chain_len, float* d_out);
int launch_similarity(pengk_ctx* ctx, int n, const float* d_pwm, const float* d_comp, const int32_t* d_len,
                      const uint64_t* d_sites, int both, const float* h_bg, int first_new, float* d_out);
int launch_iupac(pengk_ctx* ctx, int W, int both, const uint64_t* h_ids, int64_t n, const uint32_t* d_counts,
                 const float* d_bgp, const float* d_expected, pengk_iupac_stats* h_out);
int launch_em(pengk_ctx* ctx, int W, int64_t n_pwm, float* d_pwms, float saturation, float threshold, int max_it,
              const uint32_t* d_counts, const float* d_bg, int32_t* d_state, float* d_change);

}
```

Before: 588.8.

## Add top-bits bucket split for W=10 partitioned k-mer count

Adds a second key-split mode for the W=10 partitioned count that buckets k-mer ids by their top 4 bits with a 16-bit payload and groups of 128. The histogram-front kernel gets a matching per-CU workgroup map, and slice capacity is sized for the uneven bucket loads that result. The mode is chosen automatically for large inputs, so each histogram workgroup covers a contiguous id range and the gather step needs no index remapping. It also lets the suppression chain restore the full exec mask directly, adds an overflow counter, and exposes a test hook for the map. The risk is that skewed top-bit buckets overflow their slices or leave workgroups unevenly loaded.

```diff
diff --git a/include/pengk.h b/include/pengk.h
--- a/include/pengk.h
+++ b/include/pengk.h
@@ -126,6 +126,9 @@
              int max_iterations, const uint32_t* d_counts, const float* d_bg, int* h_iters, float* h_change);
 
 int pengk_test_em_generation(pengk_ctx* ctx, int generation);
+
+int pengk_test_count_top_map(int num_cu, uint32_t n_slices, uint64_t windows, uint32_t* n_workgroups, uint32_t* bucket,
+                             uint32_t* first, uint32_t* last);
 
 int pengk_em_device(pengk_ctx* ctx, int W, int64_t n_pwm, float* d_pwms, float saturation, float threshold,
                     int max_iterations, const uint32_t* d_counts, const float* d_bg, int32_t* d_state,
diff --git a/peng-motif_amd/__init__.py b/peng-motif_amd/__init__.py
--- a/peng-motif_amd/__init__.py
+++ b/peng-motif_amd/__init__.py
@@ -17,7 +17,7 @@
     "pengk_memset", "pengk_warmup", "pengk_host_alloc", "pengk_host_free", "pengk_timer_create", "pengk_timer_record", "pengk_timer_elapsed_ms", "pengk_timer_destroy",
     "pengk_pack", "pengk_pack_threads", "pengk_pack_append", "pengk_packed_free", "pengk_set_sequences", "pengk_synth_sizes", "pengk_synth_sequences",
     "pengk_count", "pengk_count_bg", "pengk_mirror_counts", "pengk_bg_count", "pengk_bg_model", "pengk_pattern_stats",
-    "pengk_seed_candidates", "pengk_iupac_aggregate", "pengk_em", "pengk_em_device", "pengk_test_em_generation", "pengk_sequential_sum_f32", "pengk_motif_similarity", "pengk_selftest_division",
+    "pengk_seed_candidates", "pengk_iupac_aggregate", "pengk_em", "pengk_em_device", "pengk_test_em_generation", "pengk_test_count_top_map", "pengk_sequential_sum_f32", "pengk_motif_similarity", "pengk_selftest_division",
     "pengk_comm_unique_id", "pengk_comm_init", "pengk_comm_init_env", "pengk_comm_info", "pengk_comm_init_abandoned", "pengk_comm_rccl_version", "pengk_comm_destroy",
     "pengk_allreduce_tables", "pengk_comm_check_bin_bound", "pengk_allgather",
     "pengk_comm_host_init_env", "pengk_comm_host_info", "pengk_comm_host_allgather", "pengk_comm_host_allreduce_u64",
@@ -121,6 +121,7 @@
         L.pengk_em.argtypes = [vp, C.c_int, i64, vp, f32, f32, C.c_int, vp, vp, vp, vp]
         L.pengk_em_device.argtypes = [vp, C.c_int, i64, vp, f32, f32, C.c_int, vp, vp, vp, vp]
         L.pengk_test_em_generation.argtypes = [vp, C.c_int]
+        L.pengk_test_count_top_map.argtypes = [C.c_int, C.c_uint32, u64, vp, vp, vp, vp]
         L.pengk_sequential_sum_f32.argtypes = [vp, vp, u64, u64, vp]
         L.pengk_selftest_division.argtypes = [vp, u64, C.c_uint32, vp]
         L.pengk_motif_similarity.argtypes = [vp, C.c_int, vp, vp, vp, vp, C.c_int, vp, C.c_int, vp]
@@ -405,6 +406,14 @@
     def test_em_generation(self, generation):
         _check(lib().pengk_test_em_generation(self.h, int(generation)))
 
+    @staticmethod
+    def count_top_map(num_cu, n_slices, windows):
+        n = C.c_uint32()
+        _check(lib().pengk_test_count_top_map(num_cu, n_slices, windows, C.byref(n), None, None, None))
+        out = [np.zeros(n.value, np.uint32) for _ in range(3)]
+        _check(lib().pengk_test_count_top_map(num_cu, n_slices, windows, C.byref(n), *(a.ctypes.data for a in out)))
+        return out
+
     def info(self, name):
         v = C.c_int64()
         _check(lib().pengk_get_info(self.h, name.encode(), C.byref(v)))
diff --git a/peng-motif_amd/csrc/api.hip b/peng-motif_amd/csrc/api.hip
--- a/peng-motif_amd/csrc/api.hip
+++ b/peng-motif_amd/csrc/api.hip
@@ -171,6 +171,11 @@
     ctx->count_group = (int)value;
     return PENGK_OK;
   }
+  if (strcmp(name, "count_split") == 0) {
+    if (value < 0 || value > 2) return fail(PENGK_ERR_ARG, "count_split must be 0 (auto), 1 (bucket = middle bits of the id) or 2 (top bits)");
+    ctx->count_split = (int)value;
+    return PENGK_OK;
+  }
   if (strcmp(name, "count_probe_slice") == 0) {
     if (value < 0) return fail(PENGK_ERR_ARG, "count_probe_slice must be >= 0 (wave * buckets + bucket)");
     ctx->count_probe_slice = (uint64_t)value;
@@ -266,8 +271,25 @@
     *value = n;
     return PENGK_OK;
   }
+  if (strcmp(name, "count_overflowed_groups") == 0) {
+    uint32_t n = 0;
+    if (ctx->d_overflow_count) {
+      PENGK_HIP(hipMemcpyAsync(&n, ctx->d_overflow_count, sizeof n, hipMemcpyDeviceToHost, ctx->stream));
+      PENGK_HIP(hipStreamSynchronize(ctx->stream));
+    }
+    *value = n;
+    return PENGK_OK;
+  }
   if (strcmp(name, "count_group") == 0) {
     *value = ctx->count_group;
+    return PENGK_OK;
+  }
+  if (strcmp(name, "count_split") == 0) {
+    *value = ctx->count_split;
+    return PENGK_OK;
+  }
+  if (strcmp(name, "count_split_used") == 0) {
+    *value = ctx->count_split_used;
     return PENGK_OK;
   }
   if (strcmp(name, "count_group_used") == 0) {
@@ -602,6 +624,12 @@
   return launch_sequential_sum(ctx, d_terms, n_chains, chain_len, d_out);
 }
 
+int pengk_test_count_top_map(int num_cu, uint32_t n_slices, uint64_t windows, uint32_t* n_workgroups, uint32_t* bucket,
+                             uint32_t* first, uint32_t* last) {
+  if (num_cu < 1 || n_slices < 1 || !n_workgroups) return fail(PENGK_ERR_ARG, "pengk_test_count_top_map: num_cu, n_slices >= 1, n_workgroups not NULL");
+  return count_top_map(num_cu, n_slices, windows, n_workgroups, bucket, first, last);
+}
+
 int pengk_test_em_generation(pengk_ctx* ctx, int generation) {
   if (!ctx) return fail(PENGK_ERR_ARG, "pengk_test_em_generation: NULL context");
   if (generation < 0 || generation > 3) return fail(PENGK_ERR_ARG, "pengk_test_em_generation: 0 (dependent additions), 1 (scan), 2 / 3 (the library's scheme)");
diff --git a/peng-motif_amd/csrc/count.hip b/peng-motif_amd/csrc/count.hip
--- a/peng-motif_amd/csrc/count.hip
+++ b/peng-motif_amd/csrc/count.hip
@@ -78,49 +78,59 @@
 
 template <int W>
 struct Suppress {
-  static __device__ __forceinline__ uint32_t apply(uint32_t can, const uint32_t (&ring)[16], int u) {
-    uint32_t out = INVALID_ID;
+  template <bool EXEC_ALL = false>
+  static __device__ __forceinline__ uint32_t apply(uint32_t can, const uint32_t (&ring)[16], int u, uint32_t mark = INVALID_ID) {
+    uint32_t out = mark;
     unsigned long long save;
 #define PENGK_R(d) "v"(ring[(u - (d)) & 15])
 #define PENGK_CX(n) "v_cmpx_ne_u32_e32 %2, %" #n "\n\t"
-#define PENGK_HEAD "s_mov_b64 %1, exec\n\t"
-#define PENGK_TAIL "v_mov_b32_e32 %0, %2\n\ts_mov_b64 exec, %1"
-    if constexpr (W == 2)
-      asm volatile(PENGK_HEAD PENGK_CX(3) PENGK_TAIL : "+v"(out), "=&s"(save) : "v"(can), PENGK_R(1) : "vcc");
-    else if constexpr (W == 4)
-      asm volatile(PENGK_HEAD PENGK_CX(3) PENGK_CX(4) PENGK_CX(5) PENGK_TAIL
-                   : "+v"(out), "=&s"(save) : "v"(can), PENGK_R(1), PENGK_R(2), PENGK_R(3) : "vcc");
-    else if constexpr (W == 6)
-      asm volatile(PENGK_HEAD PENGK_CX(3) PENGK_CX(4) PENGK_CX(5) PENGK_CX(6) PENGK_CX(7) PENGK_TAIL
-                   : "+v"(out), "=&s"(save) : "v"(can), PENGK_R(1), PENGK_R(2), PENGK_R(3), PENGK_R(4), PENGK_R(5) : "vcc");
-    else if constexpr (W == 8)
-      asm volatile(PENGK_HEAD PENGK_CX(3) PENGK_CX(4) PENGK_CX(5) PENGK_CX(6) PENGK_CX(7) PENGK_CX(8) PENGK_CX(9) PENGK_TAIL
-                   : "+v"(out), "=&s"(save)
-                   : "v"(can), PENGK_R(1), PENGK_R(2), PENGK_R(3), PENGK_R(4), PENGK_R(5), PENGK_R(6), PENGK_R(7) : "vcc");
-    else if constexpr (W == 10)
-      asm volatile(PENGK_HEAD PENGK_CX(3) PENGK_CX(4) PENGK_CX(5) PENGK_CX(6) PENGK_CX(7) PENGK_CX(8) PENGK_CX(9) PENGK_CX(10)
-                   PENGK_CX(11) PENGK_TAIL
-                   : "+v"(out), "=&s"(save)
-                   : "v"(can), PENGK_R(1), PENGK_R(2), PENGK_R(3), PENGK_R(4), PENGK_R(5), PENGK_R(6), PENGK_R(7), PENGK_R(8),
-                     PENGK_R(9) : "vcc");
-    else if constexpr (W == 12)
-      asm volatile(PENGK_HEAD PENGK_CX(3) PENGK_CX(4) PENGK_CX(5) PENGK_CX(6) PENGK_CX(7) PENGK_CX(8) PENGK_CX(9) PENGK_CX(10)
-                   PENGK_CX(11) PENGK_CX(12) PENGK_CX(13) PENGK_TAIL
-                   : "+v"(out), "=&s"(save)
-                   : "v"(can), PENGK_R(1), PENGK_R(2), PENGK_R(3), PENGK_R(4), PENGK_R(5), PENGK_R(6), PENGK_R(7), PENGK_R(8),
-                     PENGK_R(9), PENGK_R(10), PENGK_R(11) : "vcc");
-    else {
-      static_assert(W == 14, "pattern lengths 2 .. 14");
-      asm volatile(PENGK_HEAD PENGK_CX(3) PENGK_CX(4) PENGK_CX(5) PENGK_CX(6) PENGK_CX(7) PENGK_CX(8) PENGK_CX(9) PENGK_CX(10)
-                   PENGK_CX(11) PENGK_CX(12) PENGK_CX(13) PENGK_CX(14) PENGK_CX(15) PENGK_TAIL
-                   : "+v"(out), "=&s"(save)
-                   : "v"(can), PENGK_R(1), PENGK_R(2), PENGK_R(3), PENGK_R(4), PENGK_R(5), PENGK_R(6), PENGK_R(7), PENGK_R(8),
-                     PENGK_R(9), PENGK_R(10), PENGK_R(11), PENGK_R(12), PENGK_R(13) : "vcc");
-    }
+#define PENGK_SAVE "s_mov_b64 %1, exec\n\t"
+#define PENGK_RESTORE "v_mov_b32_e32 %0, %2\n\ts_mov_b64 exec, %1"
+#define PENGK_RESTORE_ALL "v_mov_b32_e32 %0, %2\n\ts_mov_b64 exec, -1"
+#define PENGK_CHAIN(HEAD, TAIL)                                                                                                \
+  if constexpr (W == 2)                                                                                                        \
+    asm volatile(HEAD PENGK_CX(3) TAIL : "+v"(out), "=&s"(save) : "v"(can), PENGK_R(1) : "vcc");                               \
+  else if constexpr (W == 4)                                                                                                   \
+    asm volatile(HEAD PENGK_CX(3) PENGK_CX(4) PENGK_CX(5) TAIL                                                                 \
+                 : "+v"(out), "=&s"(save) : "v"(can), PENGK_R(1), PENGK_R(2), PENGK_R(3) : "vcc");                             \
+  else if constexpr (W == 6)                                                                                                   \
+    asm volatile(HEAD PENGK_CX(3) PENGK_CX(4) PENGK_CX(5) PENGK_CX(6) PENGK_CX(7) TAIL                                         \
+                 : "+v"(out), "=&s"(save) : "v"(can), PENGK_R(1), PENGK_R(2), PENGK_R(3), PENGK_R(4), PENGK_R(5) : "vcc");     \
+  else if constexpr (W == 8)                                                                                                   \
+    asm volatile(HEAD PENGK_CX(3) PENGK_CX(4) PENGK_CX(5) PENGK_CX(6) PENGK_CX(7) PENGK_CX(8) PENGK_CX(9) TAIL                 \
+                 : "+v"(out), "=&s"(save)                                                                                      \
+                 : "v"(can), PENGK_R(1), PENGK_R(2), PENGK_R(3), PENGK_R(4), PENGK_R(5), PENGK_R(6), PENGK_R(7) : "vcc");      \
+  else if constexpr (W == 10)                                                                                                  \
+    asm volatile(HEAD PENGK_CX(3) PENGK_CX(4) PENGK_CX(5) PENGK_CX(6) PENGK_CX(7) PENGK_CX(8) PENGK_CX(9) PENGK_CX(10)         \
+                 PENGK_CX(11) TAIL                                                                                             \
+                 : "+v"(out), "=&s"(save)                                                                                      \
+                 : "v"(can), PENGK_R(1), PENGK_R(2), PENGK_R(3), PENGK_R(4), PENGK_R(5), PENGK_R(6), PENGK_R(7), PENGK_R(8),   \
+                   PENGK_R(9) : "vcc");                                                                                        \
+  else if constexpr (W == 12)                                                                                                  \
+    asm volatile(HEAD PENGK_CX(3) PENGK_CX(4) PENGK_CX(5) PENGK_CX(6) PENGK_CX(7) PENGK_CX(8) PENGK_CX(9) PENGK_CX(10)         \
+                 PENGK_CX(11) PENGK_CX(12) PENGK_CX(13) TAIL                                                                   \
+                 : "+v"(out), "=&s"(save)                                                                                      \
+                 : "v"(can), PENGK_R(1), PENGK_R(2), PENGK_R(3), PENGK_R(4), PENGK_R(5), PENGK_R(6), PENGK_R(7), PENGK_R(8),   \
+                   PENGK_R(9), PENGK_R(10), PENGK_R(11) : "vcc");                                                              \
+  else {                                                                                                                       \
+    static_assert(W == 14, "pattern lengths 2 .. 14");                                                                         \
+    asm volatile(HEAD PENGK_CX(3) PENGK_CX(4) PENGK_CX(5) PENGK_CX(6) PENGK_CX(7) PENGK_CX(8) PENGK_CX(9) PENGK_CX(10)         \
+                 PENGK_CX(11) PENGK_CX(12) PENGK_CX(13) PENGK_CX(14) PENGK_CX(15) TAIL                                         \
+                 : "+v"(out), "=&s"(save)                                                                                      \
+                 : "v"(can), PENGK_R(1), PENGK_R(2), PENGK_R(3), PENGK_R(4), PENGK_R(5), PENGK_R(6), PENGK_R(7), PENGK_R(8),   \
+                   PENGK_R(9), PENGK_R(10), PENGK_R(11), PENGK_R(12), PENGK_R(13) : "vcc");                                    \
+  }
+    if constexpr (EXEC_ALL) {
+      PENGK_CHAIN("", PENGK_RESTORE_ALL)
+    } else {
+      PENGK_CHAIN(PENGK_SAVE, PENGK_RESTORE)
+    }
+#undef PENGK_CHAIN
 #undef PENGK_R
 #undef PENGK_CX
-#undef PENGK_HEAD
-#undef PENGK_TAIL
+#undef PENGK_SAVE
+#undef PENGK_RESTORE
+#undef PENGK_RESTORE_ALL
     return out;
   }
 };
@@ -256,7 +266,7 @@
 #ifdef PENGK_ABLATE_NOSUPPRESS
             const uint32_t key = can;
 #else
-            const uint32_t key = Suppress<W>::apply(can, ring, u);
+            const uint32_t key = Suppress<W>::template apply<FULL>(can, ring, u, Emit::SUPPRESSED);
 #endif
             ring[u] = key;
             if (FULL) {
@@ -270,7 +280,7 @@
               emit.full(key);
             } else {
               bgc.kmer3(id_u, t0 + (uint32_t)u < nw_all);
-              emit.masked(key, key != INVALID_ID && t0 + (uint32_t)u < nw);
+              emit.masked(key, key != Emit::SUPPRESSED && t0 + (uint32_t)u < nw);
             }
           }
         }
@@ -293,6 +303,7 @@
 }
 
 struct DirectEmit {
+  static constexpr uint32_t SUPPRESSED = INVALID_ID;
   uint32_t* __restrict__ hist;
   __device__ __forceinline__ void masked(uint32_t key, bool active) const {
     if (active) __hip_atomic_fetch_add(&hist[key], 1u, __ATOMIC_RELAXED, __HIP_MEMORY_SCOPE_AGENT);
@@ -409,9 +420,19 @@
   return sh;
 }
 
+template <class KS, class = void>
+struct SuppressedKey {
+  static constexpr uint32_t value = INVALID_ID;
+};
+template <class KS>
+struct SuppressedKey<KS, std::void_t<decltype(KS::SUPPRESSED)>> {
+  static constexpr uint32_t value = KS::SUPPRESSED;
+};
+
 template <class KS, int NBITS, int WPW = 4, class E = uint16_t, int G = GROUP>
 struct ScatterEmit {
   static constexpr int NB = 1 << NBITS;
+  static constexpr uint32_t SUPPRESSED = SuppressedKey<KS>::value;
   static constexpr int CAP = 2 * G;
   static constexpr uint32_t ES = (uint32_t)sizeof(E);
   static constexpr uint32_t ESH = ES == 2u ? 1u : 2u;
@@ -428,6 +449,7 @@
   uint32_t* __restrict__ hist;
   uint32_t wave, lane, wave_global;
   uint32_t outer;
+  uint32_t* __restrict__ overflowed = nullptr;
 
   static __device__ __forceinline__ void init_lds() {
     ScatterShared<NBITS, WPW, E, CAP>& sh = scatter_lds<NBITS, WPW, E, CAP>();
@@ -539,6 +561,9 @@
       }
       const uint32_t full = G == 64 ? ((c4 >> SSH) + (uint32_t)(G - 1)) & ~(uint32_t)(G - 1) : c4 >> SSH;
       slice_fill[(size_t)wave_global * NB + lane] = full < slice_cap ? full : slice_cap;
+      if (overflowed && (c4 >> SSH) > slice_cap)
+        __hip_atomic_fetch_add(overflowed, ((c4 >> SSH) - slice_cap + (uint32_t)(G - 1)) / (uint32_t)G, __ATOMIC_RELAXED,
+                               __HIP_MEMORY_SCOPE_AGENT);
     }
     __builtin_amdgcn_wave_barrier();
     const unsigned long long trig = __builtin_amdgcn_ballot_w64(padded);
@@ -560,7 +585,22 @@
     return (KeySplit<W, NBITS>::bucket(id) << PBITS) | KeySplit<W, NBITS>::payload(id);
   }
 };
-template <int W, bool BOTH, int NBITS, bool BG>
+template <int W>
+struct KeySplitTop {
+  static_assert(W == 10, "built for 20-bit ids: 4 bucket bits and a 16-bit payload");
+  static constexpr int NBITS = 4, PBITS = 16, G = 128;
+  static constexpr uint32_t NB = 16;
+  static constexpr uint32_t SUPPRESSED = (1u << (2 * W)) - 1u;
+  __host__ __device__ static inline uint32_t bucket(uint32_t id) { return id >> PBITS; }
+  __host__ __device__ static inline uint32_t payload(uint32_t id) { return id; }
+  __host__ __device__ static inline uint32_t join(uint32_t b, uint32_t p, uint32_t  = 0) { return (b << PBITS) | p; }
+  __host__ __device__ static inline uint32_t index(uint32_t id) { return id; }
+  __host__ __device__ static inline bool valid(uint32_t) { return true; }
+};
+template <int W, int NBITS, bool TOP>
+using OneLevelSplit = std::conditional_t<TOP, KeySplitTop<W == 10 ? W : 10>, KeySplitTemp<W, NBITS>>;
+
+template <int W, bool BOTH, int NBITS, bool BG, bool TOP = false>
 __global__ __launch_bounds__(64 * SCATTER_WPW) void count_scatter_kernel(const uint32_t* __restrict__ words32,
                                                             const uint64_t* __restrict__ items, uint32_t n_items,
                                                             uint16_t* __restrict__ keys, uint32_t slice_cap,
@@ -568,15 +608,17 @@
                                                             unsigned long long* __restrict__ ltot,
                                                             uint32_t* __restrict__ defer_count,
                                                             uint32_t* __restrict__ defer_list,
-                                                            uint32_t* __restrict__ bg_partials) {
-  typedef KeySplitTemp<W, NBITS> KS;
+                                                            uint32_t* __restrict__ bg_partials,
+                                                            uint32_t* __restrict__ overflowed) {
+  static_assert(!TOP || (W == 10 && NBITS == 4), "the top-bit split is built for W = 10");
+  typedef OneLevelSplit<W, NBITS, TOP> KS;
   static_assert(KS::PBITS == PAYLOAD_BITS || BOTH, "the 16-bucket split needs both strands");
   typedef ScatterEmit<KS, NBITS, SCATTER_WPW, uint16_t, KS::G> Emit;
   Emit::init_lds();
   bg_begin<BG>();
   __syncthreads();
   const uint32_t wave = (uint32_t)__builtin_amdgcn_readfirstlane((int)(threadIdx.x >> 6));
-  Emit e{keys, slice_cap, slice_fill, temp, wave, threadIdx.x & 63u, blockIdx.x * (uint32_t)SCATTER_WPW + wave, 0u};
+  Emit e{keys, slice_cap, slice_fill, temp, wave, threadIdx.x & 63u, blockIdx.x * (uint32_t)SCATTER_WPW + wave, 0u, overflowed};
   e.bind();
   scan_items<W, BOTH, BG>(words32, items, n_items, ltot, defer_count, defer_list, e);
   e.drain();
@@ -768,17 +810,42 @@
   }
 }
 
-__device__ __forceinline__ void hist16_block(uint32_t* __restrict__ h, uint32_t block, const uint16_t* __restrict__ keys,
-                                             uint32_t slice_cap, uint32_t n_slices, uint32_t nb,
-                                             const uint32_t* __restrict__ slice_fill, uint32_t bpb,
-                                             uint32_t* __restrict__ temp, uint32_t* __restrict__ wrapped) {
+struct TopMap {
+  uint16_t start[17];
+};
+inline TopMap top_map(uint32_t num_cu, uint64_t windows) {
+  TopMap m;
+  uint32_t at = 0;
+  for (uint32_t b = 0; b < 16u; ++b) {
+    const uint64_t load = 31u - 2u * b;
+    uint64_t n = ((uint64_t)num_cu * 2u * load + 128u) / 256u;
+    const uint64_t useful = (windows * load / 256u + 1u + 65535u) / 65536u;
+    if (n > useful) n = useful;
+    if (n < 1) n = 1;
+    if (n > 2048) n = 2048;
+    m.start[b] = (uint16_t)at;
+    at += (uint32_t)n;
+  }
+  m.start[16] = (uint16_t)at;
+  return m;
+}
+__host__ __device__ inline void top_map_share(const TopMap& m, uint32_t n_slices, uint32_t wg, uint32_t& b, uint32_t& first,
+                                              uint32_t& last) {
+  b = 0;
+  for (uint32_t i = 1; i < 16u; ++i) b += wg >= m.start[i] ? 1u : 0u;
+  const uint32_t parts = (uint32_t)m.start[b + 1] - m.start[b], part = wg - m.start[b];
+  first = (uint32_t)((uint64_t)part * n_slices / parts);
+  last = (uint32_t)((uint64_t)(part + 1u) * n_slices / parts);
+}
+
+__device__ __forceinline__ void hist16_block(uint32_t* __restrict__ h, uint32_t b, uint32_t first, uint32_t last,
+                                             const uint16_t* __restrict__ keys, uint32_t slice_cap, uint32_t nb,
+                                             const uint32_t* __restrict__ slice_fill, uint32_t* __restrict__ temp,
+                                             uint32_t* __restrict__ wrapped) {
   __shared__ unsigned long long sums[2];
-  const uint32_t b = block / bpb, j = block % bpb;
   for (uint32_t i = threadIdx.x; i < (1u << 15); i += blockDim.x) h[i] = 0;
   if (threadIdx.x < 2) sums[threadIdx.x] = 0;
   __syncthreads();
-  const uint32_t per = (n_slices + bpb - 1) / bpb;
-  const uint32_t first = j * per, last = min(n_slices, j * per + per);
   const uint32_t wave = threadIdx.x >> 6, lane = threadIdx.x & 63u;
   typedef uint32_t u32x4 __attribute__((ext_vector_type(4)));
   auto add2 = [&](uint32_t x) {
@@ -880,12 +947,12 @@
   }
 }
 
-template <int W, int NBITS>
+template <int W, int NBITS, bool TOP = false>
 __global__ __launch_bounds__(256) void count_gather_kernel(const uint32_t* __restrict__ temp, uint32_t np,
                                                            uint32_t* __restrict__ hist,
                                                            const unsigned long long* __restrict__ ltot_acc,
                                                            unsigned long long* __restrict__ ltot) {
-  using KS = KeySplitTemp<W, NBITS>;
+  using KS = OneLevelSplit<W, NBITS, TOP>;
   if (blockIdx.x == 0 && threadIdx.x == 0) *ltot = *ltot_acc;
   for (uint32_t x = blockIdx.x * blockDim.x + threadIdx.x; x < np; x += gridDim.x * blockDim.x) {
     uint32_t v = temp[KS::index(x)];
@@ -1098,7 +1165,7 @@
   bg_finish_block(lds, partials, n_blocks, out);
 }
 
-template <int W, int NBITS>
+template <int W, int NBITS, bool TOP = false>
 __global__ __launch_bounds__(1024) void count_hist_front_kernel(const uint16_t* __restrict__ keys, uint32_t slice_cap,
                                                                 uint32_t n_slices, const uint32_t* __restrict__ slice_fill,
                                                                 uint32_t bpb, uint32_t* __restrict__ temp,
@@ -1108,7 +1175,8 @@
                                                                 const uint64_t* __restrict__ items, int both,
                                                                 const uint32_t* __restrict__ defer_count,
                                                                 const uint32_t* __restrict__ defer_list, uint32_t n_fix,
-                                                                uint32_t* __restrict__ wrapped) {
+                                                                uint32_t* __restrict__ wrapped, TopMap map) {
+  typedef OneLevelSplit<W, NBITS, TOP> KS;
   extern __shared__ __attribute__((aligned(16))) uint32_t h[];
   if (blockIdx.x == 0) {
     if (bg_out) bg_finish_block(reinterpret_cast<unsigned long long*>(h), bg_partials, bg_blocks, bg_out);
@@ -1119,14 +1187,21 @@
     fixup_items(words32, items, W, both, defer_count[0], defer_list, (blockIdx.x - 1u) * blockDim.x + threadIdx.x,
                 n_fix * blockDim.x, [&](uint32_t i) -> uint32_t& { return r[i * 1024u]; },
                 [&](uint32_t id) {
-                  __hip_atomic_fetch_add(&temp[KeySplitTemp<W, NBITS>::index(id)], 1u, __ATOMIC_RELAXED, __HIP_MEMORY_SCOPE_AGENT);
+                  __hip_atomic_fetch_add(&temp[KS::index(id)], 1u, __ATOMIC_RELAXED, __HIP_MEMORY_SCOPE_AGENT);
                 });
     return;
   }
-  if constexpr (KeySplitTemp<W, NBITS>::PBITS == 16)
-    hist16_block(h, blockIdx.x - 1u - n_fix, keys, slice_cap, n_slices, 1u << NBITS, slice_fill, bpb, temp, wrapped);
-  else
-    hist_block(h, blockIdx.x - 1u - n_fix, keys, slice_cap, n_slices, 1u << NBITS, slice_fill, bpb, temp, 0u);
+  const uint32_t block = blockIdx.x - 1u - n_fix;
+  if constexpr (TOP) {
+    uint32_t b, first, last;
+    top_map_share(map, n_slices, block, b, first, last);
+    if (first < last) hist16_block(h, b, first, last, keys, slice_cap, 1u << NBITS, slice_fill, temp, wrapped);
+  } else if constexpr (KS::PBITS == 16) {
+    const uint32_t b = block / bpb, j = block % bpb, per = (n_slices + bpb - 1) / bpb;
+    hist16_block(h, b, j * per, min(n_slices, j * per + per), keys, slice_cap, 1u << NBITS, slice_fill, temp, wrapped);
+  } else {
+    hist_block(h, block, keys, slice_cap, n_slices, 1u << NBITS, slice_fill, bpb, temp, 0u);
+  }
 }
 
 __global__ __launch_bounds__(128) void bg_model_kernel(const unsigned long long* __restrict__ n, int K, float a0, float a1, float a2,
@@ -1254,9 +1329,9 @@
   return d_bg ? bg_finish_fused(ctx, blocks, d_bg) : PENGK_OK;
 }
 
-template <int W, int NBITS = 2 * W - PAYLOAD_BITS>
+template <int W, int NBITS = 2 * W - PAYLOAD_BITS, bool TOP = false>
 int launch_partition_w(pengk_ctx* ctx, int both, uint32_t* d_counts, uint64_t* d_ltot, uint32_t n_items, uint64_t* d_bg) {
-  typedef KeySplitTemp<W, NBITS> KS;
+  typedef OneLevelSplit<W, NBITS, TOP> KS;
   constexpr uint32_t GRP = (uint32_t)KS::G;
   constexpr uint32_t NB = 1u << NBITS;
   const uint32_t np = 1u << (2 * W);
@@ -1271,6 +1346,7 @@
   uint64_t windows = ctx->n_windows_hint ? ctx->n_windows_hint : ctx->n_items * (uint64_t)ctx->item_windows;
   const uint64_t share = windows / ((uint64_t)NB * n_waves);
   uint64_t cap64 = share + share / 2 + 512;
+  if (TOP) cap64 = share * 31 / 16 + share * 31 / 64 + 512;
   if (ctx->key_cap_override) cap64 = ctx->key_cap_override;
   cap64 = (cap64 + GRP - 1) / GRP * GRP;
   if (cap64 * NB >= (1ull << 31))
@@ -1279,7 +1355,7 @@
   int rc = ensure_scratch(ctx, &ctx->d_keys, &ctx->keys_bytes, (size_t)NB * n_waves * slice_cap * sizeof(uint16_t));
   if (rc) return rc;
   const size_t fill_words = ((size_t)NB * n_waves + 63) / 64 * 64;
-  constexpr size_t HEAD_WORDS = 4;
+  constexpr size_t HEAD_WORDS = 8;
   const size_t aux_need = (fill_words + HEAD_WORDS + (size_t)np) * sizeof(uint32_t);
   rc = ensure_scratch(ctx, &ctx->d_count_aux, &ctx->count_aux_bytes, aux_need);
   if (rc) return rc;
@@ -1291,6 +1367,9 @@
   ctx->d_defer_count = defer_count;
   uint32_t* wrapped = slice_fill + fill_words + 3;
   ctx->d_wrap_count = wrapped;
+  uint32_t* overflowed = slice_fill + fill_words + 4;
+  ctx->d_overflow_count = overflowed;
+  ctx->count_split_used = TOP ? 2 : 1;
   ctx->d_slice_fill = slice_fill;
   ctx->n_slice_fill = (uint64_t)NB * n_waves;
   ctx->count_group_used = (int)GRP;
@@ -1302,15 +1381,15 @@
   }
   if constexpr (KS::PBITS == 16) {
     if (d_bg)
-      hipLaunchKernelGGL((count_scatter_kernel<W, true, NBITS, true>), dim3(blocks), dim3(TPB), 0, ctx->stream, w32, ctx->d_items,
-                         n_items, keys, slice_cap, slice_fill, temp, ltot_acc, defer_count, ctx->d_defer + 1, bgp);
+      hipLaunchKernelGGL((count_scatter_kernel<W, true, NBITS, true, TOP>), dim3(blocks), dim3(TPB), 0, ctx->stream, w32, ctx->d_items,
+                         n_items, keys, slice_cap, slice_fill, temp, ltot_acc, defer_count, ctx->d_defer + 1, bgp, overflowed);
     else
-      hipLaunchKernelGGL((count_scatter_kernel<W, true, NBITS, false>), dim3(blocks), dim3(TPB), 0, ctx->stream, w32, ctx->d_items,
-                         n_items, keys, slice_cap, slice_fill, temp, ltot_acc, defer_count, ctx->d_defer + 1, bgp);
+      hipLaunchKernelGGL((count_scatter_kernel<W, true, NBITS, false, TOP>), dim3(blocks), dim3(TPB), 0, ctx->stream, w32, ctx->d_items,
+                         n_items, keys, slice_cap, slice_fill, temp, ltot_acc, defer_count, ctx->d_defer + 1, bgp, overflowed);
   } else {
 #define TA_SCATTER(B, BG) W, B, NBITS, BG
     PENGK_LAUNCH_BB(count_scatter_kernel, TA_SCATTER, both, d_bg != nullptr, dim3(blocks), dim3(TPB), w32, ctx->d_items, n_items,
-                    keys, slice_cap, slice_fill, temp, ltot_acc, defer_count, ctx->d_defer + 1, bgp);
+                    keys, slice_cap, slice_fill, temp, ltot_acc, defer_count, ctx->d_defer + 1, bgp, overflowed);
 #undef TA_SCATTER
   }
   PENGK_HIP(hipGetLastError());
@@ -1321,12 +1400,18 @@
   if (bpb > n_waves) bpb = n_waves;
   if (bpb < 1) bpb = 1;
   constexpr uint32_t N_FIX = 4;
-  hipLaunchKernelGGL((count_hist_front_kernel<W, NBITS>), dim3(1u + N_FIX + NB * bpb), dim3(1024), 4 << PAYLOAD_BITS, ctx->stream,
+  TopMap map = {};
+  uint32_t n_hist = NB * bpb;
+  if (TOP) {
+    map = top_map((uint32_t)ctx->num_cu, windows);
+    n_hist = map.start[16];
+  }
+  hipLaunchKernelGGL((count_hist_front_kernel<W, NBITS, TOP>), dim3(1u + N_FIX + n_hist), dim3(1024), 4 << PAYLOAD_BITS, ctx->stream,
                      keys, slice_cap, n_waves, slice_fill, bpb, temp, bgp, blocks, (unsigned long long*)d_bg, w32, ctx->d_items, both,
-                     defer_count, ctx->d_defer + 1, N_FIX, wrapped);
+                     defer_count, ctx->d_defer + 1, N_FIX, wrapped, map);
   PENGK_HIP(hipGetLastError());
   const uint32_t gb = (np + 255) / 256 < 2048u ? (np + 255) / 256 : 2048u;
-  hipLaunchKernelGGL((count_gather_kernel<W, NBITS>), dim3(gb), dim3(256), 0, ctx->stream, temp, np, d_counts, ltot_acc,
+  hipLaunchKernelGGL((count_gather_kernel<W, NBITS, TOP>), dim3(gb), dim3(256), 0, ctx->stream, temp, np, d_counts, ltot_acc,
                      (unsigned long long*)d_ltot);
   PENGK_HIP(hipGetLastError());
   return PENGK_OK;
@@ -1476,6 +1561,8 @@
   return PENGK_OK;
 }
 
+constexpr uint64_t TOP_SPLIT_MIN_WINDOWS = 1ull << 24;
+
 template <int W>
 int launch_count_w(pengk_ctx* ctx, int both, uint32_t* d_counts, uint64_t* d_ltot, uint64_t* d_bg) {
   const uint32_t n_items = (uint32_t)ctx->n_items;
@@ -1498,8 +1585,17 @@
   if (ctx->count_group == 128 && !can_group128)
     return fail(PENGK_ERR_UNSUPPORTED, "count_group 128 is built for the partitioned count at W = 10 on both strands only (W = %d, %s, count_impl %d)",
                 W, both ? "both strands" : "one strand", impl);
+  const bool can_top = can_group128 && ctx->count_group != 64;
+  if (ctx->count_split == 2 && !can_top)
+    return fail(PENGK_ERR_UNSUPPORTED, "count_split 2 is built for groups of 128 keys of the partitioned count at W = 10 on both strands only (W = %d, %s, count_impl %d, count_group %d)",
+                W, both ? "both strands" : "one strand", impl, ctx->count_group);
   if constexpr (W == 10) {
-    if (can_group128 && ctx->count_group != 64) return launch_partition_w<10, 4>(ctx, both, d_counts, d_ltot, n_items, d_bg);
+    if (can_top) {
+      const uint64_t windows = ctx->n_windows_hint ? ctx->n_windows_hint : ctx->n_items * (uint64_t)ctx->item_windows;
+      if (ctx->count_split == 2 || (ctx->count_split == 0 && ctx->count_group == 0 && windows >= TOP_SPLIT_MIN_WINDOWS))
+        return launch_partition_w<10, 4, true>(ctx, both, d_counts, d_ltot, n_items, d_bg);
+      return launch_partition_w<10, 4>(ctx, both, d_counts, d_ltot, n_items, d_bg);
+    }
   }
   int rc;
   if constexpr (W == 14) {
@@ -1528,6 +1624,7 @@
   PENGK_HIP(hipFuncSetAttribute((const void*)count_hist_front_kernel<8, 16 - PAYLOAD_BITS>, hipFuncAttributeMaxDynamicSharedMemorySize, 4 << PAYLOAD_BITS));
   PENGK_HIP(hipFuncSetAttribute((const void*)count_hist_front_kernel<10, 20 - PAYLOAD_BITS>, hipFuncAttributeMaxDynamicSharedMemorySize, 4 << PAYLOAD_BITS));
   PENGK_HIP(hipFuncSetAttribute((const void*)count_hist_front_kernel<10, 4>, hipFuncAttributeMaxDynamicSharedMemorySize, 4 << PAYLOAD_BITS));
+  PENGK_HIP(hipFuncSetAttribute((const void*)count_hist_front_kernel<10, 4, true>, hipFuncAttributeMaxDynamicSharedMemorySize, 4 << PAYLOAD_BITS));
   return PENGK_OK;
 }
 
@@ -1546,7 +1643,9 @@
   const bool one_level = (W == 8 || W == 10) && ctx->count_impl != 1 && ctx->n_items > 0;
   ctx->d_wrap_count = nullptr;
   ctx->d_slice_fill = nullptr;
+  ctx->d_overflow_count = nullptr;
   ctx->count_group_used = 0;
+  ctx->count_split_used = 0;
   if (!one_level) {
     ctx->d_defer_count = ctx->d_defer;
     PENGK_HIP(hipMemsetAsync(ctx->d_defer, 0, sizeof(uint32_t), ctx->stream));
@@ -1563,6 +1662,15 @@
     case 14: return launch_count_w<14>(ctx, both, d_counts, d_ltot, d_bg);
     default: return fail(PENGK_ERR_ARG, "pattern length %d unsupported", W);
   }
+}
+
+int count_top_map(int num_cu, uint32_t n_slices, uint64_t windows, uint32_t* n_wg, uint32_t* bucket, uint32_t* first,
+                  uint32_t* last) {
+  const TopMap m = top_map((uint32_t)num_cu, windows);
+  *n_wg = m.start[16];
+  if (bucket && first && last)
+    for (uint32_t wg = 0; wg < m.start[16]; ++wg) top_map_share(m, n_slices, wg, bucket[wg], first[wg], last[wg]);
+  return PENGK_OK;
 }
 
 int launch_mirror(pengk_ctx* ctx, int W, uint32_t* d_counts) {
diff --git a/peng-motif_amd/csrc/pengk_internal.h b/peng-motif_amd/csrc/pengk_internal.h
--- a/peng-motif_amd/csrc/pengk_internal.h
+++ b/peng-motif_amd/csrc/pengk_internal.h
@@ -60,6 +60,9 @@
   int count_impl = 0;
   int count_group = 0;
   int count_group_used = 0;
+  int count_split = 0;
+  int count_split_used = 0;
+  const uint32_t* d_overflow_count = nullptr;
   const uint32_t* d_wrap_count = nullptr;
   const uint32_t* d_slice_fill = nullptr;
   uint64_t n_slice_fill = 0;
@@ -124,6 +127,7 @@
 
 int launch_count(pengk_ctx* ctx, int both, uint32_t* d_counts, uint64_t* d_ltot, uint64_t* d_bg );
 int launch_mirror(pengk_ctx* ctx, int W, uint32_t* d_counts);
+int count_top_map(int num_cu, uint32_t n_slices, uint64_t windows, uint32_t* n_wg, uint32_t* bucket, uint32_t* first, uint32_t* last);
 int launch_bg_count(pengk_ctx* ctx, uint64_t* d_bg);
 int launch_bg_model(pengk_ctx* ctx, const uint64_t* d_bg, int K, const float* h_alpha, float* d_V);
 int launch_synth(pengk_ctx* ctx, uint64_t seed, uint64_t seq0, uint64_t n_seq, uint32_t L, int W, int item_windows,
```

Result: slower. 165.3 (-71.9%).
